# gsanya/orbslam2_NMI

Measured on AMD Instinct MI355X. Metric: pose-candidate NMI evals/sec (640x480, 256 bins), one blocking nmi_search_grid call per step incl. its 8-byte read-back (SURVEY.md 8d's definition); beside the W warm-up steps an untimed clock warm-up of clock_warmup_ms = 200 ms precedes the timed region, higher is better.
Workload: dtype u8

## Files before the change

### include/nmi_hip.h

```cpp
#ifndef NMI_HIP_H
#define NMI_HIP_H

#include <stddef.h>
#include <stdint.h>

#ifdef __cplusplus
extern "C" {
#endif

#define NMI_HIP_ABI_VERSION 2

#define NMI_OK 0
#define NMI_ERR_INVALID_ARGUMENT (-1)
#define NMI_ERR_UNSUPPORTED (-2)
#define NMI_ERR_NO_DEVICE (-3)
#define NMI_ERR_NOT_READY (-4)
#define NMI_ERR_HIP (-1000)
#define NMI_ERR_RCCL (-2000)

#define NMI_MODE_ENMI 0
#define NMI_MODE_SUC 1

typedef struct nmi_ctx nmi_ctx;

// ... 118 lines not shown
int nmi_level_create_mesh_block(nmi_ctx *ctx, const float *d_xyz, const float *d_uv, int64_t n_triangles, const nmi_texture *tex,
                                const uint8_t *d_frame, int32_t S_local, int32_t s_offset, int32_t S_total, int32_t Wn_local,
                                int32_t w_offset, int32_t Wn_total, nmi_level **out);
int nmi_level_create_mesh_colored_block(nmi_ctx *ctx, const float *d_xyz, const float *d_red, int64_t n_triangles, const uint8_t *d_frame,
                                        int32_t S_local, int32_t s_offset, int32_t S_total, int32_t Wn_local, int32_t w_offset,
                                        int32_t Wn_total, nmi_level **out);
int nmi_level_run_rccl(nmi_level *lv, const float *h_mvps, const double *h_forward, void *nccl_comm, int64_t *h_best_index,
                       float *h_best_score);
int nmi_level_copy_outputs(nmi_level *lv, uint8_t *h_renders, uint8_t *h_warps, float *h_ratings);
int nmi_level_set_masks(nmi_level *lv, int32_t enabled, const uint8_t *d_frame_mask);
int nmi_level_copy_masks(nmi_level *lv, uint8_t *h_warp_masks, int32_t *h_counts);
int nmi_level_set_coverage(nmi_level *lv, int32_t enabled, const uint8_t *d_frame_mask);
int nmi_level_copy_coverage(nmi_level *lv, uint8_t *h_render_masks, uint8_t *h_warp_masks, int32_t *h_counts);
int nmi_level_set_distortion(nmi_level *lv, const double K[9], const float dist[5] );
int nmi_level_set_distortion_fisheye(nmi_level *lv, const double K[9], const double K_raw[9] ,
                                     const float dist[4] );
int nmi_level_set_frame_format(nmi_level *lv, int32_t format, int64_t pitch );
int nmi_level_set_frame_reduction(nmi_level *lv, int32_t factor , int32_t format, int64_t pitch );
int nmi_level_destroy(nmi_level *lv);

typedef struct nmi_stream nmi_stream;
int nmi_stream_create(nmi_ctx *ctx, int32_t max_S, int32_t max_Wn, int32_t depth, nmi_stream **out);
int nmi_stream_destroy(nmi_stream *st);
int nmi_stream_submit(nmi_stream *st, const uint8_t *h_render_stack, int32_t S, const uint8_t *h_frame,
                      const double *h_forward, int32_t Wn, int64_t *ticket);
int nmi_stream_submit_block(nmi_stream *st, const uint8_t *h_render_stack, int32_t S_local, int32_t s_offset, int32_t S_total,
                            const uint8_t *h_frame, const double *h_forward, int32_t Wn_local, int32_t w_offset, int32_t Wn_total,
                            void *nccl_comm, int64_t *ticket);
int nmi_stream_wait(nmi_stream *st, int64_t ticket, int64_t *h_best_index, float *h_best_score);
int nmi_stream_keep_ratings(nmi_stream *st, int32_t enabled);
int nmi_stream_copy_ratings(nmi_stream *st, int64_t ticket, float *h_ratings, int64_t n);
int nmi_stream_submit_masked(nmi_stream *st, const uint8_t *h_render_stack, int32_t S, const uint8_t *h_frame,
                             const uint8_t *h_frame_mask , const double *h_forward, int32_t Wn, int64_t *ticket);
int nmi_stream_submit_masked_block(nmi_stream *st, const uint8_t *h_render_stack, int32_t S_local, int32_t s_offset, int32_t S_total,
                                   const uint8_t *h_frame, const uint8_t *h_frame_mask , const double *h_forward,
                                   int32_t Wn_local, int32_t w_offset, int32_t Wn_total, void *nccl_comm, int64_t *ticket);
int nmi_stream_submit_covered(nmi_stream *st, const uint8_t *h_render_stack, const uint8_t *h_render_mask_bits, int32_t S,
                              const uint8_t *h_frame, const uint8_t *h_frame_mask , const double *h_forward,
                              int32_t Wn, int64_t *ticket);
int nmi_stream_submit_covered_block(nmi_stream *st, const uint8_t *h_render_stack, const uint8_t *h_render_mask_bits, int32_t S_local,
                                    int32_t s_offset, int32_t S_total, const uint8_t *h_frame, const uint8_t *h_frame_mask ,
                                    const double *h_forward, int32_t Wn_local, int32_t w_offset, int32_t Wn_total, void *nccl_comm,
                                    int64_t *ticket);
int nmi_stream_copy_counts(nmi_stream *st, int64_t ticket, int32_t *h_counts, int64_t n);
int nmi_stream_set_distortion(nmi_stream *st, const double K[9], const float dist[5] );
int nmi_stream_set_distortion_fisheye(nmi_stream *st, const double K[9], const double K_raw[9] ,
                                      const float dist[4] );
int nmi_stream_set_frame_format(nmi_stream *st, int32_t format, int64_t pitch );
int nmi_stream_set_frame_reduction(nmi_stream *st, int32_t factor , int32_t format, int64_t pitch );

uint64_t nmi_key_pack(float score, int64_t global_linear_index);
int nmi_key_unpack(uint64_t key, int64_t *global_linear_index, float *score);

int nmi_search_grid_rccl(nmi_ctx *ctx, const uint8_t *render_stack, int32_t S_local, int32_t s_offset,
                         int32_t S_total, const uint8_t *warp_stack, int32_t Wn, float *d_ratings,
                         void *nccl_comm, int64_t *h_best_index, float *h_best_score);
int nmi_search_grid_block_rccl(nmi_ctx *ctx, const uint8_t *render_stack, int32_t S_local, int32_t s_offset, int32_t S_total,
                               const uint8_t *warp_stack, int32_t Wn_local, int32_t w_offset, int32_t Wn_total, float *d_ratings,
                               void *nccl_comm, int64_t *h_best_index, float *h_best_score);

int nmi_rccl_unique_id(uint8_t out_id[128]);
int nmi_rccl_comm_init(nmi_ctx *ctx, const uint8_t id[128], int32_t rank, int32_t nranks, void **out_comm);
int nmi_rccl_comm_destroy(void *nccl_comm);

int nmi_set_profiling(nmi_ctx *ctx, int32_t enabled);
int nmi_last_kernel_ms(nmi_ctx *ctx, float *h_ms);

#define NMI_OPT_HIST_VARIANT 1
#define NMI_OPT_PHASE_MASK 2
#define NMI_OPT_WORKGROUPS 3
#define NMI_OPT_RESULT_PATH 4
#define NMI_OPT_XCD_TILING 5
#define NMI_OPT_TILE_QUEUE 6
#define NMI_OPT_CLIP_QUEUE 11
#define NMI_OPT_SPLIT 7
#define NMI_OPT_WAIT_MODE 8
#define NMI_OPT_SPLIT_PIXELS 10
#define NMI_OPT_CONTENT_PATH 12
#define NMI_OPT_FEWLEVELS_BINS 13
#define NMI_OPT_PIX_OWNER_BIAS 14
#define NMI_OPT_STAMPS 9
#define NMI_OPT_STAMP_CANDIDATE 15
#define NMI_OPT_WAVE_SHARES 16
int nmi_set_option(nmi_ctx *ctx, int32_t option, int64_t value);

int nmi_split_status(nmi_ctx *ctx, int32_t *timeouts, int32_t *cooldown_calls_left, int32_t *next_cooldown, int32_t *last_launch_parts);
int nmi_pix_status(nmi_ctx *ctx, int32_t *last_launch_ranges, int32_t *healed);

int nmi_copy_term_table(nmi_ctx *ctx, float *h_out, int64_t n);
int nmi_abi_version(void);
const char *nmi_error_string(int code);
const char *nmi_last_error_detail(nmi_ctx *ctx);
int nmi_get_info(nmi_ctx *ctx, int32_t *compute_units, int32_t *workgroups_per_launch, int32_t *lds_bytes);
int nmi_last_content(nmi_ctx *ctx, int32_t *few_levels, int32_t *nr, int32_t *nw);

#ifdef __cplusplus
}
#endif
#endif
```

### orbslam2_nmi_amd/capi.py

```python
import ctypes as C
import os

import numpy as np

from . import build as _build

MODE_ENMI = 0
MODE_SUC = 1

NMI_OK = 0
ERR_INVALID_ARGUMENT = -1
ERR_UNSUPPORTED = -2
ERR_NO_DEVICE = -3
ERR_NOT_READY = -4

FRAME_GRAY = 0
FRAME_BGR = 1
FRAME_RGB = 2
FRAME_BGRA = 3
FRAME_RGBA = 4
FRAME_BYTES_PER_PIXEL = {FRAME_GRAY: 1, FRAME_BGR: 3, FRAME_RGB: 3, FRAME_BGRA: 4, FRAME_RGBA: 4}

EXPORTED_SYMBOLS = (
    "nmi_params_default", "nmi_create", "nmi_destroy", "nmi_set_stream", "nmi_synchronize", "nmi_eval_pair", "nmi_eval_pairs", "nmi_eval_pair_debug",
    "nmi_search_grid", "nmi_search_grid_shard", "nmi_search_grid_block", "nmi_warp_homographies", "nmi_warp_stack", "nmi_render_mvp", "nmi_render_points", "nmi_level_create", "nmi_level_create_mesh", "nmi_level_run", "nmi_level_copy_outputs", "nmi_level_destroy", "nmi_texture_create",
    "nmi_texture_destroy", "nmi_render_mesh", "nmi_stream_create", "nmi_stream_destroy",
    "nmi_stream_submit", "nmi_stream_wait", "nmi_stream_keep_ratings", "nmi_stream_copy_ratings", "nmi_key_pack", "nmi_key_unpack", "nmi_search_grid_rccl", "nmi_search_grid_block_rccl",
    "nmi_rccl_unique_id", "nmi_rccl_comm_init", "nmi_rccl_comm_destroy", "nmi_set_profiling", "nmi_last_kernel_ms",
    "nmi_set_option", "nmi_copy_term_table", "nmi_abi_version", "nmi_error_string", "nmi_last_error_detail", "nmi_get_info", "nmi_last_content", "nmi_sort_points", "nmi_sort_triangles",
    "nmi_split_status", "nmi_pix_status", "nmi_level_create_block", "nmi_level_create_mesh_block", "nmi_level_run_rccl", "nmi_stream_submit_block",
    "nmi_warp_stack_masked", "nmi_search_grid_masked", "nmi_last_mask_counts", "nmi_level_set_masks", "nmi_level_copy_masks",
    "nmi_render_points_masked", "nmi_render_mesh_masked", "nmi_search_grid_covered", "nmi_last_cover_counts",
    "nmi_level_set_coverage", "nmi_level_copy_coverage",
    "nmi_pack_mask_bits", "nmi_stream_submit_masked", "nmi_stream_submit_masked_block", "nmi_stream_submit_covered",
    "nmi_stream_submit_covered_block", "nmi_stream_copy_counts",
    "nmi_undistort_frame", "nmi_level_set_distortion", "nmi_stream_set_distortion",
    "nmi_gray_frame", "nmi_level_set_frame_format", "nmi_stream_set_frame_format",
    "nmi_reduce_frame", "nmi_level_set_frame_reduction", "nmi_stream_set_frame_reduction",
    "nmi_render_mesh_colored", "nmi_render_mesh_colored_masked", "nmi_sort_triangles_colored", "nmi_level_create_mesh_colored",
    "nmi_level_create_mesh_colored_block",
    "nmi_undistort_frame_fisheye", "nmi_level_set_distortion_fisheye", "nmi_stream_set_distortion_fisheye",
)


class NmiParams(C.Structure):
    _fields_ = [
        ("width", C.c_int32), ("height", C.c_int32), ("bins", C.c_int32), ("mode", C.c_int32),
        ("use_bg", C.c_int32), ("render_bottom_up", C.c_int32), ("device", C.c_int32),
        ("max_candidates", C.c_int32), ("stream", C.c_void_p), ("reserved", C.c_int32 * 8),
    ]


class RenderParams(C.Structure):
    _fields_ = [("fx", C.c_double), ("fy", C.c_double), ("cx", C.c_double), ("cy", C.c_double), ("near_plane", C.c_float),
                ("far_plane", C.c_float), ("point_size", C.c_float)]


class NmiError(RuntimeError):
    def __init__(self, code, what, detail=""):
        self.code = code
        super().__init__(f"{what} failed: {code} ({error_string(code)}) {detail}".strip())


_lib = None


def library_path():
    return _build.LIB


def load_library(build_if_missing=False):
    global _lib
    if _lib is not None:
        return _lib
    path = _build.LIB
    if build_if_missing:
        _build.build()
    if not os.path.exists(path):
        raise RuntimeError(f"{path} is missing: run `python -m orbslam2_nmi_amd.build` (hipcc, gfx950). "
                           "There is no CPU fallback for the NMI path.")
    lib = C.CDLL(path, mode=C.RTLD_GLOBAL)
    vp, i32, i64p, f32p, u64p = C.c_void_p, C.c_int32, C.POINTER(C.c_int64), C.POINTER(C.c_float), C.POINTER(C.c_uint64)
    lib.nmi_params_default.argtypes = [C.POINTER(NmiParams), i32, i32]
    lib.nmi_create.argtypes = [C.POINTER(NmiParams), C.POINTER(vp)]
    lib.nmi_destroy.argtypes = [vp]
    lib.nmi_set_stream.argtypes = [vp, vp]
    lib.nmi_synchronize.argtypes = [vp]
    lib.nmi_eval_pair.argtypes = [vp, vp, vp, f32p]
    lib.nmi_eval_pairs.argtypes = [vp, C.POINTER(vp), C.POINTER(vp), i32, f32p]
    lib.nmi_eval_pair_debug.argtypes = [vp, vp, vp, f32p, vp, vp, vp, vp]
    lib.nmi_search_grid.argtypes = [vp, vp, i32, vp, i32, vp, i64p, f32p]
    lib.nmi_search_grid_shard.argtypes = [vp, vp, i32, i32, i32, vp, i32, vp, vp, u64p]
    lib.nmi_search_grid_block.argtypes = [vp, vp, i32, i32, i32, vp, i32, i32, i32, vp, vp, u64p]
    lib.nmi_warp_homographies.argtypes = [C.POINTER(C.c_double), C.POINTER(i32), f32p, C.POINTER(C.c_double)]
    lib.nmi_warp_stack.argtypes = [vp, vp, C.POINTER(C.c_double), i32, vp]
    lib.nmi_warp_stack_masked.argtypes = [vp, vp, vp, C.POINTER(C.c_double), i32, vp, vp]
    lib.nmi_search_grid_masked.argtypes = [vp, vp, i32, vp, vp, i32, vp, i64p, f32p]
    lib.nmi_last_mask_counts.argtypes = [vp, C.POINTER(i32), i32]
    lib.nmi_render_points_masked.argtypes = [vp, vp, vp, C.c_int64, C.POINTER(C.c_float), i32, C.c_float, vp, vp]
    lib.nmi_render_mesh_masked.argtypes = [vp, vp, vp, C.c_int64, vp, C.POINTER(C.c_float), i32, vp, vp]
    lib.nmi_search_grid_covered.argtypes = [vp, vp, vp, i32, vp, vp, i32, vp, i64p, f32p]
    lib.nmi_last_cover_counts.argtypes = [vp, C.POINTER(i32), i32]
    lib.nmi_render_mvp.argtypes = [C.POINTER(RenderParams), f32p, f32p, f32p, f32p, f32p]
    lib.nmi_render_points.argtypes = [vp, vp, vp, C.c_int64, f32p, i32, C.c_float, vp]
    lib.nmi_texture_create.argtypes = [vp, vp, i32, i32, C.POINTER(vp)]
    lib.nmi_texture_destroy.argtypes = [vp]
    lib.nmi_render_mesh.argtypes = [vp, vp, vp, C.c_int64, vp, f32p, i32, vp]
    lib.nmi_level_create.argtypes = [vp, vp, vp, C.c_int64, vp, i32, i32, C.c_float, C.POINTER(vp)]
    lib.nmi_level_create_mesh.argtypes = [vp, vp, vp, C.c_int64, vp, vp, i32, i32, C.POINTER(vp)]
    lib.nmi_level_run.argtypes = [vp, f32p, C.POINTER(C.c_double), i64p, f32p]
    lib.nmi_level_create_block.argtypes = [vp, vp, vp, C.c_int64, vp, i32, i32, i32, i32, i32, i32, C.c_float, C.POINTER(vp)]
    lib.nmi_level_create_mesh_block.argtypes = [vp, vp, vp, C.c_int64, vp, vp, i32, i32, i32, i32, i32, i32, C.POINTER(vp)]
    lib.nmi_render_mesh_colored.argtypes = [vp, vp, vp, C.c_int64, f32p, i32, vp]
    lib.nmi_render_mesh_colored_masked.argtypes = [vp, vp, vp, C.c_int64, f32p, i32, vp, vp]
    lib.nmi_sort_triangles_colored.argtypes = [vp, vp, vp, C.c_int64, vp, vp]
    lib.nmi_level_create_mesh_colored.argtypes = [vp, vp, vp, C.c_int64, vp, i32, i32, C.POINTER(vp)]
    lib.nmi_level_create_mesh_colored_block.argtypes = [vp, vp, vp, C.c_int64, vp, i32, i32, i32, i32, i32, i32, C.POINTER(vp)]
    lib.nmi_level_run_rccl.argtypes = [vp, f32p, C.POINTER(C.c_double), vp, i64p, f32p]
    lib.nmi_stream_submit_block.argtypes = [vp, vp, i32, i32, i32, vp, C.POINTER(C.c_double), i32, i32, i32, vp, i64p]
    lib.nmi_level_copy_outputs.argtypes = [vp, vp, vp, vp]
    lib.nmi_level_set_masks.argtypes = [vp, i32, vp]
    lib.nmi_level_copy_masks.argtypes = [vp, vp, C.POINTER(i32)]
    lib.nmi_level_set_coverage.argtypes = [vp, i32, vp]
    lib.nmi_level_copy_coverage.argtypes = [vp, vp, vp, C.POINTER(i32)]
    lib.nmi_level_destroy.argtypes = [vp]
    lib.nmi_stream_create.argtypes = [vp, i32, i32, i32, C.POINTER(vp)]
    lib.nmi_stream_destroy.argtypes = [vp]
    lib.nmi_stream_submit.argtypes = [vp, vp, i32, vp, C.POINTER(C.c_double), i32, i64p]
    lib.nmi_stream_wait.argtypes = [vp, C.c_int64, i64p, f32p]
    lib.nmi_stream_keep_ratings.argtypes = [vp, i32]
    lib.nmi_stream_copy_ratings.argtypes = [vp, C.c_int64, f32p, C.c_int64]
    lib.nmi_pack_mask_bits.argtypes = [vp, vp, i32, vp]
    lib.nmi_stream_submit_masked.argtypes = [vp, vp, i32, vp, vp, C.POINTER(C.c_double), i32, i64p]
    lib.nmi_stream_submit_masked_block.argtypes = [vp, vp, i32, i32, i32, vp, vp, C.POINTER(C.c_double), i32, i32, i32, vp, i64p]
    lib.nmi_stream_submit_covered.argtypes = [vp, vp, vp, i32, vp, vp, C.POINTER(C.c_double), i32, i64p]
    lib.nmi_stream_submit_covered_block.argtypes = [vp, vp, vp, i32, i32, i32, vp, vp, C.POINTER(C.c_double), i32, i32, i32, vp, i64p]
    lib.nmi_stream_copy_counts.argtypes = [vp, C.c_int64, C.POINTER(i32), C.c_int64]
    lib.nmi_undistort_frame.argtypes = [vp, C.POINTER(C.c_double), f32p, vp, vp, vp, vp]
    lib.nmi_level_set_distortion.argtypes = [vp, C.POINTER(C.c_double), f32p]
    lib.nmi_stream_set_distortion.argtypes = [vp, C.POINTER(C.c_double), f32p]
    lib.nmi_undistort_frame_fisheye.argtypes = [vp, C.POINTER(C.c_double), C.POINTER(C.c_double), f32p, vp, vp, vp, vp]
    lib.nmi_level_set_distortion_fisheye.argtypes = [vp, C.POINTER(C.c_double), C.POINTER(C.c_double), f32p]
    lib.nmi_stream_set_distortion_fisheye.argtypes = [vp, C.POINTER(C.c_double), C.POINTER(C.c_double), f32p]
    lib.nmi_gray_frame.argtypes = [vp, vp, i32, C.c_int64, vp]
    lib.nmi_level_set_frame_format.argtypes = [vp, i32, C.c_int64]
    lib.nmi_stream_set_frame_format.argtypes = [vp, i32, C.c_int64]
    lib.nmi_reduce_frame.argtypes = [vp, vp, i32, C.c_int64, i32, vp, vp, vp]
    lib.nmi_level_set_frame_reduction.argtypes = [vp, i32, i32, C.c_int64]
    lib.nmi_stream_set_frame_reduction.argtypes = [vp, i32, i32, C.c_int64]
    lib.nmi_key_pack.argtypes = [C.c_float, C.c_int64]
    lib.nmi_key_pack.restype = C.c_uint64
    lib.nmi_key_unpack.argtypes = [C.c_uint64, i64p, f32p]
    lib.nmi_search_grid_rccl.argtypes = [vp, vp, i32, i32, i32, vp, i32, vp, vp, i64p, f32p]
    lib.nmi_search_grid_block_rccl.argtypes = [vp, vp, i32, i32, i32, vp, i32, i32, i32, vp, vp, i64p, f32p]
    lib.nmi_rccl_unique_id.argtypes = [C.POINTER(C.c_uint8)]
    lib.nmi_rccl_comm_init.argtypes = [vp, C.POINTER(C.c_uint8), i32, i32, C.POINTER(vp)]
    lib.nmi_rccl_comm_destroy.argtypes = [vp]
    lib.nmi_set_option.argtypes = [vp, i32, C.c_int64]
    lib.nmi_set_profiling.argtypes = [vp, i32]
    lib.nmi_last_kernel_ms.argtypes = [vp, f32p]
    lib.nmi_copy_term_table.argtypes = [vp, f32p, C.c_int64]
    lib.nmi_error_string.argtypes = [C.c_int]
    lib.nmi_error_string.restype = C.c_char_p
    lib.nmi_last_error_detail.argtypes = [vp]
    lib.nmi_last_error_detail.restype = C.c_char_p
    lib.nmi_get_info.argtypes = [vp, C.POINTER(i32), C.POINTER(i32), C.POINTER(i32)]
    lib.nmi_last_content.argtypes = [vp, C.POINTER(i32), C.POINTER(i32), C.POINTER(i32)]
    lib.nmi_split_status.argtypes = [vp, C.POINTER(i32), C.POINTER(i32), C.POINTER(i32), C.POINTER(i32)]
    lib.nmi_pix_status.argtypes = [vp, C.POINTER(i32), C.POINTER(i32)]
    lib.nmi_sort_points.argtypes = [vp, vp, vp, C.c_int64, vp, vp]
    lib.nmi_sort_triangles.argtypes = [vp, vp, vp, C.c_int64, vp, vp]
    _lib = lib
    return lib


def error_string(code):
    return load_library().nmi_error_string(int(code)).decode()


def key_pack(score, index):
    return int(load_library().nmi_key_pack(float(score), int(index)))


def key_unpack(key):
    idx, sc = C.c_int64(0), C.c_float(0)
    load_library().nmi_key_unpack(C.c_uint64(int(key) & 0xFFFFFFFFFFFFFFFF), C.byref(idx), C.byref(sc))
    return int(idx.value), np.float32(sc.value)


def warp_homographies(K, num_warp_xyz, step_rad_xyz):
    K = np.ascontiguousarray(K, np.float64).reshape(9)
    num = (C.c_int32 * 3)(*[int(n) for n in num_warp_xyz])
    step = (C.c_float * 3)(*[float(s) for s in step_rad_xyz])
    wn = int(np.prod([int(n) for n in num_warp_xyz]))
    out = np.zeros((wn, 3, 3), np.float64)
    rc = load_library().nmi_warp_homographies(K.ctypes.data_as(C.POINTER(C.c_double)), num, step,
                                              out.ctypes.data_as(C.POINTER(C.c_double)))
    if rc != NMI_OK:
        raise NmiError(rc, "nmi_warp_homographies")
    return out


def render_mvp(rp, cam_pos, cam_look_at, cam_up, translation):
    f3 = lambda v: (C.c_float * 3)(*[float(x) for x in v])
    out = (C.c_float * 16)()
    rc = load_library().nmi_render_mvp(C.byref(rp), f3(cam_pos), f3(cam_look_at), f3(cam_up), f3(translation), out)
    if rc != NMI_OK:
        raise NmiError(rc, "nmi_render_mvp")
    return np.array(out, np.float32)


def _lens(K, dist):
    if K is None and dist is None:
        return None, None, None, None
    k = np.ascontiguousarray(K, np.float64).reshape(-1)
    if k.size != 9:
        raise ValueError("K must have 9 entries")
    if dist is None:
        return k, None, k.ctypes.data_as(C.POINTER(C.c_double)), None
    d = np.ascontiguousarray(dist, np.float32).reshape(-1)
    if d.size != 5:
        raise ValueError("dist must be k1 k2 p1 p2 k3 (5 entries; pad k3 = 0)")
    return k, d, k.ctypes.data_as(C.POINTER(C.c_double)), d.ctypes.data_as(C.POINTER(C.c_float))


def _fisheye(K, K_raw, dist):
    if K is None and dist is None:
        return (None, None, None), (None, None, None)
    k = np.ascontiguousarray(K, np.float64).reshape(-1)
    kr = None if K_raw is None else np.ascontiguousarray(K_raw, np.float64).reshape(-1)
    if k.size != 9 or (kr is not None and kr.size != 9):
        raise ValueError("K and K_raw must have 9 entries")
    d = None if dist is None else np.ascontiguousarray(dist, np.float32).reshape(-1)
    if d is not None and d.size != 4:
        raise ValueError("dist must be k1 k2 k3 k4 (4 entries)")
    dp = C.POINTER(C.c_double)
    return (k, kr, d), (k.ctypes.data_as(dp), None if kr is None else kr.ctypes.data_as(dp),
                        None if d is None else d.ctypes.data_as(C.POINTER(C.c_float)))


def _dev_mask(t, ndim, what):
    import torch
    if not isinstance(t, torch.Tensor) or not t.is_cuda:
        raise TypeError(f"{what} must be a device (HIP) torch tensor; the NMI path has no CPU implementation")
    if t.dtype not in (torch.uint8, torch.bool) or t.dim() != ndim or not t.is_contiguous():
        raise TypeError(f"{what} must be a contiguous uint8 or bool tensor with {ndim} dims, got {t.dtype} {tuple(t.shape)}")
    return t


def _dev_u8(t, ndim, what):
    import torch
    if not isinstance(t, torch.Tensor) or not t.is_cuda:
        raise TypeError(f"{what} must be a device (HIP) torch tensor; the NMI path has no CPU implementation")
    if t.dtype != torch.uint8 or t.dim() != ndim or not t.is_contiguous():
        raise TypeError(f"{what} must be a contiguous uint8 tensor with {ndim} dims, got {t.dtype} {tuple(t.shape)}")
    return t


class NmiContext:

    default_options = {}

    def __init__(self, width, height, bins=256, mode=MODE_SUC, use_bg=True, render_bottom_up=True, device=None,
                 stream=None, max_candidates=0):
        import torch
        if not torch.cuda.is_available():
            raise RuntimeError("no HIP device visible: orbslam2_nmi_amd needs an AMD GPU (gfx950)")
        self._lib = load_library()
        self.width, self.height = int(width), int(height)
        self.bins, self.mode, self.use_bg, self.render_bottom_up = bins, mode, bool(use_bg), bool(render_bottom_up)
        if device is None:
            device = torch.cuda.current_device()
        self.device = torch.device("cuda", int(device) if not isinstance(device, torch.device) else device.index or 0)
        p = NmiParams()
        self._check(self._lib.nmi_params_default(C.byref(p), self.width, self.height), "nmi_params_default")
        p.bins, p.mode, p.use_bg, p.render_bottom_up = int(bins), int(mode), int(bool(use_bg)), int(bool(render_bottom_up))
        p.device = self.device.index
        p.max_candidates = int(max_candidates)
        p.stream = stream
        self._h = C.c_void_p()
        rc = self._lib.nmi_create(C.byref(p), C.byref(self._h))
        if rc != NMI_OK:
            self._h = C.c_void_p()
            raise NmiError(rc, "nmi_create")
        for opt, val in type(self).default_options.items():
            self.set_option(opt, val)

    def _check(self, rc, what):
        if rc != NMI_OK:
            detail = self._lib.nmi_last_error_detail(self._h).decode() if getattr(self, "_h", None) else ""
            raise NmiError(rc, what, detail)

    def close(self):
        if getattr(self, "_h", None) and self._h.value:
            self._lib.nmi_destroy(self._h)
            self._h = C.c_void_p()

    def __del__(self):
        try:
            self.close()
        except Exception:
            pass

    def __enter__(self):
        return self

    def __exit__(self, *exc):
        self.close()

    def set_stream(self, stream_handle):
        if stream_handle == 0:
            raise ValueError("handle 0 is the legacy default stream; use a torch.cuda.Stream() (non-default) instead")
        self._check(self._lib.nmi_set_stream(self._h, C.c_void_p(stream_handle)), "nmi_set_stream")
        self._bound_stream = stream_handle

    def _order_after_torch(self):
        import torch
        cur = torch.cuda.current_stream(self.device)
        if getattr(self, "_bound_stream", None) != cur.cuda_stream:
            cur.synchronize()

    OPT_HIST_VARIANT, OPT_PHASE_MASK, OPT_WORKGROUPS, OPT_RESULT_PATH, OPT_XCD_TILING, OPT_TILE_QUEUE = 1, 2, 3, 4, 5, 6
    OPT_SPLIT, OPT_WAIT_MODE, OPT_STAMPS, OPT_SPLIT_PIXELS, OPT_CLIP_QUEUE = 7, 8, 9, 10, 11
    OPT_PIX_OWNER_BIAS = 14
    OPT_STAMP_CANDIDATE, OPT_WAVE_SHARES = 15, 16
    OPT_CONTENT_PATH, OPT_FEWLEVELS_BINS = 12, 13

    def set_option(self, option, value):
        self._check(self._lib.nmi_set_option(self._h, int(option), int(value)), "nmi_set_option")

    def synchronize(self):
        self._check(self._lib.nmi_synchronize(self._h), "nmi_synchronize")

    def set_profiling(self, on):
        self._check(self._lib.nmi_set_profiling(self._h, int(bool(on))), "nmi_set_profiling")

    def last_kernel_ms(self):
        ms = C.c_float(0)
        self._check(self._lib.nmi_last_kernel_ms(self._h, C.byref(ms)), "nmi_last_kernel_ms")
        return float(ms.value)

    def info(self):
        cu, wg, lds = C.c_int32(0), C.c_int32(0), C.c_int32(0)
        self._check(self._lib.nmi_get_info(self._h, C.byref(cu), C.byref(wg), C.byref(lds)), "nmi_get_info")
        return {"compute_units": cu.value, "workgroups_per_launch": wg.value, "lds_bytes": lds.value}

    def last_content(self):
        f, r, w = C.c_int32(0), C.c_int32(0), C.c_int32(0)
        self._check(self._lib.nmi_last_content(self._h, C.byref(f), C.byref(r), C.byref(w)), "nmi_last_content")
        return {"few_levels": bool(f.value), "nr": r.value, "nw": w.value}

    def split_status(self):
        v = [C.c_int32(0) for _ in range(4)]
        self._check(self._lib.nmi_split_status(self._h, *[C.byref(x) for x in v]), "nmi_split_status")
        return dict(zip(("timeouts", "cooldown_calls_left", "next_cooldown", "last_launch_parts"), (x.value for x in v)))

    def pix_status(self):
        v = [C.c_int32(0) for _ in range(2)]
        self._check(self._lib.nmi_pix_status(self._h, *[C.byref(x) for x in v]), "nmi_pix_status")
        return dict(zip(("last_launch_ranges", "healed"), (x.value for x in v)))

    def term_table(self):
        out = np.zeros(self.width * self.height + 1, np.float32)
        self._check(self._lib.nmi_copy_term_table(self._h, out.ctypes.data_as(C.POINTER(C.c_float)), out.size),
                    "nmi_copy_term_table")
        return out

    def _img(self, t, what):
        t = _dev_u8(t, 2, what)
        if tuple(t.shape) != (self.height, self.width):
            raise ValueError(f"{what} is {tuple(t.shape)}, context is {(self.height, self.width)}")
        return t

    def _stack(self, t, what):
        t = _dev_u8(t, 3, what)
        if tuple(t.shape[1:]) != (self.height, self.width):
            raise ValueError(f"{what} is {tuple(t.shape)}, context images are {(self.height, self.width)}")
        return t

    def eval_pair(self, render, warped):
        r, w = self._img(render, "render"), self._img(warped, "warped")
        out = C.c_float(0)
        self._order_after_torch()
        self._check(self._lib.nmi_eval_pair(self._h, r.data_ptr(), w.data_ptr(), C.byref(out)), "nmi_eval_pair")
        return np.float32(out.value)

    def eval_pairs(self, renders, warps):
        assert len(renders) == len(warps)
        n = len(renders)
        rp = (C.c_void_p * max(n, 1))(*[self._img(r, "render").data_ptr() for r in renders])
        wp = (C.c_void_p * max(n, 1))(*[self._img(w, "warped").data_ptr() for w in warps])
        out = np.zeros(n, np.float32)
        self._order_after_torch()
        self._check(self._lib.nmi_eval_pairs(self._h, rp, wp, n, out.ctypes.data_as(C.POINTER(C.c_float))), "nmi_eval_pairs")
        return out

    def eval_pair_debug(self, render, warped):
        import torch
        r, w = self._img(render, "render"), self._img(warped, "warped")
        joint = torch.zeros(65536, dtype=torch.int32, device=self.device)
        h1 = torch.zeros(256, dtype=torch.int32, device=self.device)
        h2 = torch.zeros(256, dtype=torch.int32, device=self.device)
        sums = torch.zeros(3, dtype=torch.float32, device=self.device)
        torch.cuda.synchronize(self.device)
        out = C.c_float(0)
        self._check(self._lib.nmi_eval_pair_debug(self._h, r.data_ptr(), w.data_ptr(), C.byref(out), joint.data_ptr(),
                                                  h1.data_ptr(), h2.data_ptr(), sums.data_ptr()), "nmi_eval_pair_debug")
        u32 = lambda t: t.cpu().numpy().view(np.uint32)
        return np.float32(out.value), u32(joint).reshape(256, 256), u32(h1), u32(h2), sums.cpu().numpy()

    def sort_points(self, xyz, red):
        import torch
        assert xyz.is_cuda and red.is_cuda and xyz.dtype == torch.float32 and red.dtype == torch.float32
        xyz, red = xyz.contiguous(), red.contiguous()
        n = xyz.shape[0]
        assert tuple(xyz.shape) == (n, 3) and red.numel() == n
        xo, ro = torch.empty_like(xyz), torch.empty_like(red)
        self._order_after_torch()
        self._check(self._lib.nmi_sort_points(self._h, xyz.data_ptr(), red.data_ptr(), n, xo.data_ptr(), ro.data_ptr()), "nmi_sort_points")
        return xo, ro

    def sort_triangles(self, xyz, uv):
        import torch
        assert xyz.is_cuda and uv.is_cuda and xyz.dtype == torch.float32 and uv.dtype == torch.float32
        xyz, uv = xyz.contiguous(), uv.contiguous()
        t = xyz.shape[0] // 3
        assert tuple(xyz.shape) == (3 * t, 3) and tuple(uv.shape) == (3 * t, 2)
        xo, uo = torch.empty_like(xyz), torch.empty_like(uv)
        self._order_after_torch()
        self._check(self._lib.nmi_sort_triangles(self._h, xyz.data_ptr(), uv.data_ptr(), t, xo.data_ptr(), uo.data_ptr()), "nmi_sort_triangles")
        return xo, uo

    def sort_triangles_colored(self, xyz, red):
# ... 707 lines not shown
```

### orbslam2_nmi_amd/csrc/nmi_capi.cpp

```cpp
#include <sched.h>

#include "nmi_ctx.h"

namespace nmi_internal {

int hip_fail(nmi_ctx *ctx, hipError_t e, const char *what)
{
    if (ctx) {
        char buf[256];
        snprintf(buf, sizeof buf, "%s: %s (%d)", what, hipGetErrorString(e), (int)e);
        ctx->detail = buf;
    }
    return NMI_ERR_HIP - (int)e;
}



void build_order(int S, int Wn, int *order)
{
    const int tile_s = S >= 8 ? 8 : (S >= 4 ? 4 : (S >= 2 ? 2 : 1)), tile_w = 32 / tile_s;
    int64_t o = 0;
    for (int w0 = 0; w0 < Wn; w0 += tile_w)
        for (int s0 = 0; s0 < S; s0 += tile_s)
            for (int w = w0; w < w0 + tile_w && w < Wn; ++w)
                for (int s = s0; s < s0 + tile_s && s < S; ++s) order[o++] = w * S + s;
}

int ensure_order(nmi_ctx *ctx, int S, int Wn, const int **d_order)
{
    *d_order = nullptr;
    if (!ctx->xcd_tiling) return NMI_OK;
    const int64_t total = (int64_t)S * Wn;
    nmi_ctx::OrderEntry *victim = nullptr;
    for (auto &e : ctx->orders) {
        if (e.S == S && e.Wn == Wn) {
            e.last_use = ++ctx->order_clock;
            *d_order = e.d;
            return NMI_OK;
        }
        if (!victim || (e.d == nullptr && victim->d != nullptr) || ((e.d == nullptr) == (victim->d == nullptr) && e.last_use < victim->last_use))
            victim = &e;
    }
    nmi_ctx::OrderEntry &e = *victim;
    if (e.d) NMI_HIP_TRY(ctx, hipStreamSynchronize(ctx->stream));
    if (total > e.cap) {
        if (e.d) NMI_HIP_TRY(ctx, hipFree(e.d));
        if (e.h) NMI_HIP_TRY(ctx, hipHostFree(e.h));
        e.d = e.h = nullptr;
        e.cap = 0;
        e.S = e.Wn = -1;
        NMI_HIP_TRY(ctx, hipMalloc((void **)&e.d, (size_t)total * sizeof(int)));
        NMI_HIP_TRY(ctx, hipHostMalloc((void **)&e.h, (size_t)total * sizeof(int), hipHostMallocDefault));
        e.cap = total;
    }
    build_order(S, Wn, e.h);
    NMI_HIP_TRY(ctx, hipMemcpyAsync(e.d, e.h, (size_t)total * sizeof(int), hipMemcpyHostToDevice, ctx->stream));
    e.S = S;
    e.Wn = Wn;
    e.last_use = ++ctx->order_clock;
    *d_order = e.d;
    return NMI_OK;
}

static void choose_split(const nmi_ctx *ctx, int64_t total, int cap, int *parts, int *pix_parts)
{
    *parts = 0;
    *pix_parts = 1;
    if (cap > ctx->compute_units) cap = ctx->compute_units;
    if (ctx->hist_variant != 3 || ctx->split_mode == 0 || ctx->split_mode == 1 || total <= 0 || total > cap) return;
    auto fits = [&](int k, int p) { return nmi::split_workgroups((int)total, k, p) <= cap; };
    auto exists = [](int k, int p) { return p == 1 || (k == 8 && (p == 2 || p == 4)) || (k == 4 && p == 2); };
    const int want_p = ctx->split_pixels;
    if (ctx->split_mode > 0) {
        const int k = ctx->split_mode;
        if (!fits(k, 1)) return;
        *parts = k;
        if (want_p == 1) return;
        for (int p = 4; p >= 2; p >>= 1)
            if ((want_p == -1 || want_p == p) && exists(k, p) && fits(k, p)) {
                *pix_parts = p;
                return;
            }
        return;
    }
    static const int order[][2] = {{8, 4}, {8, 2}, {4, 2}, {8, 1}, {4, 1}};
    for (const auto &kp : order) {
        if (kp[1] > 1 && want_p != -1 && want_p != kp[1]) continue;
        if (fits(kp[0], kp[1])) {
            *parts = kp[0];
            *pix_parts = kp[1];
            return;
        }
    }
}

int choose_pix(const nmi_ctx *ctx, const nmi::GridArgs &a, int64_t total, int cap)
{
    if (cap > ctx->compute_units) cap = ctx->compute_units;
    if (ctx->hist_variant != 3 || a.width < 32 || (ctx->shift != 0 && !ctx->params.use_bg) || ctx->pair_renders || total <= 0) return 0;
    if ((ctx->phase_mask & ~512) != 3 || (a.dbg_stamps != nullptr && ctx->split_mode != 1)) return 0;
    if (ctx->split_mode == 1) {
        const int p = ctx->split_pixels;
        return (p >= 2 && p <= nmi::pix_max_ranges() && total * p <= cap) ? p : 0;
    }
    if (ctx->split_mode != -1 || ctx->split_pixels != -1 || total * 2 > cap) return 0;
    const int p = (int)(cap / total);
    if (!a.vec_ok) return p > nmi::pix_max_ranges() ? nmi::pix_max_ranges() : p;
    if (total <= 32) return 0;
    return p > 3 ? 3 : p;
}

double pix_owner_share(const nmi_ctx *ctx, int pix)
{
    const double owner_px = ((double)ctx->npix + (double)(pix - 1) * ctx->pix_owner_bias) / pix;
    return owner_px < ctx->npix ? owner_px / ctx->npix : 1.0;
}

int ensure_pix_timeouts(nmi_ctx *ctx)
{
    if (ctx->d_pix_timeouts) return NMI_OK;
    NMI_HIP_TRY(ctx, hipMalloc((void **)&ctx->d_pix_timeouts, sizeof(uint32_t)));
    NMI_HIP_TRY(ctx, hipMemsetAsync(ctx->d_pix_timeouts, 0, sizeof(uint32_t), ctx->stream));
    return NMI_OK;
}

int next_split_epoch(nmi_ctx *ctx, uint32_t *epoch)
{
    uint32_t e = ctx->split_epoch + 1;
    if ((e & 0xFFFFu) == 0) {
        if (ctx->d_blocks) NMI_HIP_TRY(ctx, hipMemsetAsync(ctx->d_blocks, 0, ctx->blocks_bytes, ctx->stream));
        if (ctx->d_pix_blocks) NMI_HIP_TRY(ctx, hipMemsetAsync(ctx->d_pix_blocks, 0, ctx->pix_blocks_bytes, ctx->stream));
        if (e == 0 && ctx->d_slabs) NMI_HIP_TRY(ctx, hipMemsetAsync(ctx->d_slabs, 0, (size_t)ctx->slab_cap * sizeof(nmi::SplitSlab), ctx->stream));
        ++e;
    }
    ctx->split_epoch = *epoch = e;
    return NMI_OK;
}

static int ensure_slabs(nmi_ctx *ctx, int n)
{
    if (n <= ctx->slab_cap) return NMI_OK;
    if (ctx->d_slabs) {
        NMI_HIP_TRY(ctx, hipStreamSynchronize(ctx->stream));
        NMI_HIP_TRY(ctx, hipFree(ctx->d_slabs));
// ... 16 lines not shown
        ctx->d_pix_blocks = nullptr;
        ctx->pix_blocks_bytes = 0;
    }
    NMI_HIP_TRY(ctx, hipMalloc((void **)&ctx->d_pix_blocks, bytes));
    NMI_HIP_TRY(ctx, hipMemsetAsync(ctx->d_pix_blocks, 0, bytes, ctx->stream));
    ctx->pix_blocks_bytes = bytes;
    return NMI_OK;
}

static int ensure_blocks(nmi_ctx *ctx, size_t bytes)
{
    if (bytes <= ctx->blocks_bytes) return NMI_OK;
    if (ctx->d_blocks) {
        NMI_HIP_TRY(ctx, hipStreamSynchronize(ctx->stream));
        NMI_HIP_TRY(ctx, hipFree(ctx->d_blocks));
        ctx->d_blocks = nullptr;
        ctx->blocks_bytes = 0;
    }
    NMI_HIP_TRY(ctx, hipMalloc((void **)&ctx->d_blocks, bytes));
    NMI_HIP_TRY(ctx, hipMemsetAsync(ctx->d_blocks, 0, bytes, ctx->stream));
    ctx->blocks_bytes = bytes;
    return NMI_OK;
}

int enqueue_grid(nmi_ctx *ctx, const uint8_t *render_stack, int S_local, int s_offset, int S_total,
                 const uint8_t *warp_stack, int Wn, float *d_ratings, unsigned long long *out_key, bool post,
                 uint32_t *dbg_joint, uint32_t *dbg_h1, uint32_t *dbg_h2, float *dbg_sums, int w_offset, bool post_score)
{
    const nmi_params &p = ctx->params;
    nmi::GridArgs a{};
    a.render_stack = render_stack;
    a.warp_stack = warp_stack;
    a.S_local = S_local;
    a.Wn = Wn;
    a.s_offset = s_offset;
    a.S_total = S_total;
    a.w_offset = w_offset;
    nmi::set_geometry(a, p.width, p.height, render_stack, warp_stack, p.render_bottom_up != 0);
    if (ctx->pair_renders) {
        a.pair_renders = ctx->pair_renders;
        a.pair_warps = ctx->pair_warps;
        uintptr_t bits = 0;
        for (int i = 0; i < S_local; ++i) bits |= (uintptr_t)ctx->pair_renders_host[i] | (uintptr_t)ctx->pair_warps_host[i];
        if (bits % 16) nmi::set_geometry(a, p.width, p.height, (const void *)1, (const void *)1, p.render_bottom_up != 0);
    }
    a.shift = ctx->shift;
    a.mode = p.mode;
    a.table = ctx->table;
    a.scratch = ctx->d_scratch;
    a.order = nullptr;
    a.ratings = d_ratings;
    a.key = ctx->d_keys + ctx->slot;
    a.reset_key = ctx->d_keys + (ctx->slot ^ 1);
    a.out_key = out_key;
    a.done = ctx->d_done;
    const bool split_checked = post || post_score || ctx->allow_unchecked_split || ctx->pair_renders != nullptr;
    post = post && ctx->result_path == 1;
    post_score = post_score && ctx->result_path == 1;
    a.mailbox = post ? ctx->mailbox : nullptr;
    a.score_post = post_score ? ctx->score_mailbox : nullptr;
    a.seq = post ? ctx->seq + 1 : (post_score ? ctx->pair_seq + 1 : 0);
    a.dbg_joint = dbg_joint;
    a.dbg_h1 = dbg_h1;
    a.dbg_h2 = dbg_h2;
    a.dbg_sums = dbg_sums;
    a.hist_variant = ctx->hist_variant;
    a.phase_mask = ctx->phase_mask;
    a.dbg_stamps = ctx->dbg_stamps;

    const int64_t total = (int64_t)S_local * Wn;
    if (total == 0) {
        if (out_key) NMI_HIP_TRY(ctx, hipMemsetAsync(out_key, 0, sizeof(unsigned long long), ctx->stream));
        NMI_HIP_TRY(ctx, hipMemsetAsync(ctx->d_keys + ctx->slot, 0, sizeof(unsigned long long), ctx->stream));
        NMI_HIP_TRY(ctx, hipStreamSynchronize(ctx->stream));
        if (post) {
            ++ctx->seq;
            ctx->mailbox->word = (unsigned long long)(ctx->seq & 1u) << 63;
        }
        ctx->posted = post;
        ctx->last_slot = ctx->slot;
        ctx->last_parts = 0;
        ctx->last_pix = 0;
        ctx->last_epoch = 0;
        return NMI_OK;
    }
    const int cap = ctx->workgroups > 0 ? ctx->workgroups : ctx->compute_units;
    int parts = 0, pix_parts = 1;
    choose_split(ctx, total, cap, &parts, &pix_parts);
    if (pix_parts > 1 && ctx->npix >= (1 << 24)) pix_parts = 1;
    int pix = choose_pix(ctx, a, total, cap);
    if (pix) parts = 0;
    if (parts && !split_checked) parts = 0;
    if (parts && ctx->split_cooldown > 0) {
        --ctx->split_cooldown;
        parts = 0;
    }
    if (!parts) pix_parts = 1;
    bool few = false;
    const bool few_eligible = !parts && !(pix && ctx->split_mode == 1) && a.vec_ok && (ctx->shift == 0 || p.use_bg) && ctx->hist_variant == 3 && ctx->phase_mask == 3 && !dbg_joint &&
                              !dbg_h1 && !dbg_h2 && !dbg_sums && !ctx->pair_renders && !ctx->dbg_stamps && ctx->content_path != 0;
    if (few_eligible) {
        const unsigned long long posted = __atomic_load_n(ctx->level_post, __ATOMIC_ACQUIRE);
        if ((uint32_t)(posted >> 32) != ctx->level_seen) {
            ctx->level_seen = (uint32_t)(posted >> 32);
            const uint32_t joint = (uint32_t)((posted >> 16) & 0xFFFFu) * (uint32_t)(posted & 0xFFFFu);
            ctx->few_hint = joint > 0 && joint <= (uint32_t)ctx->fewlevels_bins;
        }
        few = ctx->content_path == 1 || ctx->few_hint;
    }
    if (few) pix = 0;
    if (ctx->pair_renders && !parts) return NMI_ERR_UNSUPPORTED;
    int workgroups = (int)(total < cap ? total : cap);
    if (parts) {
        int rs = ensure_slabs(ctx, (int)total);
        if (rs == NMI_OK && pix_parts > 1) rs = ensure_blocks(ctx, (size_t)total * nmi::split_block_bytes_per_candidate(pix_parts));
        if (rs != NMI_OK) return rs;
        if (rs == NMI_OK) rs = next_split_epoch(ctx, &a.epoch);
        if (rs != NMI_OK) return rs;
        a.slabs = ctx->d_slabs;
        a.blocks = ctx->d_blocks;
        a.split_error = ctx->d_split_error;
        workgroups = nmi::split_workgroups((int)total, parts, pix_parts);
    } else if (pix) {
        int rs = ensure_pix_blocks(ctx, nmi::pix_block_bytes((int)total, pix));
        if (rs == NMI_OK) rs = next_split_epoch(ctx, &a.epoch);
        if (rs == NMI_OK) rs = ensure_pix_timeouts(ctx);
        if (rs != NMI_OK) return rs;
        a.blocks = ctx->d_pix_blocks;
        workgroups = (int)total * pix;
    } else if (ctx->xcd_tiling && total <= (1ll << 24)) {
        const int orc = ensure_order(ctx, S_local, Wn, &a.order);
        if (orc != NMI_OK) return orc;
    }
#ifdef NMI_BUILD_ABLATIONS
    if (ctx->hist_variant == 4 && workgroups > ctx->scratch_workgroups) {
        NMI_HIP_TRY(ctx, hipStreamSynchronize(ctx->stream));
        if (ctx->d_scratch) NMI_HIP_TRY(ctx, hipFree(ctx->d_scratch));
        ctx->d_scratch = nullptr;
        ctx->scratch_workgroups = 0;
        const int alloc = workgroups > ctx->compute_units ? workgroups : ctx->compute_units;
        NMI_HIP_TRY(ctx, hipMalloc((void **)&ctx->d_scratch, nmi::grid_kernel_scratch_bytes(alloc)));
        ctx->scratch_workgroups = alloc;
        a.scratch = ctx->d_scratch;
    }
#endif
    if (!parts && !few && ctx->hist_variant == 3 && ctx->content_path != 0) a.plan = ctx->d_plan;
    if (few) {
        const size_t need = (size_t)(S_local + Wn) * (size_t)ctx->npix;
        if (need > ctx->rank_bytes) {
            NMI_HIP_TRY(ctx, hipStreamSynchronize(ctx->stream));
            if (ctx->d_rank_stacks) NMI_HIP_TRY(ctx, hipFree(ctx->d_rank_stacks));
            ctx->d_rank_stacks = nullptr;
            ctx->rank_bytes = 0;
            const size_t want = need + need / 2;
            NMI_HIP_TRY(ctx, hipMalloc((void **)&ctx->d_rank_stacks, want));
            ctx->rank_bytes = want;
        }
        a.plan = ctx->d_plan;
    }
    if (ctx->profiling) NMI_HIP_TRY(ctx, hipEventRecord(ctx->ev_start, ctx->stream));
    if (few)
        NMI_HIP_TRY(ctx, nmi::launch_levels(render_stack, S_local, warp_stack, Wn, ctx->npix, ctx->shift, ctx->d_plan, ctx->level_post, ++ctx->level_seq,
                                            (uint32_t)ctx->fewlevels_bins, few, ctx->stream));
    if (parts) {
        NMI_HIP_TRY(ctx, nmi::launch_split(a, parts, pix_parts, workgroups, p.use_bg != 0, ctx->stream));
    } else if (pix) {
        NMI_HIP_TRY(ctx, nmi::launch_pix(a, pix, pix_owner_share(ctx, pix), p.use_bg != 0, nullptr, ctx->d_pix_timeouts, ctx->stream));
    } else if (few) {
        NMI_HIP_TRY(ctx, nmi::launch_fewlevels(a, ctx->d_rank_stacks, ctx->d_rank_stacks + (size_t)S_local * ctx->npix, workgroups,
                                               p.use_bg != 0, ctx->stream));
        NMI_HIP_TRY(ctx, nmi::launch_grid_gated(a, workgroups, p.use_bg != 0, ctx->stream));
    } else {
        NMI_HIP_TRY(ctx, nmi::launch_grid(a, workgroups, p.use_bg != 0, ctx->stream));
    }
    ctx->last_few = few ? 1 : 0;
    if (post) ++ctx->seq;
    if (post_score) ++ctx->pair_seq;
    ctx->posted = post;
    ctx->last_slot = ctx->slot;
    ctx->slot ^= 1;
    ctx->last_parts = parts;
    ctx->last_pix = pix;
    ctx->last_epoch = parts ? a.epoch : 0;
    if (ctx->profiling) {
        NMI_HIP_TRY(ctx, hipEventRecord(ctx->ev_stop, ctx->stream));
        ctx->have_timing = true;
    }
    return NMI_OK;
}

bool split_launch_failed(nmi_ctx *ctx, int parts, uint32_t epoch)
{
    if (!parts) return false;
    uint32_t *word = ctx->h_split_error + (epoch % nmi::kSplitRing);
    if (__atomic_load_n(word, __ATOMIC_ACQUIRE) != epoch) {
        if ((int32_t)(epoch - ctx->split_cooldown_epoch) > 0) ctx->split_backoff = nmi_ctx::kSplitBackoffMin;
        return false;
    }
    (void)hipStreamSynchronize(ctx->stream);
    __atomic_store_n(word, 0u, __ATOMIC_RELEASE);
    ++ctx->split_timeouts;
    ctx->split_cooldown = ctx->split_backoff;
    ctx->split_cooldown_epoch = ctx->split_epoch;
    if (ctx->split_backoff < nmi_ctx::kSplitBackoffMax) ctx->split_backoff *= 2;
    return true;
}

bool split_timed_out(nmi_ctx *ctx) { return split_launch_failed(ctx, ctx->last_parts, ctx->last_epoch); }

static const char *const kSplitTimeoutNote = "split kernel hand-off timed out; call redone by the one-workgroup kernel, split forms paused (nmi_split_status)";

int wait_word(nmi_ctx *ctx, const volatile unsigned long long *word, unsigned long long mask, unsigned long long want,
              unsigned long long *out)
{
    const uint64_t check_every = ctx->wait_mode == 1 ? 0x3F : 0xFFFF;
    for (uint64_t spin = 0;; ++spin) {
        const unsigned long long v = __atomic_load_n(word, __ATOMIC_ACQUIRE);
        if ((v & mask) == want) {
            *out = v;
            return NMI_OK;
        }
        if (ctx->wait_mode == 1) sched_yield();
        if ((spin & check_every) == check_every) {
            const hipError_t q = hipStreamQuery(ctx->stream);
            if (q == hipSuccess) {
                const unsigned long long v2 = __atomic_load_n(word, __ATOMIC_ACQUIRE);
                *out = v2;
                return (v2 & mask) == want ? NMI_OK : NMI_ERR_NOT_READY;
            }
            if (q != hipErrorNotReady) return hip_fail(ctx, q, "hipStreamQuery");
        }
    }
}

int fetch_key(nmi_ctx *ctx, unsigned long long *key)
{
    if (ctx->posted) {
        unsigned long long word = 0;
        const int rc = wait_word(ctx, &ctx->mailbox->word, 1ull << 63, (unsigned long long)(ctx->seq & 1u) << 63, &word);
        if (rc == NMI_OK) {
            *key = word & 0x7FFFFFFFFFFFFFFFull;
            return NMI_OK;
        }
        if (rc != NMI_ERR_NOT_READY) return rc;
    }
    NMI_HIP_TRY(ctx, hipMemcpyAsync(ctx->h_key, ctx->d_keys + ctx->last_slot, sizeof(unsigned long long),
                                    hipMemcpyDeviceToHost, ctx->stream));
    NMI_HIP_TRY(ctx, hipStreamSynchronize(ctx->stream));
    *key = *ctx->h_key;
    return NMI_OK;
}

int stage_floats(nmi_ctx *ctx, StagingRing &ring, const float *h_src, size_t n, float **d_out)
{
    if (n > ring.cap) {
        NMI_HIP_TRY(ctx, hipStreamSynchronize(ctx->stream));
        for (int i = 0; i < StagingRing::kSlots; ++i) {
            if (ring.d[i]) NMI_HIP_TRY(ctx, hipFree(ring.d[i]));
// ... 96 lines not shown
    ctx->shift = shift;
    DeviceGuard guard(dev);

    int rc = NMI_OK;
    auto fail = [&](hipError_t e, const char *what) {
        rc = hip_fail(ctx, e, what);
        fprintf(stderr, "nmi_create: %s\n", ctx->detail.c_str());
        nmi_destroy(ctx);
        return rc;
    };
    hipDeviceProp_t prop;
    hipError_t e = hipGetDeviceProperties(&prop, dev);
    if (e != hipSuccess) return fail(e, "hipGetDeviceProperties");
    ctx->compute_units = prop.multiProcessorCount;
    if ((size_t)nmi::grid_kernel_lds_bytes() > prop.sharedMemPerBlock) {
        nmi_destroy(ctx);
        return NMI_ERR_UNSUPPORTED;
    }
    if ((e = hipStreamCreateWithFlags(&ctx->own_stream, hipStreamNonBlocking)) != hipSuccess)
        return fail(e, "hipStreamCreateWithFlags");
    ctx->stream = p.stream ? (hipStream_t)p.stream : ctx->own_stream;
    if ((e = hipMalloc((void **)&ctx->table, ((size_t)ctx->npix + 1) * sizeof(float))) != hipSuccess)
        return fail(e, "hipMalloc(table)");
    if ((e = hipMalloc((void **)&ctx->d_keys, 2 * sizeof(unsigned long long))) != hipSuccess) return fail(e, "hipMalloc(key)");
    if ((e = hipMalloc((void **)&ctx->d_done, sizeof(unsigned int))) != hipSuccess) return fail(e, "hipMalloc(done)");
    if ((e = hipMemsetAsync(ctx->d_keys, 0, 2 * sizeof(unsigned long long), ctx->stream)) != hipSuccess)
        return fail(e, "hipMemsetAsync(key)");
    if ((e = hipMemsetAsync(ctx->d_done, 0, sizeof(unsigned int), ctx->stream)) != hipSuccess)
        return fail(e, "hipMemsetAsync(done)");
    if ((e = hipHostMalloc((void **)&ctx->mailbox, sizeof(nmi::Mailbox), hipHostMallocCoherent | hipHostMallocMapped)) !=
        hipSuccess)
        return fail(e, "hipHostMalloc(mailbox)");
    memset(ctx->mailbox, 0, sizeof(nmi::Mailbox));
    if ((e = hipMalloc((void **)&ctx->d_pair_rating, sizeof(float))) != hipSuccess) return fail(e, "hipMalloc(rating)");
    if ((e = hipMalloc((void **)&ctx->d_reduced_key, sizeof(unsigned long long))) != hipSuccess) return fail(e, "hipMalloc(reduced key)");
    if ((e = hipHostMalloc((void **)&ctx->score_mailbox, 2 * sizeof(unsigned long long), hipHostMallocCoherent | hipHostMallocMapped)) !=
        hipSuccess)
        return fail(e, "hipHostMalloc(score mailbox)");
    memset(ctx->score_mailbox, 0, 2 * sizeof(unsigned long long));
    if ((e = hipHostMalloc((void **)&ctx->h_split_error, nmi::kSplitRing * sizeof(uint32_t), hipHostMallocCoherent | hipHostMallocMapped)) != hipSuccess)
        return fail(e, "hipHostMalloc(split error)");
    memset(ctx->h_split_error, 0, nmi::kSplitRing * sizeof(uint32_t));
    if ((e = hipHostGetDevicePointer((void **)&ctx->d_split_error, ctx->h_split_error, 0)) != hipSuccess)
        return fail(e, "hipHostGetDevicePointer(split error)");
    if ((e = hipHostMalloc((void **)&ctx->h_key, sizeof(unsigned long long), hipHostMallocDefault)) != hipSuccess)
        return fail(e, "hipHostMalloc(key)");
    if ((e = hipHostMalloc((void **)&ctx->level_post, 64, hipHostMallocCoherent | hipHostMallocMapped)) != hipSuccess)
        return fail(e, "hipHostMalloc(level post)");
    *ctx->level_post = 0;
    if ((e = hipMalloc((void **)&ctx->d_plan, sizeof(nmi::LevelPlan))) != hipSuccess) return fail(e, "hipMalloc(level plan)");
    if ((e = hipMemsetAsync(ctx->d_plan, 0, sizeof(nmi::LevelPlan), ctx->stream)) != hipSuccess) return fail(e, "hipMemsetAsync(level plan)");
    {
        unsigned long long *d_post = nullptr;
        if ((e = hipHostGetDevicePointer((void **)&d_post, ctx->level_post, 0)) != hipSuccess) return fail(e, "hipHostGetDevicePointer(level post)");
        if ((e = hipMemcpyAsync(&ctx->d_plan->seen_post, &d_post, sizeof d_post, hipMemcpyHostToDevice, ctx->stream)) != hipSuccess)
            return fail(e, "hipMemcpyAsync(level post)");
        const uint32_t max_joint = (uint32_t)ctx->fewlevels_bins;
        if ((e = hipMemcpyAsync(&ctx->d_plan->seen_max_joint, &max_joint, sizeof max_joint, hipMemcpyHostToDevice, ctx->stream)) != hipSuccess)
            return fail(e, "hipMemcpyAsync(level plan)");
        if ((e = hipStreamSynchronize(ctx->stream)) != hipSuccess) return fail(e, "hipStreamSynchronize");
    }
    if ((e = hipEventCreate(&ctx->ev_start)) != hipSuccess) return fail(e, "hipEventCreate");
    if ((e = hipEventCreate(&ctx->ev_stop)) != hipSuccess) return fail(e, "hipEventCreate");
    if ((e = nmi::launch_table(ctx->table, ctx->npix, ctx->stream)) != hipSuccess) return fail(e, "launch_table");
    if ((e = hipStreamSynchronize(ctx->stream)) != hipSuccess) return fail(e, "hipStreamSynchronize");
    *out_ctx = ctx;
    return NMI_OK;
}

int nmi_destroy(nmi_ctx *ctx)
{
    if (!ctx) return NMI_OK;
    DeviceGuard guard(ctx->device);
    if (ctx->own_stream) (void)hipStreamSynchronize(ctx->own_stream);
    if (ctx->table) (void)hipFree(ctx->table);
    if (ctx->d_reduced_key) (void)hipFree(ctx->d_reduced_key);
    if (ctx->score_mailbox) (void)hipHostFree(ctx->score_mailbox);
    if (ctx->d_slabs) (void)hipFree(ctx->d_slabs);
    if (ctx->h_pair_table) (void)hipHostFree(ctx->h_pair_table);
    if (ctx->d_pair_scores) (void)hipFree(ctx->d_pair_scores);
    if (ctx->d_blocks) (void)hipFree(ctx->d_blocks);
    if (ctx->d_pix_timeouts) (void)hipFree(ctx->d_pix_timeouts);
    if (ctx->d_pix_blocks) (void)hipFree(ctx->d_pix_blocks);
    if (ctx->h_split_error) (void)hipHostFree(ctx->h_split_error);
    if (ctx->level_post) (void)hipHostFree(ctx->level_post);
    if (ctx->d_plan) (void)hipFree(ctx->d_plan);
    if (ctx->d_rank_stacks) (void)hipFree(ctx->d_rank_stacks);
    if (ctx->d_keys) (void)hipFree(ctx->d_keys);
    if (ctx->d_done) (void)hipFree(ctx->d_done);
    if (ctx->mailbox) (void)hipHostFree(ctx->mailbox);
    if (ctx->d_pair_rating) (void)hipFree(ctx->d_pair_rating);
    if (ctx->d_scratch) (void)hipFree(ctx->d_scratch);
    if (ctx->d_mask_counts) (void)hipFree(ctx->d_mask_counts);
    if (ctx->d_mask_tables) (void)hipFree(ctx->d_mask_tables);
    if (ctx->d_mask_redo) (void)hipFree(ctx->d_mask_redo);
    if (ctx->d_mask_redo_state) (void)hipFree(ctx->d_mask_redo_state);
    if (ctx->d_cover_counts) (void)hipFree(ctx->d_cover_counts);
    if (ctx->d_zbuf) (void)hipFree(ctx->d_zbuf);
    mesh_work_free(&ctx->mesh);
    for (int i = 0; i < StagingRing::kSlots; ++i) {
        if (ctx->mvp_ring.d[i]) (void)hipFree(ctx->mvp_ring.d[i]);
        if (ctx->mvp_ring.h[i]) (void)hipHostFree(ctx->mvp_ring.h[i]);
        if (ctx->mvp_ring.ev[i]) (void)hipEventDestroy(ctx->mvp_ring.ev[i]);
    }
    for (auto &oe : ctx->orders) {
        if (oe.d) (void)hipFree(oe.d);
        if (oe.h) (void)hipHostFree(oe.h);
    }
    for (int i = 0; i < nmi_ctx::kWarpRing; ++i) {
        if (ctx->d_warp_coeffs[i]) (void)hipFree(ctx->d_warp_coeffs[i]);
        if (ctx->h_warp_coeffs[i]) (void)hipHostFree(ctx->h_warp_coeffs[i]);
        if (ctx->warp_ev[i]) (void)hipEventDestroy(ctx->warp_ev[i]);
    }
    if (ctx->h_key) (void)hipHostFree(ctx->h_key);
    if (ctx->ev_start) (void)hipEventDestroy(ctx->ev_start);
    if (ctx->ev_stop) (void)hipEventDestroy(ctx->ev_stop);
    if (ctx->own_stream) (void)hipStreamDestroy(ctx->own_stream);
    delete ctx;
    return NMI_OK;
}

int nmi_set_stream(nmi_ctx *ctx, void *stream)
{
    if (!ctx) return NMI_ERR_INVALID_ARGUMENT;
    ctx->stream = stream ? (hipStream_t)stream : ctx->own_stream;
    return NMI_OK;
}

int nmi_synchronize(nmi_ctx *ctx)
{
    if (!ctx) return NMI_ERR_INVALID_ARGUMENT;
    DeviceGuard guard(ctx->device);
    NMI_HIP_TRY(ctx, hipStreamSynchronize(ctx->stream));
    return NMI_OK;
}

int nmi_set_option(nmi_ctx *ctx, int32_t option, int64_t value)
{
    if (!ctx) return NMI_ERR_INVALID_ARGUMENT;
    switch (option) {
    case NMI_OPT_HIST_VARIANT:
        if (value < 0 || value > 4) return NMI_ERR_INVALID_ARGUMENT;
        if (value != 1 && value != 3 && !nmi::ablation_variants_built()) return NMI_ERR_UNSUPPORTED;
        ctx->hist_variant = (int)value;
        return NMI_OK;
    case NMI_OPT_SPLIT:
        if (value != -1 && value != 0 && value != 1 && value != 2 && value != 4 && value != 8) return NMI_ERR_INVALID_ARGUMENT;
        ctx->split_mode = (int)value;
        return NMI_OK;
    case NMI_OPT_SPLIT_PIXELS:
        if (value != -1 && (value < 1 || value > 8)) return NMI_ERR_INVALID_ARGUMENT;
        ctx->split_pixels = (int)value;
        return NMI_OK;
    case NMI_OPT_PIX_OWNER_BIAS:
        if (value < 0 || value > (1 << 24)) return NMI_ERR_INVALID_ARGUMENT;
        ctx->pix_owner_bias = (int)value;
        return NMI_OK;
    case NMI_OPT_STAMPS:
        ctx->dbg_stamps = (unsigned long long *)(uintptr_t)value;
        return NMI_OK;
    case NMI_OPT_STAMP_CANDIDATE:
    case NMI_OPT_WAVE_SHARES:
        if (option == NMI_OPT_STAMP_CANDIDATE ? (value < 0 || value > 65535) : value == 0) return NMI_ERR_INVALID_ARGUMENT;
        {
            DeviceGuard guard(ctx->device);
            NMI_HIP_TRY(ctx, hipStreamSynchronize(ctx->stream));
            if (option == NMI_OPT_STAMP_CANDIDATE) ctx->stamp_candidate = (int)value;
            NMI_HIP_TRY(ctx, nmi::set_stamped_experiment(ctx->stamp_candidate, option == NMI_OPT_WAVE_SHARES ? (const uint32_t *)(uintptr_t)value : nullptr));
        }
        return NMI_OK;
    case NMI_OPT_WAIT_MODE:
        if (value < 0 || value > 1) return NMI_ERR_INVALID_ARGUMENT;
        ctx->wait_mode = (int)value;
        return NMI_OK;
    case NMI_OPT_PHASE_MASK:
        if (value < 0 || value > 1023) return NMI_ERR_INVALID_ARGUMENT;
        ctx->phase_mask = (int)value;
        return NMI_OK;
    case NMI_OPT_XCD_TILING:
        if (value < 0 || value > 1) return NMI_ERR_INVALID_ARGUMENT;
        ctx->xcd_tiling = (int)value;
        return NMI_OK;
    case NMI_OPT_RESULT_PATH:
        if (value < 0 || value > 1) return NMI_ERR_INVALID_ARGUMENT;
        ctx->result_path = (int)value;
        return NMI_OK;
    case NMI_OPT_TILE_QUEUE:
        if (value < 0 || value > (4ll << 20)) return NMI_ERR_INVALID_ARGUMENT;
        ctx->tile_queue_limit = (unsigned long long)value;
        return NMI_OK;
    case NMI_OPT_CLIP_QUEUE:
        if (value < 0) return NMI_ERR_INVALID_ARGUMENT;
        ctx->clip_queue_limit = (unsigned long long)value;
        return NMI_OK;
    case NMI_OPT_CONTENT_PATH:
        if (value < -1 || value > 1) return NMI_ERR_INVALID_ARGUMENT;
        ctx->content_path = (int)value;
        ctx->few_hint = false;
        {
            DeviceGuard guard(ctx->device);
            const uint32_t zero = 0;
            NMI_HIP_TRY(ctx, hipMemcpyAsync(&ctx->d_plan->seen_state, &zero, sizeof zero, hipMemcpyHostToDevice, ctx->stream));
            NMI_HIP_TRY(ctx, hipStreamSynchronize(ctx->stream));
        }
        return NMI_OK;
    case NMI_OPT_FEWLEVELS_BINS:
        if (value < 1 || value > nmi::fewlevels_max_joint()) return NMI_ERR_INVALID_ARGUMENT;
        ctx->fewlevels_bins = (int)value;
        {
            DeviceGuard guard(ctx->device);
            const uint32_t max_joint = (uint32_t)value, zero = 0;
            NMI_HIP_TRY(ctx, hipMemcpyAsync(&ctx->d_plan->seen_max_joint, &max_joint, sizeof max_joint, hipMemcpyHostToDevice, ctx->stream));
            NMI_HIP_TRY(ctx, hipMemcpyAsync(&ctx->d_plan->seen_state, &zero, sizeof zero, hipMemcpyHostToDevice, ctx->stream));
            NMI_HIP_TRY(ctx, hipStreamSynchronize(ctx->stream));
            ctx->few_hint = false;
        }
        return NMI_OK;
    case NMI_OPT_WORKGROUPS:
        if (value < 0 || value > (1 << 20)) return NMI_ERR_INVALID_ARGUMENT;
        ctx->workgroups = (int)value;
        return NMI_OK;
    default:
        return NMI_ERR_INVALID_ARGUMENT;
    }
}

int nmi_set_profiling(nmi_ctx *ctx, int32_t enabled)
{
    if (!ctx) return NMI_ERR_INVALID_ARGUMENT;
    ctx->profiling = enabled != 0;
    ctx->have_timing = false;
    return NMI_OK;
}

int nmi_last_kernel_ms(nmi_ctx *ctx, float *h_ms)
{
    if (!ctx || !h_ms) return NMI_ERR_INVALID_ARGUMENT;
    if (!ctx->have_timing) return NMI_ERR_NOT_READY;
    DeviceGuard guard(ctx->device);
    NMI_HIP_TRY(ctx, hipEventSynchronize(ctx->ev_stop));
    NMI_HIP_TRY(ctx, hipEventElapsedTime(h_ms, ctx->ev_start, ctx->ev_stop));
    return NMI_OK;
}

int nmi_get_info(nmi_ctx *ctx, int32_t *compute_units, int32_t *workgroups_per_launch, int32_t *lds_bytes)
{
    if (!ctx) return NMI_ERR_INVALID_ARGUMENT;
    if (compute_units) *compute_units = ctx->compute_units;
    if (workgroups_per_launch) *workgroups_per_launch = ctx->workgroups > 0 ? ctx->workgroups : ctx->compute_units;
    if (lds_bytes) *lds_bytes = nmi::grid_kernel_lds_bytes();
    return NMI_OK;
}

int nmi_last_content(nmi_ctx *ctx, int32_t *few_levels, int32_t *nr, int32_t *nw)
{
    if (!ctx) return NMI_ERR_INVALID_ARGUMENT;
    DeviceGuard guard(ctx->device);
    NMI_HIP_TRY(ctx, hipStreamSynchronize(ctx->stream));
    const unsigned long long posted = __atomic_load_n(ctx->level_post, __ATOMIC_ACQUIRE);
    const int32_t r = (int32_t)((posted >> 16) & 0xFFFFu), w = (int32_t)(posted & 0xFFFFu);
    if (nr) *nr = r;
    if (nw) *nw = w;
    uint32_t use = 0;
    if (few_levels && ctx->last_few) {
        NMI_HIP_TRY(ctx, hipMemcpyAsync(&use, &ctx->d_plan->use, sizeof use, hipMemcpyDeviceToHost, ctx->stream));
        NMI_HIP_TRY(ctx, hipStreamSynchronize(ctx->stream));
    }
    if (few_levels) *few_levels = use ? 1 : 0;
    return NMI_OK;
}

int nmi_copy_term_table(nmi_ctx *ctx, float *h_out, int64_t n)
{
    if (!ctx || !h_out || n != (int64_t)ctx->npix + 1) return NMI_ERR_INVALID_ARGUMENT;
    DeviceGuard guard(ctx->device);
    NMI_HIP_TRY(ctx, hipMemcpyAsync(h_out, ctx->table, (size_t)n * sizeof(float), hipMemcpyDeviceToHost, ctx->stream));
    NMI_HIP_TRY(ctx, hipStreamSynchronize(ctx->stream));
    return NMI_OK;
}

uint64_t nmi_key_pack(float score, int64_t global_linear_index)
{
    if (!(score >= 0.0f) || global_linear_index < 0 || global_linear_index >= 0xFFFFFFFFll) return 0;
    uint32_t bits = 0;
    if (score != 0.0f) memcpy(&bits, &score, sizeof bits);
    return ((uint64_t)bits << 32) | (uint64_t)(0xFFFFFFFFu - (uint32_t)global_linear_index);
}

int nmi_key_unpack(uint64_t key, int64_t *global_linear_index, float *score)
{
    if (key == 0) {
        if (global_linear_index) *global_linear_index = -1;
        if (score) *score = 0.0f;
        return NMI_OK;
    }
    const uint32_t bits = (uint32_t)(key >> 32);
    if (global_linear_index) *global_linear_index = (int64_t)(0xFFFFFFFFu - (uint32_t)(key & 0xFFFFFFFFu));
    if (score) memcpy(score, &bits, sizeof bits);
    return NMI_OK;
}

int nmi_search_grid_shard(nmi_ctx *ctx, const uint8_t *render_stack, int32_t S_local, int32_t s_offset, int32_t S_total,
                          const uint8_t *warp_stack, int32_t Wn, float *d_ratings, uint64_t *d_key, uint64_t *h_key)
{
    return nmi_search_grid_block(ctx, render_stack, S_local, s_offset, S_total, warp_stack, Wn, 0, Wn, d_ratings, d_key, h_key);
}

int nmi_search_grid_block(nmi_ctx *ctx, const uint8_t *render_stack, int32_t S_local, int32_t s_offset, int32_t S_total,
                          const uint8_t *warp_stack, int32_t Wn_local, int32_t w_offset, int32_t Wn_total, float *d_ratings,
                          uint64_t *d_key, uint64_t *h_key)
{
    return search_block(ctx, render_stack, S_local, s_offset, S_total, warp_stack, Wn_local, w_offset, Wn_total, d_ratings, d_key, h_key,
                        false);
}

}

int nmi_internal::search_block(nmi_ctx *ctx, const uint8_t *render_stack, int32_t S_local, int32_t s_offset, int32_t S_total,
                               const uint8_t *warp_stack, int32_t Wn_local, int32_t w_offset, int32_t Wn_total, float *d_ratings,
                               uint64_t *d_key, uint64_t *h_key, bool caller_checks)
{
    int rc = check_grid_args(ctx, render_stack, S_local, s_offset, S_total, warp_stack, Wn_local);
    if (rc != NMI_OK) return rc;
    if (w_offset < 0 || Wn_total < Wn_local || w_offset + Wn_local > Wn_total) return NMI_ERR_INVALID_ARGUMENT;
    if ((int64_t)S_total * Wn_total >= 0x7FFFFFFFll) return NMI_ERR_UNSUPPORTED;
    const int32_t Wn = Wn_local;
    DeviceGuard guard(ctx->device);
    ctx->allow_unchecked_split = caller_checks;
    rc = enqueue_grid(ctx, render_stack, S_local, s_offset, S_total, warp_stack, Wn, d_ratings, (unsigned long long *)d_key,
                      h_key != nullptr, nullptr, nullptr, nullptr, nullptr, w_offset);
    ctx->allow_unchecked_split = false;
    if (rc != NMI_OK) return rc;
    if (h_key) {
        unsigned long long k = 0;
        rc = fetch_key(ctx, &k);
// ... 171 lines not shown
```

### orbslam2_nmi_amd/csrc/nmi_capi_masked.cpp

```cpp
#include "nmi_ctx.h"

using namespace nmi_internal;

namespace {

int ensure_mask_work(nmi_ctx *ctx, int Wn)
{
    if (Wn > ctx->mask_warps_cap) {
        NMI_HIP_TRY(ctx, hipStreamSynchronize(ctx->stream));
        if (ctx->d_mask_counts) NMI_HIP_TRY(ctx, hipFree(ctx->d_mask_counts));
        if (ctx->d_mask_tables) NMI_HIP_TRY(ctx, hipFree(ctx->d_mask_tables));
        ctx->d_mask_counts = nullptr;
        ctx->d_mask_tables = nullptr;
        ctx->mask_warps_cap = 0;
        ctx->mask_count_n = 0;
        NMI_HIP_TRY(ctx, hipMalloc((void **)&ctx->d_mask_counts, (size_t)Wn * sizeof(int32_t)));
        NMI_HIP_TRY(ctx, hipMalloc((void **)&ctx->d_mask_tables, (size_t)Wn * ((size_t)ctx->npix + 1) * sizeof(float)));
        ctx->mask_warps_cap = Wn;
    }
    return NMI_OK;
}

}

// ... 30 lines not shown
        m.redo_n = redo_state;
        m.redo_done = redo_state + 1;
    } else {
        nmi::MaskedGridArgs &m = ms.masked;
        m.g = a;
        m.warp_masks = warp_masks;
        m.tables = tables;
        m.counts = counts;
        m.vec_ok = a.vec_ok && ((uintptr_t)warp_masks % 16) == 0;
        m.redo = redo;
        m.redo_n = redo_state;
        m.redo_done = redo_state + 1;
    }
    return ms;
}

hipError_t nmi_internal::launch_mask_search(const MaskSearch &ms, int pix, double owner_share, int workgroups, bool use_bg, bool exact,
                                            const uint32_t *replay, uint32_t *healed, hipStream_t stream)
{
    if (ms.covered)
        return pix ? nmi::launch_pix_covered(ms.cover, pix, owner_share, use_bg, replay, healed, stream)
                   : nmi::launch_grid_covered(ms.cover, workgroups, use_bg, exact, stream);
    return pix ? nmi::launch_pix_masked(ms.masked, pix, owner_share, use_bg, replay, healed, stream)
               : nmi::launch_grid_masked(ms.masked, workgroups, use_bg, exact, stream);
}

int nmi_internal::enqueue_grid_mask(nmi_ctx *ctx, const uint8_t *render_stack, const uint8_t *render_masks, int S_local, int s_offset,
                                    int S_total, const uint8_t *warp_stack, const uint8_t *warp_masks, int Wn, int w_offset, int32_t *counts,
                                    const float *tables, int32_t *redo, uint32_t *redo_state, float *d_ratings, unsigned long long *out_key,
                                    bool post)
{
    const nmi_params &p = ctx->params;
    const int64_t total = (int64_t)S_local * Wn;
    int rc = NMI_OK;
    nmi::GridArgs a{};
    a.render_stack = render_stack;
    a.warp_stack = warp_stack;
    a.S_local = S_local;
    a.Wn = Wn;
    a.s_offset = s_offset;
    a.S_total = S_total;
    a.w_offset = w_offset;
    nmi::set_geometry(a, p.width, p.height, render_stack, warp_stack, p.render_bottom_up != 0);
    a.shift = ctx->shift;
    a.mode = p.mode;
    a.table = nullptr;
    a.plan = nullptr;
    a.ratings = d_ratings;
    a.key = ctx->d_keys + ctx->slot;
    a.reset_key = ctx->d_keys + (ctx->slot ^ 1);
    a.out_key = out_key;
    a.done = ctx->d_done;
    post = post && ctx->result_path == 1;
    a.mailbox = post ? ctx->mailbox : nullptr;
    a.seq = post ? ctx->seq + 1 : 0;
    a.hist_variant = ctx->hist_variant;
    a.phase_mask = 3;
    const int cap = ctx->workgroups > 0 ? ctx->workgroups : ctx->compute_units;
    const int workgroups = (int)(total < cap ? total : cap);
    const int pix = choose_pix(ctx, a, total, cap);
    if (pix) {
        rc = ensure_pix_blocks(ctx, nmi::pix_block_bytes((int)total, pix));
        if (rc == NMI_OK) rc = next_split_epoch(ctx, &a.epoch);
        if (rc == NMI_OK) rc = ensure_pix_timeouts(ctx);
        if (rc != NMI_OK) return rc;
        a.blocks = ctx->d_pix_blocks;
        a.phase_mask = 3 | (ctx->phase_mask & 512);
    } else if (ctx->xcd_tiling && total <= (1ll << 24)) {
        rc = ensure_order(ctx, S_local, Wn, &a.order);
        if (rc != NMI_OK) return rc;
    }
    const MaskSearch ms = mask_search_args(a, warp_masks, render_masks, counts, tables, redo, redo_state);
    if (ctx->profiling) NMI_HIP_TRY(ctx, hipEventRecord(ctx->ev_start, ctx->stream));
    NMI_HIP_TRY(ctx, launch_mask_search(ms, pix, pix ? pix_owner_share(ctx, pix) : 0.0, workgroups, p.use_bg != 0, ctx->hist_variant == 1, nullptr,
                                        ctx->d_pix_timeouts, ctx->stream));
    if (post) ++ctx->seq;
    ctx->posted = post;
    ctx->last_slot = ctx->slot;
    ctx->slot ^= 1;
    ctx->last_parts = 0;
    ctx->last_pix = pix;
    ctx->last_epoch = 0;
    ctx->last_few = 0;
    if (ctx->profiling) {
        NMI_HIP_TRY(ctx, hipEventRecord(ctx->ev_stop, ctx->stream));
        ctx->have_timing = true;
    }
    return NMI_OK;
}

extern "C" {

int nmi_warp_stack_masked(nmi_ctx *ctx, const uint8_t *d_frame, const uint8_t *d_frame_mask, const double *h_forward, int32_t Wn,
                          uint8_t *d_warp_stack, uint8_t *d_warp_masks)
{
    if (!ctx || !d_frame || !h_forward || !d_warp_stack || !d_warp_masks || Wn <= 0) return NMI_ERR_INVALID_ARGUMENT;
    int rc = nmi_warp_stack(ctx, d_frame, h_forward, Wn, d_warp_stack);
    if (rc != NMI_OK) return rc;
    DeviceGuard guard(ctx->device);
    const int ring = (int)((ctx->warp_uses - 1) % nmi_ctx::kWarpRing);
    NMI_HIP_TRY(ctx, nmi::launch_warp_masks(d_frame_mask, ctx->d_warp_coeffs[ring], d_warp_masks, ctx->params.width, ctx->params.height,
                                            Wn, ctx->stream));
    NMI_HIP_TRY(ctx, hipEventRecord(ctx->warp_ev[ring], ctx->stream));
    return NMI_OK;
}

int nmi_search_grid_masked(nmi_ctx *ctx, const uint8_t *render_stack, int32_t S, const uint8_t *warp_stack, const uint8_t *warp_masks,
                           int32_t Wn, float *d_ratings, int64_t *h_best_index, float *h_best_score)
{
    int rc = check_grid_args(ctx, render_stack, S, 0, S, warp_stack, Wn);
    if (rc != NMI_OK) return rc;
    if (!warp_masks) return NMI_ERR_INVALID_ARGUMENT;
    DeviceGuard guard(ctx->device);
    const int64_t total = (int64_t)S * Wn;
    if (Wn > 0) {
        rc = ensure_mask_work(ctx, Wn);
        if (rc == NMI_OK) rc = ensure_mask_redo(ctx, total);
        if (rc != NMI_OK) return rc;
        NMI_HIP_TRY(ctx, nmi::launch_mask_counts(warp_masks, Wn, ctx->npix, ctx->d_mask_counts, ctx->stream));
        NMI_HIP_TRY(ctx, nmi::launch_mask_tables(ctx->d_mask_counts, Wn, ctx->npix, ctx->d_mask_tables, ctx->stream));
        ctx->mask_count_n = Wn;
    }
    if (total == 0) {
        NMI_HIP_TRY(ctx, hipStreamSynchronize(ctx->stream));
        ctx->have_timing = false;
        return nmi_key_unpack(0, h_best_index, h_best_score);
    }

    rc = enqueue_grid_mask(ctx, render_stack, nullptr, S, 0, S, warp_stack, warp_masks, Wn, 0, ctx->d_mask_counts, ctx->d_mask_tables,
                           ctx->d_mask_redo, ctx->d_mask_redo_state, d_ratings, nullptr, true);
    if (rc != NMI_OK) return rc;
    unsigned long long key = 0;
    rc = fetch_key(ctx, &key);
    if (rc != NMI_OK) return rc;
    if (d_ratings) NMI_HIP_TRY(ctx, hipStreamSynchronize(ctx->stream));
    return nmi_key_unpack(key, h_best_index, h_best_score);
}

int nmi_last_mask_counts(nmi_ctx *ctx, int32_t *h_counts, int32_t n)
{
    if (!ctx || !h_counts || n < 0 || n > ctx->mask_count_n) return NMI_ERR_INVALID_ARGUMENT;
    if (n == 0) return NMI_OK;
    DeviceGuard guard(ctx->device);
    NMI_HIP_TRY(ctx, hipMemcpyAsync(h_counts, ctx->d_mask_counts, (size_t)n * sizeof(int32_t), hipMemcpyDeviceToHost, ctx->stream));
    NMI_HIP_TRY(ctx, hipStreamSynchronize(ctx->stream));
    return NMI_OK;
}

}
```

### orbslam2_nmi_amd/csrc/nmi_capi_pipeline.cpp

```cpp
#include "nmi_covered.h"
#include "nmi_color.h"
#include "nmi_ctx.h"
#include "nmi_intake.h"
#include "nmi_mask_bits.h"
#include "nmi_masked.h"
#include "nmi_reduce.h"
#include "nmi_undistort.h"

using namespace nmi_internal;

extern "C" {

}

struct LevelSettings {
    bool masked = false, covered = false;
    const uint8_t *d_frame_mask = nullptr;
    FrameIntake intake;
};

struct nmi_level {
    nmi_ctx *ctx = nullptr;
    int S = 0, Wn = 0, size = 1;
    int s_offset = 0, S_total = 0, w_offset = 0, Wn_total = 0;
    uint8_t *d_renders = nullptr, *d_warps = nullptr;
    uint32_t *d_zbuf = nullptr;
    void *d_packed = nullptr;
    nmi::MeshWork mesh;
    MapKind kind = MapKind::points;
    bool fused_points = false;
    uint32_t *d_kept = nullptr, *d_kept_count = nullptr;
    uint32_t replay = 0;
    float *d_mvps = nullptr, *h_mvps = nullptr, *d_coeffs = nullptr, *h_coeffs = nullptr;
    int *d_order = nullptr;
    float *d_ratings = nullptr;
    unsigned long long *d_key = nullptr, *h_key = nullptr;
    unsigned int *d_done = nullptr;
    uint32_t *d_epoch = nullptr;
    unsigned long long *d_pix_blocks = nullptr;
    int pix = 0;
    hipStream_t side = nullptr;
    hipEvent_t ev_fork = nullptr, ev_join = nullptr;
    hipGraph_t graph = nullptr;
    hipGraphExec_t exec = nullptr;
    const float *d_xyz = nullptr, *d_attr = nullptr;
    int64_t n_points = 0;
    const nmi_texture *tex = nullptr;
    const uint8_t *d_frame = nullptr;
    nmi::GridArgs args{};
    float *hd_mvps = nullptr, *hd_coeffs = nullptr;
    int workgroups = 0;
    size_t pix_blocks_bytes = 0;
    LevelSettings set;
    uint8_t *d_masks = nullptr;
    int32_t *d_counts = nullptr;
    float *d_tables = nullptr;
    int32_t *d_redo = nullptr;
    uint32_t *d_redo_state = nullptr;
    uint8_t *d_rmasks = nullptr;
    int32_t *d_cover_counts = nullptr;
    uint8_t *d_ud = nullptr, *d_ud_mask = nullptr, *d_small = nullptr;
};

extern "C" {

int nmi_level_destroy(nmi_level *lv)
{
    if (!lv) return NMI_OK;
    DeviceGuard guard(lv->ctx->device);
    (void)hipStreamSynchronize(lv->ctx->stream);
    if (lv->exec) (void)hipGraphExecDestroy(lv->exec);
    if (lv->graph) (void)hipGraphDestroy(lv->graph);
    void *dev[] = {lv->d_kept, lv->d_kept_count, lv->d_packed, lv->d_renders, lv->d_warps, lv->d_zbuf, lv->d_mvps, lv->d_coeffs, lv->d_order, lv->d_key, lv->d_done, lv->d_ratings, lv->d_epoch, lv->d_pix_blocks,
                   lv->d_masks, lv->d_counts, lv->d_tables, lv->d_redo, lv->d_redo_state, lv->d_rmasks, lv->d_cover_counts, lv->d_ud, lv->d_ud_mask, lv->d_small};
    for (void *q : dev)
        if (q) (void)hipFree(q);
    void *host[] = {lv->h_mvps, lv->h_coeffs, lv->h_key};
    for (void *q : host)
        if (q) (void)hipHostFree(q);
    if (lv->ev_fork) (void)hipEventDestroy(lv->ev_fork);
    if (lv->ev_join) (void)hipEventDestroy(lv->ev_join);
    if (lv->side) (void)hipStreamDestroy(lv->side);
    mesh_work_free(&lv->mesh);
    delete lv;
    return NMI_OK;
}

}

struct LevelNeeds {
    bool mode;
    bool masks;
    bool cover;
    bool ud;
    bool ud_mask;
    bool small;
};

static LevelNeeds level_needs(const LevelSettings &s)
{
    const bool mode = s.masked || s.covered;
    return {mode, s.masked, s.covered, s.intake.own_frame(), s.intake.distorted && mode, s.intake.reduced() && s.intake.distorted};
}

struct LevelBuffer {
    void **slot;
    size_t bytes, zeroed;
    bool needed;
};

static std::vector<LevelBuffer> level_buffers(nmi_level *lv, const LevelSettings &s)
{
    const LevelNeeds n = level_needs(s);
    const size_t npix = (size_t)lv->ctx->npix, S = (size_t)lv->S, Wn = (size_t)lv->Wn, cells = S * Wn * sizeof(int32_t);
    return {{(void **)&lv->d_masks, npix * Wn, npix * Wn, n.mode},
            {(void **)&lv->d_redo, cells, 0, n.mode},
            {(void **)&lv->d_redo_state, 2 * sizeof(uint32_t), 2 * sizeof(uint32_t), n.mode},
            {(void **)&lv->d_counts, 3 * Wn * sizeof(int32_t), Wn * sizeof(int32_t), n.masks},
            {(void **)&lv->d_tables, Wn * (npix + 1) * sizeof(float), 0, n.masks},
            {(void **)&lv->d_rmasks, npix * S, npix * S, n.cover},
            {(void **)&lv->d_cover_counts, cells, cells, n.cover},
            {(void **)&lv->d_ud, npix, 0, n.ud},
            {(void **)&lv->d_ud_mask, npix, 0, n.ud_mask},
            {(void **)&lv->d_small, npix, 0, n.small}};
}

static int level_capture(nmi_level *lv)
{
    nmi_ctx *ctx = lv->ctx;
    const nmi_params &p = ctx->params;
    const int S = lv->S, Wn = lv->Wn;
    const int64_t total = (int64_t)S * Wn;
    const nmi_texture *tex = lv->tex;
    const bool mesh = lv->kind != MapKind::points;
    const float *d_xyz = lv->d_xyz, *d_attr = lv->d_attr, *d_red = lv->d_attr;
    const int64_t n_points = lv->n_points;
    float *hd_mvps = lv->hd_mvps, *hd_coeffs = lv->hd_coeffs;
    FirstError ok;
    const LevelSettings &set = lv->set;
    const FrameIntake &in = set.intake;
    const bool masked = set.masked, covered = set.covered;
    uint8_t *ud_mask = level_needs(set).ud_mask ? lv->d_ud_mask : nullptr;
    const uint8_t *d_frame = in.own_frame() ? lv->d_ud : lv->d_frame;
    const uint8_t *d_frame_mask = in.distorted ? ud_mask : set.d_frame_mask;
    nmi::GridArgs a = lv->args;
    const int cap = ctx->workgroups > 0 ? ctx->workgroups : ctx->compute_units;
    lv->pix = choose_pix(ctx, a, total, cap);
    if (lv->pix) {
        const size_t bytes = nmi::pix_block_bytes((int)total, lv->pix);
        if (bytes > lv->pix_blocks_bytes) {
            if (lv->d_pix_blocks) ok(hipFree(lv->d_pix_blocks));
            lv->d_pix_blocks = nullptr;
            lv->pix_blocks_bytes = 0;
            ok(hipMalloc((void **)&lv->d_pix_blocks, bytes));
            if (ok.e == hipSuccess) ok(hipMemset(lv->d_pix_blocks, 0, bytes));
            if (ok.e == hipSuccess) lv->pix_blocks_bytes = bytes;
        }
        if (ok.e == hipSuccess && lv->args.epoch == 0 && next_split_epoch(ctx, &lv->args.epoch) != NMI_OK) ok.e = hipErrorOutOfMemory;
        if (ok.e == hipSuccess && ensure_pix_timeouts(ctx) != NMI_OK) ok.e = hipErrorOutOfMemory;
        if (ok.e == hipSuccess) ok(hipStreamSynchronize(ctx->stream));
        a.epoch = lv->args.epoch;
        a.blocks = lv->d_pix_blocks;
        a.order = nullptr;
    }
    const int workgroups = lv->workgroups;
    nmi::GridArgs ma = a;
    ma.phase_mask = lv->pix ? 3 | (ctx->phase_mask & 512) : 3;
    const MaskSearch ms = mask_search_args(ma, lv->d_masks, covered ? lv->d_rmasks : nullptr, covered ? lv->d_cover_counts : lv->d_counts,
                                           lv->d_tables, lv->d_redo, lv->d_redo_state);
    uint8_t *cover = covered ? lv->d_rmasks : nullptr;
    int32_t *d_prev = lv->d_counts + Wn, *d_changed = lv->d_counts + 2 * Wn;
    hipGraph_t graph = nullptr;
    hipGraphExec_t exec = nullptr;
    hipStream_t st = ctx->stream;
    if (ok.e == hipSuccess && ok(hipStreamBeginCapture(st, hipStreamCaptureModeThreadLocal))) {
        ok(nmi::launch_level_prep(hd_mvps, lv->d_mvps, S * 16 + nmi::kLevelMvpExtra, hd_coeffs, lv->d_coeffs, Wn * 9, lv->d_key, lv->d_zbuf,
                                  (mesh || lv->fused_points) ? 0 : nmi::render_zbuf_words(S, p.width, p.height, lv->size), st,
                                  lv->d_epoch, lv->fused_points ? lv->d_packed : nullptr, n_points,
                                  lv->fused_points ? hd_mvps + (size_t)S * 16 : nullptr, lv->d_kept, lv->d_kept_count));
        ok(launch_intake(in, lv->d_frame, in.frame_pitch, set.d_frame_mask, lv->d_small, lv->d_ud, ud_mask, p.width, p.height, st));
        const bool fused = mesh ? (nmi::level_front_eligible(d_frame, lv->d_warps, p.width, S) && n_points > 0) : lv->fused_points;
        if (!fused || masked || covered) {
            ok(hipEventRecord(lv->ev_fork, st));
            ok(hipStreamWaitEvent(lv->side, lv->ev_fork, 0));
            if (!fused) ok(nmi::launch_warp(d_frame, lv->d_coeffs, lv->d_warps, p.width, p.height, Wn, lv->side));
            if (masked) {
                ok(nmi::launch_warp_masks(d_frame_mask, lv->d_coeffs, lv->d_masks, p.width, p.height, Wn, lv->side));
                ok(nmi::launch_level_mask_counts(lv->d_masks, Wn, ctx->npix, lv->d_counts, d_prev, d_changed, lv->side));
                ok(nmi::launch_level_mask_tables(lv->d_counts, d_changed, Wn, ctx->npix, lv->d_tables, lv->side));
            }
            if (covered) ok(nmi::launch_warp_masks(d_frame_mask, lv->d_coeffs, lv->d_masks, p.width, p.height, Wn, lv->side));
            ok(hipEventRecord(lv->ev_join, lv->side));
        }
        if (mesh)
            ok(nmi::launch_render_mesh(d_xyz, mesh_shading(lv->kind, d_attr, tex), n_points, lv->d_mvps, S, lv->mesh, S,
                                       (int)(ctx->tile_queue_limit < 511 ? ctx->tile_queue_limit : 511), ctx->clip_queue_limit, lv->d_renders,
                                       p.width, p.height, st, fused ? d_frame : nullptr, lv->d_coeffs, lv->d_warps, Wn, cover));
        else if (fused)
            ok(nmi::launch_level_front_points(lv->d_packed, n_points, lv->d_mvps, S, lv->d_zbuf, lv->d_epoch, lv->d_renders, p.width, p.height,
                                              lv->size, d_frame, lv->d_coeffs, lv->d_warps, Wn, st, lv->d_kept, lv->d_kept_count, ctx->compute_units,
                                              cover));
        else
            ok(nmi::launch_render_points(d_xyz, d_red, n_points, lv->d_mvps, S, lv->d_zbuf, lv->d_renders, p.width, p.height, lv->size, st,
                                         false, cover));
        if (!fused || masked || covered) ok(hipStreamWaitEvent(st, lv->ev_join, 0));
        if (masked || covered)
            ok(launch_mask_search(ms, lv->pix, lv->pix ? pix_owner_share(ctx, lv->pix) : 0.0, workgroups, true, false, lv->d_epoch,
                                  ctx->d_pix_timeouts, st));
        else if (lv->pix)
            ok(nmi::launch_pix(a, lv->pix, pix_owner_share(ctx, lv->pix), true, lv->d_epoch, ctx->d_pix_timeouts, st));
        else
            ok(nmi::launch_grid(a, workgroups, true, st));
        hipError_t ec = hipStreamEndCapture(st, &graph);
        ok(ec);
    }
    if (ok.e == hipSuccess) ok(hipGraphInstantiate(&exec, graph, nullptr, nullptr, 0));
    if (ok.e != hipSuccess) {
        if (exec) (void)hipGraphExecDestroy(exec);
        if (graph) (void)hipGraphDestroy(graph);
        return hip_fail(ctx, ok.e, "nmi_level (graph capture)");
    }
    if (lv->exec) (void)hipGraphExecDestroy(lv->exec);
    if (lv->graph) (void)hipGraphDestroy(lv->graph);
    lv->graph = graph;
    lv->exec = exec;
    return NMI_OK;
}

static int level_apply(nmi_level *lv, const LevelSettings &next, const char *what, bool all_tables = false)
{
    nmi_ctx *ctx = lv->ctx;
    ctx->detail.clear();
    if (lv->S == 0 || lv->Wn == 0) {
        lv->set = next;
        return NMI_OK;
    }
    DeviceGuard guard(ctx->device);
    NMI_HIP_TRY(ctx, hipStreamSynchronize(ctx->stream));
    FirstError ok;
    std::vector<void **> fresh;
    for (const LevelBuffer &b : level_buffers(lv, next)) {
        if (!b.needed || *b.slot || ok.e != hipSuccess) continue;
        if (ok(hipMalloc(b.slot, b.bytes))) fresh.push_back(b.slot);
        if (ok.e == hipSuccess && b.zeroed) ok(hipMemset(*b.slot, 0, b.zeroed));
    }
    if (ok.e == hipSuccess && all_tables) ok(hipMemset(lv->d_counts + lv->Wn, 0xFF, (size_t)lv->Wn * sizeof(int32_t)));
    int rc = ok.e == hipSuccess ? NMI_OK : hip_fail(ctx, ok.e, what);
    const LevelSettings was = lv->set;
    if (rc == NMI_OK) {
        lv->set = next;
        rc = level_capture(lv);
    }
    if (rc != NMI_OK) {
        lv->set = was;
        for (void **slot : fresh) {
            (void)hipFree(*slot);
            *slot = nullptr;
        }
        return rc;
    }
    for (const LevelBuffer &b : level_buffers(lv, lv->set))
        if (!b.needed && *b.slot) {
            (void)hipFree(*b.slot);
            *b.slot = nullptr;
        }
    return NMI_OK;
}

struct LevelBlock {
    int32_t S, s_offset, S_total, Wn, w_offset, Wn_total;
};

static int level_create(nmi_ctx *ctx, MapKind kind, const float *d_xyz, const float *d_attr, int64_t n_points, const nmi_texture *tex,
                        const uint8_t *d_frame, const LevelBlock &blk, float point_size, nmi_level **out)
{
    const bool mesh = kind != MapKind::points;
    const float *d_red = d_attr;
    const int32_t S = blk.S, Wn = blk.Wn;
    if (!ctx || !out || !d_frame || S < 0 || Wn < 0 || n_points < 0 || (n_points > 0 && (!d_xyz || !d_attr)))
        return NMI_ERR_INVALID_ARGUMENT;
    if (blk.S_total <= 0 || blk.Wn_total <= 0 || blk.s_offset < 0 || blk.w_offset < 0 || blk.s_offset + S > blk.S_total ||
        blk.w_offset + Wn > blk.Wn_total)
        return NMI_ERR_INVALID_ARGUMENT;
    if ((int64_t)blk.S_total * blk.Wn_total >= 0x7FFFFFFFll) return NMI_ERR_UNSUPPORTED;
    if (kind == MapKind::textured_mesh ? (!tex || tex->ctx != ctx) : tex != nullptr) return NMI_ERR_INVALID_ARGUMENT;
    int size = 1;
    if (!mesh && point_sprite_size(point_size, &size) != NMI_OK) return NMI_ERR_INVALID_ARGUMENT;
    if (!ctx->params.use_bg) return NMI_ERR_UNSUPPORTED;
    *out = nullptr;
    ctx->detail.clear();
    DeviceGuard guard(ctx->device);
    nmi_level *lv = new (std::nothrow) nmi_level;
    if (!lv) return NMI_ERR_INVALID_ARGUMENT;
    lv->ctx = ctx;
    lv->kind = kind;
    lv->S = S;
    lv->Wn = Wn;
    lv->s_offset = blk.s_offset;
    lv->S_total = blk.S_total;
    lv->w_offset = blk.w_offset;
    lv->Wn_total = blk.Wn_total;
    if (S == 0 || Wn == 0) {
        hipError_t e0 = hipMalloc((void **)&lv->d_key, sizeof(unsigned long long));
        if (e0 == hipSuccess) e0 = hipMemset(lv->d_key, 0, sizeof(unsigned long long));
        if (e0 != hipSuccess) {
            const int rc = hip_fail(ctx, e0, "nmi_level_create (empty block)");
            nmi_level_destroy(lv);
            return rc;
        }
        *out = lv;
        return NMI_OK;
    }
    lv->size = size;
    const nmi_params &p = ctx->params;
    const size_t npix = (size_t)ctx->npix;
    const int64_t total = (int64_t)S * Wn;
    FirstError ok;
    ok(hipMalloc((void **)&lv->d_renders, npix * S));
    ok(hipMalloc((void **)&lv->d_warps, npix * Wn));
    if (mesh) {
        if (mesh_work_alloc(ctx, S, &lv->mesh) != NMI_OK) ok.e = hipErrorOutOfMemory;
        if (ok.e == hipSuccess && ensure_mesh_pairs(ctx, &lv->mesh, n_points) != NMI_OK) ok.e = hipErrorOutOfMemory;
        ok(hipMalloc((void **)&lv->d_epoch, sizeof(uint32_t)));
        if (ok.e == hipSuccess) ok(hipMemsetAsync(lv->d_epoch, 0, sizeof(uint32_t), ctx->stream));
    } else {
        lv->fused_points = nmi::level_front_eligible(d_frame, nullptr, p.width, S) && n_points > 0 && nmi::level_points_double_buffered(p.width, lv->size);
        const size_t words = lv->fused_points ? 2 * nmi::level_zbuf_pair_words(S, p.width, p.height, lv->size)
                                              : nmi::render_zbuf_words(S, p.width, p.height, lv->size);
        ok(hipMalloc((void **)&lv->d_zbuf, words * sizeof(uint32_t)));
        ok(hipMalloc((void **)&lv->d_epoch, sizeof(uint32_t)));
        ok(hipMalloc(&lv->d_packed, nmi::cloud_pack_bytes(n_points, nullptr) + 16));
        if (ok.e == hipSuccess) ok(hipMemsetAsync(lv->d_zbuf, 0xFF, words * sizeof(uint32_t), ctx->stream));
        if (ok.e == hipSuccess) ok(hipMemsetAsync(lv->d_epoch, 0, sizeof(uint32_t), ctx->stream));
        if (ok.e == hipSuccess) ok(nmi::launch_cloud_pack(d_xyz, d_red, n_points, lv->d_packed, ctx->stream));
        if (lv->fused_points) {
            ok(hipMalloc((void **)&lv->d_kept, (size_t)(2 * ((n_points + 63) / 64) + 1) * sizeof(uint32_t)));
            ok(hipMalloc((void **)&lv->d_kept_count, 2 * sizeof(uint32_t)));
            if (ok.e == hipSuccess) ok(hipMemsetAsync(lv->d_kept_count, 0, 2 * sizeof(uint32_t), ctx->stream));
        }
    }
    ok(hipMalloc((void **)&lv->d_mvps, ((size_t)S * 16 + nmi::kLevelMvpExtra) * sizeof(float)));
    ok(hipMalloc((void **)&lv->d_coeffs, (size_t)Wn * 9 * sizeof(float)));
    ok(hipMalloc((void **)&lv->d_order, (size_t)total * sizeof(int)));
    ok(hipMalloc((void **)&lv->d_ratings, (size_t)total * sizeof(float)));
    ok(hipMalloc((void **)&lv->d_key, sizeof(unsigned long long)));
    ok(hipMalloc((void **)&lv->d_done, sizeof(unsigned int)));
    ok(hipHostMalloc((void **)&lv->h_mvps, ((size_t)S * 16 + nmi::kLevelMvpExtra) * sizeof(float), hipHostMallocMapped | hipHostMallocCoherent));
    ok(hipHostMalloc((void **)&lv->h_coeffs, (size_t)Wn * 9 * sizeof(float), hipHostMallocMapped | hipHostMallocCoherent));
    ok(hipHostMalloc((void **)&lv->h_key, sizeof(unsigned long long), hipHostMallocMapped | hipHostMallocCoherent));
    ok(hipStreamCreateWithFlags(&lv->side, hipStreamNonBlocking));
    ok(hipEventCreateWithFlags(&lv->ev_fork, hipEventDisableTiming));
    ok(hipEventCreateWithFlags(&lv->ev_join, hipEventDisableTiming));
    int *order = ok.e == hipSuccess ? new (std::nothrow) int[(size_t)total] : nullptr;
    if (ok.e != hipSuccess || !order) {
        const int rc = ok.e != hipSuccess ? hip_fail(ctx, ok.e, "nmi_level_create") : NMI_ERR_INVALID_ARGUMENT;
        nmi_level_destroy(lv);
        return rc;
    }
    build_order(S, Wn, order);
    ok(hipMemcpy(lv->d_order, order, (size_t)total * sizeof(int), hipMemcpyHostToDevice));
    delete[] order;
    ok(hipMemset(lv->d_done, 0, sizeof(unsigned int)));
    memset(lv->h_mvps, 0, ((size_t)S * 16 + nmi::kLevelMvpExtra) * sizeof(float));
    memset(lv->h_coeffs, 0, (size_t)Wn * 9 * sizeof(float));
    ok(hipDeviceSynchronize());

    nmi::GridArgs a{};
    a.render_stack = lv->d_renders;
    a.warp_stack = lv->d_warps;
    a.S_local = S;
    a.Wn = Wn;
    a.s_offset = blk.s_offset;
    a.S_total = blk.S_total;
    a.w_offset = blk.w_offset;
    nmi::set_geometry(a, p.width, p.height, lv->d_renders, lv->d_warps, p.render_bottom_up != 0);
    a.shift = ctx->shift;
    a.mode = p.mode;
    a.table = ctx->table;
    a.order = lv->d_order;
    a.ratings = lv->d_ratings;
    a.key = lv->d_key;
    a.reset_key = nullptr;
    a.done = lv->d_done;
    float *hd_mvps = nullptr, *hd_coeffs = nullptr;
    unsigned long long *hd_key = nullptr;
    if (ok.e == hipSuccess) {
        ok(hipHostGetDevicePointer((void **)&hd_mvps, lv->h_mvps, 0));
        ok(hipHostGetDevicePointer((void **)&hd_coeffs, lv->h_coeffs, 0));
        ok(hipHostGetDevicePointer((void **)&hd_key, lv->h_key, 0));
    }
    a.out_key = hd_key;
    a.hist_variant = 3;
    a.phase_mask = 3;
    const int cap = ctx->workgroups > 0 ? ctx->workgroups : ctx->compute_units;
    const int workgroups = (int)(total < cap ? total : cap);
    lv->d_xyz = d_xyz;
    lv->d_attr = d_attr;
    lv->n_points = n_points;
    lv->tex = tex;
    lv->d_frame = d_frame;
    lv->args = a;
    lv->hd_mvps = hd_mvps;
    lv->hd_coeffs = hd_coeffs;
    lv->workgroups = workgroups;
    if (ok.e == hipSuccess) {
        const int rc = level_capture(lv);
        if (rc != NMI_OK) {
            nmi_level_destroy(lv);
            return rc;
        }
    }
    if (ok.e != hipSuccess) {
        const int rc = hip_fail(ctx, ok.e, "nmi_level_create");
        nmi_level_destroy(lv);
        return rc;
    }
    *out = lv;
    return NMI_OK;
}

extern "C" {

int nmi_level_create(nmi_ctx *ctx, const float *d_xyz, const float *d_red, int64_t n_points, const uint8_t *d_frame, int32_t S,
                     int32_t Wn, float point_size, nmi_level **out)
{
    if (S <= 0 || Wn <= 0) return NMI_ERR_INVALID_ARGUMENT;
    return level_create(ctx, MapKind::points, d_xyz, d_red, n_points, nullptr, d_frame, LevelBlock{S, 0, S, Wn, 0, Wn}, point_size, out);
}

int nmi_level_create_mesh(nmi_ctx *ctx, const float *d_xyz, const float *d_uv, int64_t n_triangles, const nmi_texture *tex,
                          const uint8_t *d_frame, int32_t S, int32_t Wn, nmi_level **out)
{
    if (!tex || S <= 0 || Wn <= 0) return NMI_ERR_INVALID_ARGUMENT;
    return level_create(ctx, MapKind::textured_mesh, d_xyz, d_uv, n_triangles, tex, d_frame, LevelBlock{S, 0, S, Wn, 0, Wn}, 1.0f, out);
}

int nmi_level_create_mesh_colored(nmi_ctx *ctx, const float *d_xyz, const float *d_red, int64_t n_triangles, const uint8_t *d_frame, int32_t S,
                                  int32_t Wn, nmi_level **out)
{
    if (S <= 0 || Wn <= 0) return NMI_ERR_INVALID_ARGUMENT;
    return level_create(ctx, MapKind::colored_mesh, d_xyz, d_red, n_triangles, nullptr, d_frame, LevelBlock{S, 0, S, Wn, 0, Wn}, 1.0f, out);
}

int nmi_level_create_block(nmi_ctx *ctx, const float *d_xyz, const float *d_red, int64_t n_points, const uint8_t *d_frame, int32_t S_local,
                           int32_t s_offset, int32_t S_total, int32_t Wn_local, int32_t w_offset, int32_t Wn_total, float point_size,
                           nmi_level **out)
{
    return level_create(ctx, MapKind::points, d_xyz, d_red, n_points, nullptr, d_frame,
                        LevelBlock{S_local, s_offset, S_total, Wn_local, w_offset, Wn_total}, point_size, out);
}

int nmi_level_create_mesh_block(nmi_ctx *ctx, const float *d_xyz, const float *d_uv, int64_t n_triangles, const nmi_texture *tex,
                                const uint8_t *d_frame, int32_t S_local, int32_t s_offset, int32_t S_total, int32_t Wn_local,
                                int32_t w_offset, int32_t Wn_total, nmi_level **out)
{
    if (!tex) return NMI_ERR_INVALID_ARGUMENT;
    return level_create(ctx, MapKind::textured_mesh, d_xyz, d_uv, n_triangles, tex, d_frame,
                        LevelBlock{S_local, s_offset, S_total, Wn_local, w_offset, Wn_total}, 1.0f, out);
}

int nmi_level_create_mesh_colored_block(nmi_ctx *ctx, const float *d_xyz, const float *d_red, int64_t n_triangles, const uint8_t *d_frame,
                                        int32_t S_local, int32_t s_offset, int32_t S_total, int32_t Wn_local, int32_t w_offset,
                                        int32_t Wn_total, nmi_level **out)
{
    return level_create(ctx, MapKind::colored_mesh, d_xyz, d_red, n_triangles, nullptr, d_frame,
                        LevelBlock{S_local, s_offset, S_total, Wn_local, w_offset, Wn_total}, 1.0f, out);
}

}

static int level_launch(nmi_level *lv, const float *h_mvps, const double *h_forward)
{
    nmi_ctx *ctx = lv->ctx;
    std::vector<float> coeffs((size_t)lv->Wn * 9);
    for (int w = 0; w < lv->Wn; ++w)
        if (warp_inverse_coeffs(h_forward + (size_t)w * 9, coeffs.data() + (size_t)w * 9) != NMI_OK) return NMI_ERR_INVALID_ARGUMENT;
    memcpy(lv->h_mvps, h_mvps, (size_t)lv->S * 16 * sizeof(float));
    nmi::level_views_bound(h_mvps, lv->S, lv->h_mvps + (size_t)lv->S * 16);
    static const bool no_bound = getenv("NMI_LEVEL_NO_BOUND") != nullptr;
    if (no_bound) memset(lv->h_mvps + (size_t)lv->S * 16, 0, 24 * sizeof(float));
    const uint32_t parity = ++lv->replay & 1u;
    memcpy(lv->h_mvps + (size_t)lv->S * 16 + 24, &parity, sizeof parity);
    memcpy(lv->h_coeffs, coeffs.data(), coeffs.size() * sizeof(float));
    constexpr unsigned long long kPending = ~0ull;
    __atomic_store_n(lv->h_key, kPending, __ATOMIC_RELEASE);
    const hipError_t le = hipGraphLaunch(lv->exec, ctx->stream);
    if (le != hipSuccess) {
        --lv->replay;
        return hip_fail(ctx, le, "hipGraphLaunch");
    }
    return NMI_OK;
}

int nmi_internal::level_enqueue(nmi_level *lv, const float *h_mvps, const double *h_forward, const unsigned long long **d_key)
{
    if (!lv || !d_key) return NMI_ERR_INVALID_ARGUMENT;
    *d_key = lv->d_key;
    if (lv->S == 0 || lv->Wn == 0) return NMI_OK;
    if (!h_mvps || !h_forward) return NMI_ERR_INVALID_ARGUMENT;
    lv->ctx->detail.clear();
    return level_launch(lv, h_mvps, h_forward);
}

nmi_ctx *nmi_internal::level_ctx(nmi_level *lv) { return lv ? lv->ctx : nullptr; }

extern "C" {

int nmi_level_run(nmi_level *lv, const float *h_mvps, const double *h_forward, int64_t *h_best_index, float *h_best_score)
{
    if (!lv) return NMI_ERR_INVALID_ARGUMENT;
    if (lv->S == 0 || lv->Wn == 0) return nmi_key_unpack(0, h_best_index, h_best_score);
    if (!h_mvps || !h_forward) return NMI_ERR_INVALID_ARGUMENT;
    nmi_ctx *ctx = lv->ctx;
    ctx->detail.clear();
    DeviceGuard guard(ctx->device);
    constexpr unsigned long long kPending = ~0ull;
    const int lrc = level_launch(lv, h_mvps, h_forward);
    if (lrc != NMI_OK) return lrc;
    unsigned long long key = kPending;
    for (uint64_t spin = 0; key == kPending; ++spin) {
        key = __atomic_load_n(lv->h_key, __ATOMIC_ACQUIRE);
        if (key == kPending && (spin & 0xFFFF) == 0xFFFF) {
            const hipError_t q = hipStreamQuery(ctx->stream);
            if (q == hipSuccess) {
                key = __atomic_load_n(lv->h_key, __ATOMIC_ACQUIRE);
                break;
            }
            if (q != hipErrorNotReady) return hip_fail(ctx, q, "hipStreamQuery");
        }
    }
    if (key == kPending) return NMI_ERR_HIP;
    return nmi_key_unpack(key, h_best_index, h_best_score);
}

int nmi_level_copy_outputs(nmi_level *lv, uint8_t *h_renders, uint8_t *h_warps, float *h_ratings)
{
    if (!lv) return NMI_ERR_INVALID_ARGUMENT;
    nmi_ctx *ctx = lv->ctx;
    if (lv->S == 0 || lv->Wn == 0) return NMI_OK;
    DeviceGuard guard(ctx->device);
    NMI_HIP_TRY(ctx, hipStreamSynchronize(ctx->stream));
    const size_t npix = (size_t)ctx->npix;
    if (h_renders) NMI_HIP_TRY(ctx, hipMemcpy(h_renders, lv->d_renders, npix * lv->S, hipMemcpyDeviceToHost));
    if (h_warps) NMI_HIP_TRY(ctx, hipMemcpy(h_warps, lv->d_warps, npix * lv->Wn, hipMemcpyDeviceToHost));
    if (h_ratings) NMI_HIP_TRY(ctx, hipMemcpy(h_ratings, lv->d_ratings, (size_t)lv->S * lv->Wn * sizeof(float), hipMemcpyDeviceToHost));
    return NMI_OK;
}

int nmi_level_set_masks(nmi_level *lv, int32_t enabled, const uint8_t *d_frame_mask)
{
    if (!lv || (enabled != 0 && enabled != 1) || (!enabled && d_frame_mask)) return NMI_ERR_INVALID_ARGUMENT;
    if (lv->set.covered) return NMI_ERR_INVALID_ARGUMENT;
    LevelSettings next = lv->set;
    next.masked = enabled != 0;
    next.d_frame_mask = d_frame_mask;
    return level_apply(lv, next, "nmi_level_set_masks", next.masked);
}

int nmi_level_copy_masks(nmi_level *lv, uint8_t *h_warp_masks, int32_t *h_counts)
{
    if (!lv || !lv->set.masked) return NMI_ERR_INVALID_ARGUMENT;
    if (lv->S == 0 || lv->Wn == 0) return NMI_OK;
    nmi_ctx *ctx = lv->ctx;
    DeviceGuard guard(ctx->device);
    NMI_HIP_TRY(ctx, hipStreamSynchronize(ctx->stream));
    if (h_warp_masks) NMI_HIP_TRY(ctx, hipMemcpy(h_warp_masks, lv->d_masks, (size_t)ctx->npix * lv->Wn, hipMemcpyDeviceToHost));
    if (h_counts) NMI_HIP_TRY(ctx, hipMemcpy(h_counts, lv->d_counts, (size_t)lv->Wn * sizeof(int32_t), hipMemcpyDeviceToHost));
    return NMI_OK;
}

int nmi_level_set_coverage(nmi_level *lv, int32_t enabled, const uint8_t *d_frame_mask)
{
    if (!lv || (enabled != 0 && enabled != 1) || (!enabled && d_frame_mask)) return NMI_ERR_INVALID_ARGUMENT;
// ... 107 lines not shown
    nmi_ctx *ctx = st->ctx;
    const size_t npix = (size_t)ctx->npix, cells = (size_t)st->max_S * st->max_Wn;
    auto alloc = [](void *p, size_t bytes) {
        void **pp = (void **)p;
        return *pp ? hipSuccess : hipMalloc(pp, bytes);
    };
    for (int b = 0; b < 2; ++b) {
        NMI_HIP_TRY(ctx, alloc(&st->d_fmask[b], npix));
        NMI_HIP_TRY(ctx, alloc(&st->d_wmasks[b], npix * st->max_Wn));
    }
    for (int i = 0; i < st->depth; ++i) NMI_HIP_TRY(ctx, alloc(&st->slots[i].d_counts, cells * sizeof(int32_t)));
    NMI_HIP_TRY(ctx, alloc(&st->d_redo, cells * sizeof(int32_t)));
    if (!st->d_redo_state) {
        NMI_HIP_TRY(ctx, alloc(&st->d_redo_state, 2 * sizeof(uint32_t)));
        NMI_HIP_TRY(ctx, hipMemsetAsync(st->d_redo_state, 0, 2 * sizeof(uint32_t), ctx->stream));
    }
    if (kind == kMasked) {
        for (int b = 0; b < 2; ++b) {
            NMI_HIP_TRY(ctx, alloc(&st->d_wcounts[b], (size_t)st->max_Wn * sizeof(int32_t)));
            NMI_HIP_TRY(ctx, alloc(&st->d_wtables[b], (size_t)st->max_Wn * (npix + 1) * sizeof(float)));
        }
    }
    if (kind == kCovered) {
        for (int i = 0; i < st->depth; ++i) NMI_HIP_TRY(ctx, alloc(&st->slots[i].d_bits, nmi::mask_bit_bytes(ctx->npix) * st->max_S));
        NMI_HIP_TRY(ctx, alloc(&st->d_rmasks, npix * st->max_S));
    }
    return NMI_OK;
}

}

extern "C" {

int nmi_stream_destroy(nmi_stream *st)
{
    if (!st) return NMI_OK;
    DeviceGuard guard(st->ctx->device);
    (void)hipStreamSynchronize(st->ctx->stream);
    if (st->copy) (void)hipStreamSynchronize(st->copy);
    for (int i = 0; st->slots && i < st->depth; ++i) {
        nmi_stream::Slot &s = st->slots[i];
        if (s.d_renders) (void)hipFree(s.d_renders);
        if (s.d_ratings) (void)hipFree(s.d_ratings);
        if (s.d_key) (void)hipFree(s.d_key);
        if (s.h_key) (void)hipHostFree(s.h_key);
        if (s.copied) (void)hipEventDestroy(s.copied);
        if (s.done) (void)hipEventDestroy(s.done);
        if (s.d_counts) (void)hipFree(s.d_counts);
        if (s.d_bits) (void)hipFree(s.d_bits);
    }
    delete[] st->slots;
    for (int b = 0; b < 2; ++b) {
        if (st->d_frame[b]) (void)hipFree(st->d_frame[b]);
        if (st->d_warps[b]) (void)hipFree(st->d_warps[b]);
        if (st->warps_free[b]) (void)hipEventDestroy(st->warps_free[b]);
        if (st->d_fmask[b]) (void)hipFree(st->d_fmask[b]);
        if (st->d_wmasks[b]) (void)hipFree(st->d_wmasks[b]);
        if (st->d_wcounts[b]) (void)hipFree(st->d_wcounts[b]);
        if (st->d_wtables[b]) (void)hipFree(st->d_wtables[b]);
        if (st->d_ud[b]) (void)hipFree(st->d_ud[b]);
        if (st->d_ud_mask[b]) (void)hipFree(st->d_ud_mask[b]);
        if (st->d_color[b]) (void)hipFree(st->d_color[b]);
    }
    if (st->d_rmasks) (void)hipFree(st->d_rmasks);
    if (st->d_redo) (void)hipFree(st->d_redo);
    if (st->d_redo_state) (void)hipFree(st->d_redo_state);
    if (st->frame_copied) (void)hipEventDestroy(st->frame_copied);
    if (st->copy) (void)hipStreamDestroy(st->copy);
    delete st;
    return NMI_OK;
}

int nmi_stream_create(nmi_ctx *ctx, int32_t max_S, int32_t max_Wn, int32_t depth, nmi_stream **out)
{
    if (!ctx || !out || max_S <= 0 || max_Wn <= 0 || depth < 2 || depth > 64) return NMI_ERR_INVALID_ARGUMENT;
    *out = nullptr;
    DeviceGuard guard(ctx->device);
    nmi_stream *st = new (std::nothrow) nmi_stream;
    if (!st) return NMI_ERR_INVALID_ARGUMENT;
    st->ctx = ctx;
    st->depth = depth;
    st->max_S = max_S;
    st->max_Wn = max_Wn;
    st->slots = new (std::nothrow) nmi_stream::Slot[depth];
    const size_t npix = (size_t)ctx->npix;
    FirstError ok;
    ok(hipStreamCreateWithFlags(&st->copy, hipStreamNonBlocking));
    for (int i = 0; st->slots && i < depth && ok.e == hipSuccess; ++i) {
        nmi_stream::Slot &s = st->slots[i];
        ok(hipMalloc((void **)&s.d_renders, npix * max_S));
        ok(hipMalloc((void **)&s.d_key, 2 * sizeof(unsigned long long)));
        ok(hipHostMalloc((void **)&s.h_key, sizeof(unsigned long long), hipHostMallocDefault));
        ok(hipEventCreateWithFlags(&s.copied, hipEventDisableTiming));
        ok(hipEventCreateWithFlags(&s.done, hipEventDisableTiming));
    }
    for (int b = 0; b < 2 && ok.e == hipSuccess; ++b) {
        ok(hipMalloc((void **)&st->d_frame[b], npix));
        ok(hipMalloc((void **)&st->d_warps[b], npix * max_Wn));
        ok(hipEventCreateWithFlags(&st->warps_free[b], hipEventDisableTiming));
    }
    ok(hipEventCreateWithFlags(&st->frame_copied, hipEventDisableTiming));
    if (!st->slots || ok.e != hipSuccess) {
        const int rc = st->slots ? hip_fail(ctx, ok.e, "nmi_stream_create") : NMI_ERR_INVALID_ARGUMENT;
        nmi_stream_destroy(st);
        return rc;
    }
    *out = st;
    return NMI_OK;
}

int nmi_stream_submit(nmi_stream *st, const uint8_t *h_render_stack, int32_t S, const uint8_t *h_frame,
                      const double *h_forward, int32_t Wn, int64_t *ticket)
{
    if (S <= 0) return NMI_ERR_INVALID_ARGUMENT;
    return nmi_stream_submit_block(st, h_render_stack, S, 0, S, h_frame, h_forward, Wn, 0, h_frame ? Wn : (st ? st->cur_Wn : 0), nullptr, ticket);
}

}

static int stream_submit(nmi_stream *st, int kind, const uint8_t *h_render_stack, const uint8_t *h_bits, int32_t S, int32_t s_offset,
                         int32_t S_total, const uint8_t *h_frame, const uint8_t *h_frame_mask, const double *h_forward, int32_t Wn,
                         int32_t w_offset, int32_t Wn_total, void *nccl_comm, int64_t *ticket)
{
    if (!st || !ticket || S < 0 || S > st->max_S || (S > 0 && !h_render_stack)) return NMI_ERR_INVALID_ARGUMENT;
    if (h_frame && (!h_forward || Wn <= 0 || Wn > st->max_Wn)) return NMI_ERR_INVALID_ARGUMENT;
    if (!h_frame && !st->have_warps && !(S == 0 && nccl_comm)) return NMI_ERR_INVALID_ARGUMENT;
    if (h_frame_mask && !h_frame) return NMI_ERR_INVALID_ARGUMENT;
    if (kind == kCovered && S > 0 && !h_bits) return NMI_ERR_INVALID_ARGUMENT;
    if (kind != kPlain && !h_frame && st->have_warps && !st->masks_ok[st->warp_buf]) return NMI_ERR_INVALID_ARGUMENT;
    const int32_t Wn_block = h_frame ? Wn : st->cur_Wn;
    if (s_offset < 0 || w_offset < 0 || s_offset + S > S_total || w_offset + Wn_block > Wn_total) return NMI_ERR_INVALID_ARGUMENT;
    if ((int64_t)S_total * Wn_total >= 0x7FFFFFFFll) return NMI_ERR_UNSUPPORTED;
    nmi_ctx *ctx = st->ctx;
    ctx->detail.clear();
    DeviceGuard guard(ctx->device);
    const int64_t t = st->next_ticket;
    nmi_stream::Slot &s = st->slots[t % st->depth];
    if (!s.waited) return NMI_ERR_NOT_READY;
    const size_t npix = (size_t)ctx->npix;
    if (kind != kPlain) {
        const int rc = stream_alloc_masks(st, kind);
        if (rc != NMI_OK) return rc;
    }
    const FrameIntake in = st->intake;
    const bool undistort = h_frame && in.distorted, colored = h_frame && in.colored;
    const int32_t factor = in.frame_factor;
    const int64_t dense_row = (int64_t)factor * ctx->params.width * frame_bytes_per_pixel(in.frame_format);
    const size_t color_rows = (size_t)factor * ctx->params.height, color_need = (size_t)dense_row * color_rows;
    for (int b = 0; (undistort || colored) && b < 2; ++b) {
        if (!st->d_ud[b]) NMI_HIP_TRY(ctx, hipMalloc((void **)&st->d_ud[b], npix));
        if (undistort && kind != kPlain && !st->d_ud_mask[b]) NMI_HIP_TRY(ctx, hipMalloc((void **)&st->d_ud_mask[b], npix));
    }
    if (colored && st->color_bytes < color_need) {
        NMI_HIP_TRY(ctx, hipStreamSynchronize(st->copy));
        NMI_HIP_TRY(ctx, hipStreamSynchronize(ctx->stream));
        st->color_bytes = 0;
        for (int b = 0; b < 2; ++b) {
            if (st->d_color[b]) (void)hipFree(st->d_color[b]);
            st->d_color[b] = nullptr;
        }
        for (int b = 0; b < 2; ++b) NMI_HIP_TRY(ctx, hipMalloc((void **)&st->d_color[b], color_need));
        st->color_bytes = color_need;
    }

    if (S > 0) NMI_HIP_TRY(ctx, hipMemcpyAsync(s.d_renders, h_render_stack, npix * S, hipMemcpyHostToDevice, st->copy));
    if (kind == kCovered && S > 0)
// ... 207 lines not shown
```

### orbslam2_nmi_amd/csrc/nmi_ctx.h

```cpp
#pragma once
#include <hip/hip_runtime.h>
#include <math.h>
#include <stdio.h>
#include <string.h>

#include <new>
#include <string>
#include <vector>

#include "nmi_hip.h"
#include "nmi_covered.h"
#include "nmi_kernels.h"
#include "nmi_masked.h"

struct StagingRing {
    static constexpr int kSlots = 4;
    float *h[kSlots] = {};
    float *d[kSlots] = {};
    hipEvent_t ev[kSlots] = {};
    size_t cap = 0;
    unsigned uses = 0;
};

struct nmi_ctx {
    nmi_params params{};
    int device = 0;
    int compute_units = 0;
    int npix = 0;
    int shift = 0;
    hipStream_t own_stream = nullptr;
    hipStream_t stream = nullptr;
    float *table = nullptr;
    unsigned long long *d_keys = nullptr;
    unsigned long long *h_key = nullptr;
    unsigned int *d_done = nullptr;
    nmi::Mailbox *mailbox = nullptr;
    unsigned int seq = 0;
    int slot = 0;
    int last_slot = 0;
    int last_parts = 0;
    int pix_owner_bias = 49152;
    int last_pix = 0;
    uint32_t *d_pix_timeouts = nullptr;
    uint32_t last_epoch = 0;
    bool allow_unchecked_split = false;
    uint32_t split_timeouts = 0;
    uint32_t split_cooldown = 0;
    uint32_t split_backoff = kSplitBackoffMin;
    uint32_t split_cooldown_epoch = 0;
    static constexpr uint32_t kSplitBackoffMin = 16, kSplitBackoffMax = 4096;
    int result_path = 1;
    bool posted = false;
    float *d_pair_rating = nullptr;
    unsigned long long *d_reduced_key = nullptr;
    unsigned long long *score_mailbox = nullptr;
    unsigned int pair_seq = 0;
    int wait_mode = 0;
    struct OrderEntry {
        int S = -1, Wn = -1;
        int *d = nullptr, *h = nullptr;
        int64_t cap = 0;
        uint64_t last_use = 0;
    };
    static constexpr int kOrderCache = 16;
    OrderEntry orders[kOrderCache];
    uint64_t order_clock = 0;
    int xcd_tiling = 1;
    nmi::SplitSlab *d_slabs = nullptr;
    int slab_cap = 0;
    unsigned long long *d_blocks = nullptr;
    uint32_t split_epoch = 0;
    uint32_t *h_split_error = nullptr, *d_split_error = nullptr;
    size_t blocks_bytes = 0;
    unsigned long long *d_pix_blocks = nullptr;
    size_t pix_blocks_bytes = 0;
    const uint8_t **h_pair_table = nullptr, **d_pair_table = nullptr;
    float *d_pair_scores = nullptr;
    int pairs_cap = 0;
    const uint8_t *const *pair_renders = nullptr, *const *pair_warps = nullptr;
    const uint8_t *const *pair_renders_host = nullptr, *const *pair_warps_host = nullptr;
    int split_pixels = -1;
    nmi::LevelPlan *d_plan = nullptr;
    unsigned long long *level_post = nullptr;
    uint32_t level_seq = 0;
    uint32_t level_seen = 0;
    bool few_hint = false;
    int content_path = -1;
    int fewlevels_bins = 4096;
    uint8_t *d_rank_stacks = nullptr;
    size_t rank_bytes = 0;
    int last_few = 0;
    unsigned long long *dbg_stamps = nullptr;
    int stamp_candidate = 0;
    int split_mode = -1;
    uint32_t *d_zbuf = nullptr;
    int64_t zbuf_cap = 0;
    nmi::MeshWork mesh;
    int mesh_views = 0;
    unsigned long long tile_queue_limit = 4ull << 20;
    unsigned long long clip_queue_limit = ~0ull;
    StagingRing mvp_ring;
    uint32_t *d_scratch = nullptr;
    int scratch_workgroups = 0;
    static constexpr int kWarpRing = 4;
    float *d_warp_coeffs[kWarpRing] = {};
    float *h_warp_coeffs[kWarpRing] = {};
    hipEvent_t warp_ev[kWarpRing] = {};
    int warp_coeffs_cap = 0;
    unsigned warp_uses = 0;
    int32_t *d_mask_counts = nullptr;
    float *d_mask_tables = nullptr;
    int mask_warps_cap = 0;
    int mask_count_n = 0;
    int32_t *d_mask_redo = nullptr;
    uint32_t *d_mask_redo_state = nullptr;
    int64_t mask_redo_cap = 0;
    int32_t *d_cover_counts = nullptr;
    int64_t cover_cap = 0;
    int64_t cover_count_n = 0;
    hipEvent_t ev_start = nullptr, ev_stop = nullptr;
    int hist_variant = 3;
    int phase_mask = 3;
    int workgroups = 0;
    bool profiling = false;
    bool have_timing = false;
    std::string detail;
};

struct nmi_texture {
    nmi_ctx *ctx = nullptr;
    float *d_luma = nullptr;
    int levels = 0;
    int w[16] = {}, h[16] = {};
    long long off[16] = {};
};

namespace nmi_internal {

int mesh_work_alloc(nmi_ctx *ctx, int S, nmi::MeshWork *w);
void mesh_work_free(nmi::MeshWork *w);
int ensure_mesh_work(nmi_ctx *ctx, int S);
int ensure_mesh_pairs(nmi_ctx *ctx, nmi::MeshWork *w, long long n_triangles);
int warp_inverse_coeffs(const double *forward , float *coeffs );
int point_sprite_size(float point_size, int *size);
int level_enqueue(nmi_level *lv, const float *h_mvps, const double *h_forward, const unsigned long long **d_key);
nmi_ctx *level_ctx(nmi_level *lv);
int rccl_allreduce_key(nmi_ctx *ctx, const unsigned long long *d_send, unsigned long long *d_recv, void *nccl_comm);

int hip_fail(nmi_ctx *ctx, hipError_t e, const char *what);
void build_order(int S, int Wn, int *order);
int ensure_order(nmi_ctx *ctx, int S, int Wn, const int **d_order);
int choose_pix(const nmi_ctx *ctx, const nmi::GridArgs &a, int64_t total, int cap);
double pix_owner_share(const nmi_ctx *ctx, int pix);
int next_split_epoch(nmi_ctx *ctx, uint32_t *epoch);
int ensure_pix_timeouts(nmi_ctx *ctx);
int ensure_pix_blocks(nmi_ctx *ctx, size_t bytes);
int enqueue_grid(nmi_ctx *ctx, const uint8_t *render_stack, int S_local, int s_offset, int S_total, const uint8_t *warp_stack, int Wn,
                 float *d_ratings, unsigned long long *out_key, bool post, uint32_t *dbg_joint, uint32_t *dbg_h1, uint32_t *dbg_h2,
                 float *dbg_sums, int w_offset = 0, bool post_score = false);
struct MaskSearch {
    bool covered;
    nmi::MaskedGridArgs masked;
    nmi::CoveredGridArgs cover;
};
MaskSearch mask_search_args(const nmi::GridArgs &a, const uint8_t *warp_masks, const uint8_t *render_masks, int32_t *counts,
                            const float *tables, int32_t *redo, uint32_t *redo_state);
hipError_t launch_mask_search(const MaskSearch &ms, int pix, double owner_share, int workgroups, bool use_bg, bool exact,
                              const uint32_t *replay, uint32_t *healed, hipStream_t stream);
int ensure_mask_redo(nmi_ctx *ctx, int64_t total);
int enqueue_grid_mask(nmi_ctx *ctx, const uint8_t *render_stack, const uint8_t *render_masks, int S_local, int s_offset, int S_total,
                      const uint8_t *warp_stack, const uint8_t *warp_masks, int Wn, int w_offset, int32_t *counts, const float *tables,
                      int32_t *redo, uint32_t *redo_state, float *d_ratings, unsigned long long *out_key, bool post);
int wait_word(nmi_ctx *ctx, const volatile unsigned long long *word, unsigned long long mask, unsigned long long want,
              unsigned long long *out);
int stage_floats(nmi_ctx *ctx, StagingRing &ring, const float *h_src, size_t n, float **d_out);
int fetch_key(nmi_ctx *ctx, unsigned long long *key);
bool split_timed_out(nmi_ctx *ctx);
bool split_launch_failed(nmi_ctx *ctx, int parts, uint32_t epoch);
int search_block(nmi_ctx *ctx, const uint8_t *render_stack, int32_t S_local, int32_t s_offset, int32_t S_total, const uint8_t *warp_stack,
                 int32_t Wn_local, int32_t w_offset, int32_t Wn_total, float *d_ratings, uint64_t *d_key, uint64_t *h_key,
                 bool caller_checks);
enum class MapKind { points, textured_mesh, colored_mesh };
int render_points_impl(nmi_ctx *ctx, const float *d_xyz, const float *d_red, int64_t n_points, const float *h_mvps, int32_t S,
                       float point_size, uint8_t *d_render_stack, uint8_t *cover);
int render_mesh_impl(nmi_ctx *ctx, MapKind kind, const float *d_xyz, const float *d_attr, int64_t n_triangles, const nmi_texture *tex,
                     const float *h_mvps, int32_t S, uint8_t *d_render_stack, uint8_t *cover);
nmi::MeshShading mesh_shading(MapKind kind, const float *d_attr, const nmi_texture *tex);
int check_grid_args(nmi_ctx *ctx, const uint8_t *render_stack, int S_local, int s_offset, int S_total, const uint8_t *warp_stack,
                    int Wn);

#define NMI_HIP_TRY(ctx, call)                                  \
    do {                                                        \
        hipError_t e_ = (call);                                 \
        if (e_ != hipSuccess) return nmi_internal::hip_fail((ctx), e_, #call); \
    } while (0)

struct FirstError {
    hipError_t e = hipSuccess;
    bool operator()(hipError_t r)
    {
        if (e == hipSuccess) e = r;
        return r == hipSuccess;
    }
};

struct DeviceGuard {
    int prev = -1;
    bool active = false;
    explicit DeviceGuard(int dev)
    {
        if (hipGetDevice(&prev) == hipSuccess && prev != dev) active = hipSetDevice(dev) == hipSuccess;
    }
    ~DeviceGuard()
    {
        if (active) (void)hipSetDevice(prev);
    }
};

}
```

### orbslam2_nmi_amd/csrc/nmi_grid_device.h

```cpp
#pragma once
#include <hip/hip_runtime.h>
#include <stdint.h>

#include "nmi_kernels.h"
#include "nmi_device.h"

namespace nmi {

namespace {

constexpr int kBlock = NMI_BLOCK_THREADS;
constexpr int kWaves = kBlock / 64;
constexpr int kBins = 256;
constexpr int kWords = kBins * kBins / 2;
constexpr int kRowStride = 129;
constexpr int kJointWords = kBins * kRowStride;
constexpr int kOvfCap = 1024;
constexpr int kRowsPerWave = kBins / kWaves;
constexpr int kLdsTable = 4096;
constexpr int kSide = 8;


struct Lds {
    uint32_t joint[kJointWords];
// ... 260 lines not shown
                const int cn = min(ch + kStep, last);
                const uint4 wn = ldw(cn), rn = ldr(cn);
                add_chunk<BG, SHIFTED, HIST, true>(lds, par, rc, wc, a.shift, try_flat);
                wc = wn;
                rc = rn;
            }
        }
        if (ROWS && row_rem > 0) {
            const int x0 = a.chunks_per_row << 4, n = a.height * row_rem;
            for (int t = tid; t < n; t += NT) {
                const int y = t / row_rem, x = x0 + t - y * row_rem;
                const int ry = a.flip ? (a.height - 1 - y) : y;
                uint32_t d1 = render[ry * a.width + x], d2 = warped[y * a.width + x];
                if (HIST == 2) {
                    if (BG || (d1 != 0 && d2 != 0)) {
                        if (SHIFTED) {
                            d1 >>= a.shift;
                            d2 >>= a.shift;
                        }
                        (void)__hip_atomic_fetch_add(&lds.joint[joint_word(d1, d2)], joint_inc(d2), __ATOMIC_RELAXED, __HIP_MEMORY_SCOPE_WORKGROUP);
                    }
                } else {
                    add_pixel<BG, SHIFTED>(lds, par, d1, d2, a.shift);
                }
            }
        }
    } else {
        for (int pos = tid; pos < a.npix; pos += NT) {
            const int y = pos / a.width;
            const int x = pos - y * a.width;
            const int ry = a.flip ? (a.height - 1 - y) : y;
            if (HIST == 2) {
                uint32_t d1 = render[ry * a.width + x], d2 = warped[pos];
                if (BG || (d1 != 0 && d2 != 0)) {
                    if (SHIFTED) {
                        d1 >>= a.shift;
                        d2 >>= a.shift;
                    }
                    (void)__hip_atomic_fetch_add(&lds.joint[joint_word(d1, d2)], joint_inc(d2), __ATOMIC_RELAXED,
                                                 __HIP_MEMORY_SCOPE_WORKGROUP);
                }
            } else {
                add_pixel<BG, SHIFTED>(lds, par, render[ry * a.width + x], warped[pos], a.shift);
            }
        }
    }
}

__device__ __forceinline__ float term(const float *__restrict__ table, uint32_t c)
{
    return c ? table[c] : 0.0f;
}
__device__ __forceinline__ float term_lds(const Lds &lds, const float *__restrict__ table, uint32_t c)
{
    float t = lds.table[c < (uint32_t)kLdsTable ? c : 0u];
    if (__builtin_expect(c >= (uint32_t)kLdsTable, 0)) t = table[c];
    return t;
}

static_assert(kWaves == 16 && (kWaves * kRowStride) % 32 == 16, "rows kWaves apart must fall on opposite halves of the 32 banks");
__device__ __forceinline__ int decode_row(int wave, int pass, int r) { return wave + 4 * kWaves * pass + kWaves * r; }
__device__ __forceinline__ bool in_decode_pass(uint32_t d1, int wave, int pass)
{
    return (d1 % (uint32_t)kWaves) == (uint32_t)wave && (d1 / (uint32_t)(4 * kWaves)) == (uint32_t)pass;
}
__device__ __forceinline__ uint32_t decode_word(int d1, int i, int k) { return (uint32_t)(d1 * kRowStride + i + 16 * k); }

__device__ __forceinline__ void apply_wraps(const Lds &lds, int par, uint32_t novf, uint32_t word, uint32_t &lo,
                                            uint32_t &hi)
{
    for (uint32_t e = 0; e < novf; ++e) {
        const uint32_t ev = lds.ovf[par][e];
        if ((ev >> 1) == word) {
            if (ev & 1u) {
                hi += 65536u;
            } else {
                lo += 65536u;
                hi -= 1u;
            }
        }
    }
}

template <bool ZERO0 = false>
__device__ __forceinline__ void decode_phase(Lds &lds, int par, const GridArgs &a, int wave, int lane)
{
    const uint32_t novf = lds.ovf_n[par] < (uint32_t)kOvfCap ? lds.ovf_n[par] : (uint32_t)kOvfCap;
    const bool side_any = lds.side_key[par][0] != 0u;
    uint32_t wave_total = 0;
    const int i = lane & 15, r = lane >> 4;
    uint32_t col_lo[8], col_hi[8];
#pragma unroll
    for (int k = 0; k < 8; ++k) col_lo[k] = col_hi[k] = 0;
#pragma unroll 1
    for (int pass = 0; pass < kRowsPerWave / 4; ++pass) {
        const int d1 = decode_row(wave, pass, r);
        const uint32_t a0 = decode_word(d1, i, 0);
        uint32_t lo[8], hi[8];
#pragma unroll
        for (int k = 0; k < 8; ++k) {
            const uint32_t idx = a0 + 16 * k;
            const uint32_t wd = lds.joint[idx];
            lds.joint[idx] = 0;
            lo[k] = wd & 0xFFFFu;
            hi[k] = wd >> 16;
        }
        if (__builtin_expect(novf != 0, 0)) {
#pragma unroll
            for (int k = 0; k < 8; ++k) apply_wraps(lds, par, novf, a0 + 16 * k, lo[k], hi[k]);
        }
        if (__builtin_expect(side_any, 0)) {
            for (int e = 0; e < kSide; ++e) {
                const uint32_t key1 = __builtin_amdgcn_readfirstlane(lds.side_key[par][e]);
                if (key1 == 0u) break;
                const uint32_t sd1 = (key1 - 1u) >> 8, sd2 = (key1 - 1u) & 0xFFu;
                if (!in_decode_pass(sd1, wave, pass)) continue;
                const uint32_t sword = joint_word(sd1, sd2);
                const uint32_t cnt = lds.side_cnt[par][e];
#pragma unroll
                for (int k = 0; k < 8; ++k) {
                    if (a0 + 16 * k == sword) {
                        if (sd2 & 128u)
                            hi[k] += cnt;
                        else
                            lo[k] += cnt;
                    }
                }
            }
        }
        uint32_t rsum = 0, cmax = 0;
        if (ZERO0) {
            uint32_t raw = 0;
#pragma unroll
            for (int k = 0; k < 8; ++k) raw += lo[k] + hi[k];
            wave_total += row_sum_16(raw);
            if (i == 0) lo[0] = 0;
            if (d1 == 0) {
#pragma unroll
                for (int k = 0; k < 8; ++k) lo[k] = hi[k] = 0;
            }
        }
        float tl[8], th[8];
#pragma unroll
        for (int k = 0; k < 8; ++k) {
            col_lo[k] += lo[k];
            col_hi[k] += hi[k];
            rsum += lo[k] + hi[k];
            cmax = max(cmax, max(lo[k], hi[k]));
            tl[k] = lds.table[lo[k] & (kLdsTable - 1)];
            th[k] = lds.table[hi[k] & (kLdsTable - 1)];
        }
        if (__builtin_expect(cmax >= (uint32_t)kLdsTable, 0)) {
#pragma unroll
            for (int k = 0; k < 8; ++k) {
                if (lo[k] >= (uint32_t)kLdsTable) tl[k] = a.table[lo[k]];
                if (hi[k] >= (uint32_t)kLdsTable) th[k] = a.table[hi[k]];
            }
        }
        rsum = row_sum_16(rsum);
        if (!ZERO0) wave_total += rsum;
        const float x = row_tree_16(lane_tree_16(tl, th));
        if (i == 0) {
            lds.hist_render[d1] = rsum;
            lds.joint_row_sums[d1] = x;
        }
        if (a.dbg_joint) {
            uint32_t *row = a.dbg_joint + d1 * kBins;
#pragma unroll
            for (int k = 0; k < 8; ++k) {
                const int q = i + 16 * k;
                row[q] = lo[k];
                row[q + 128] = hi[k];
            }
        }
    }
#pragma unroll
    for (int k = 0; k < 8; ++k) {
        const int q = i + 16 * k;
        atomicAdd(&lds.hist_warped[q], col_lo[k]);
        atomicAdd(&lds.hist_warped[q + 128], col_hi[k]);
    }
    if (i == 0) atomicAdd(&lds.total[par], wave_total);
}

__device__ __forceinline__ void final_phase(Lds &lds, const GridArgs &a, int lane, int p, int w, int s,
                                            unsigned long long &prev_key)
{
    const int i = lane & 15, r = lane >> 4;
    float lo[8], hi[8];
    const uint32_t *h = r == 0 ? lds.hist_render : lds.hist_warped;
    uint32_t cl[8], ch[8];
#pragma unroll
    for (int k = 0; k < 8; ++k) {
        cl[k] = r < 2 ? h[i + 16 * k] : 0u;
        ch[k] = r < 2 ? h[i + 16 * k + 128] : 0u;
    }
#pragma unroll
    for (int k = 0; k < 8; ++k) {
        lo[k] = a.table[cl[k]];
        hi[k] = a.table[ch[k]];
    }
    if ((w == 0 || s == 0) && a.plan) {
        uint32_t m = 0;
#pragma unroll
        for (int k = 0; k < 8; ++k) m |= (cl[k] != 0u ? 1u << k : 0u) | (ch[k] != 0u ? 0x100u << k : 0u);
        if (lane < 32 && m) __hip_atomic_fetch_or(const_cast<uint32_t *>(&a.plan->seen[lane]), m, __ATOMIC_RELAXED, __HIP_MEMORY_SCOPE_AGENT);
    }
    if (r == 2) {
#pragma unroll
        for (int k = 0; k < 8; ++k) {
            lo[k] = lds.joint_row_sums[i + 16 * k];
            hi[k] = lds.joint_row_sums[i + 16 * k + 128];
        }
    }
    const float x = row_tree_16(lane_tree_16(lo, hi));
    const float a1 = __shfl(x, 0, 64), a2 = __shfl(x, 16, 64), a3 = __shfl(x, 32, 64);
    if (a.dbg_h1 && lane < 64) {
        for (int t = lane; t < kBins; t += 64) {
            a.dbg_h1[t] = lds.hist_render[t];
            if (a.dbg_h2) a.dbg_h2[t] = lds.hist_warped[t];
        }
    }
    if (lane == 0) commit_score(a, p, w, s, a1, a2, a3, prev_key);
}

__device__ __forceinline__ void finish_search(const GridArgs &a, int lane, unsigned long long prev_key, uint32_t expected)
{
    LevelPlan *plan = const_cast<LevelPlan *>(a.plan);
    uint32_t arrived = 0;
    if (lane == 0) {
        const unsigned int one = prev_key == ~0ull ? 2u : 1u;
        arrived = __hip_atomic_fetch_add(a.done, one, __ATOMIC_RELAXED, __HIP_MEMORY_SCOPE_AGENT);
    }
    if (__builtin_amdgcn_readfirstlane(arrived) != expected - 1) return;
    unsigned long long final_key = 0;
    uint32_t bits = 0;
    unsigned long long *post = nullptr;
    uint32_t state = 0, max_joint = 0;
    if (lane == 0) final_key = __hip_atomic_load(a.key, __ATOMIC_RELAXED, __HIP_MEMORY_SCOPE_AGENT);
    if (plan && lane < 32) bits = __hip_atomic_exchange(&plan->seen[lane], 0u, __ATOMIC_RELAXED, __HIP_MEMORY_SCOPE_AGENT);
    if (plan && lane == 0) post = plan->seen_post, state = plan->seen_state, max_joint = plan->seen_max_joint;
    if (lane == 0) {
        __hip_atomic_store(a.done, 0u, __ATOMIC_RELAXED, __HIP_MEMORY_SCOPE_AGENT);
        if (a.out_key) __hip_atomic_store(a.out_key, final_key, __ATOMIC_RELAXED, __HIP_MEMORY_SCOPE_SYSTEM);
        if (a.mailbox)
            __hip_atomic_store(&a.mailbox->word, final_key | ((unsigned long long)(a.seq & 1u) << 63), __ATOMIC_RELAXED, __HIP_MEMORY_SCOPE_SYSTEM);
    }
    if (plan) {
        const uint32_t n = row_sum_16((uint32_t)__popc(bits));
        const uint32_t nw = (uint32_t)__shfl((int)n, 16, 64);
        const uint32_t few = (n > 0u && nw > 0u && n * nw <= max_joint) ? 1u : 0u;
        if (lane == 0 && post && few != state) {
            plan->seen_state = few;
            const uint32_t stamp = 0x80000000u | (uint32_t)wall_clock64();
            __hip_atomic_store(post, ((unsigned long long)stamp << 32) | ((unsigned long long)n << 16) | nw, __ATOMIC_RELAXED, __HIP_MEMORY_SCOPE_SYSTEM);
        }
    }
}

template <bool SHIFTED, bool BG = true, bool ROWS = false>
__device__ __forceinline__ void exact_candidate(Lds &lds, const GridArgs &a, int tid, int p, unsigned long long &prev_key)
{
    const int lane = tid & 63, wave = tid >> 6;
    const int w = p / a.S_local, s = p - w * a.S_local;
    __syncthreads();
    histogram_phase<true, SHIFTED, 1, kBlock, true, ROWS>(lds, 0, a, a.render_stack + (size_t)s * a.npix, a.warp_stack + (size_t)w * a.npix, tid, 0,
                                                          ROWS ? a.height * a.chunks_per_row : a.npix >> 4);
    __syncthreads();
    decode_phase<!BG>(lds, 0, a, wave, lane);
    __syncthreads();
    if (wave == 0) {
        final_phase(lds, a, lane, p, w, s, prev_key);
        for (int t = lane; t < kBins; t += 64) lds.hist_warped[t] = 0;
        if (lane == 0) lds.ovf_n[0] = lds.total[0] = 0;
        if (lane < kSide) lds.side_key[0][lane] = lds.side_cnt[0][lane] = 0;
    }
    __syncthreads();
}

}

}
```

### orbslam2_nmi_amd/csrc/nmi_kernels.h

```cpp
#pragma once
#include <hip/hip_runtime.h>
#include <stdint.h>

#define NMI_BLOCK_THREADS 1024
#define NMI_MODE_ENMI_ 0
#define NMI_MODE_SUC_ 1

namespace nmi {

struct Mailbox {
    unsigned long long word;
    unsigned long long pad;
};

struct LevelPlan {
    uint32_t use;
    uint32_t nr, nw;
    uint32_t copies;
    uint32_t ticket;
    uint32_t pad[3];
    uint32_t mask[2][8];
    uint8_t rank_r[256], rank_w[256];
    uint8_t level_r[256], level_w[256];
    uint32_t seen[32];
    uint32_t seen_state;
    uint32_t seen_max_joint;
    unsigned long long *seen_post;
};

constexpr uint32_t kSplitRing = 256;

struct GridArgs {
    const uint8_t *render_stack;
    const uint8_t *warp_stack;
    const uint8_t *const *pair_renders;
    const uint8_t *const *pair_warps;
    int S_local, Wn;
    int s_offset, S_total;
    int w_offset;
    int width, height, npix;
    int chunks_per_row;
    uint32_t cpr_magic;
    int vec_ok;
    int flip_base, flip_row;
    int shift;
    int mode;
    int flip;
    const float *table;
    union {
        uint32_t *scratch;
        const LevelPlan *plan;
    };
    const int *order;
    float *ratings;
    unsigned long long *key;
    unsigned long long *reset_key;
    unsigned long long *out_key;
    unsigned int *done;
    Mailbox *mailbox;
    unsigned int seq;
    unsigned long long *score_post;
    struct SplitSlab *slabs;
    unsigned long long *blocks;
    uint32_t epoch;
    uint32_t *split_error;
    unsigned long long *dbg_stamps;
    uint32_t *dbg_joint, *dbg_h1, *dbg_h2;
    float *dbg_sums;
    int hist_variant;
    int phase_mask;
};

inline void set_geometry(GridArgs &a, int width, int height, const void *render_stack, const void *warp_stack, bool render_bottom_up)
{
    a.width = width;
    a.height = height;
    a.npix = width * height;
    a.vec_ok = (width % 16 == 0) && width >= 32 && (((uintptr_t)render_stack | (uintptr_t)warp_stack) % 16 == 0);
    a.chunks_per_row = width >= 32 ? width / 16 : 1;
    a.cpr_magic = a.chunks_per_row > 1 ? (uint32_t)((0x100000000ull + a.chunks_per_row - 1) / a.chunks_per_row) : 0u;
    a.flip = render_bottom_up ? 1 : 0;
    a.flip_base = render_bottom_up ? (height - 1) * a.chunks_per_row : 0;
    a.flip_row = render_bottom_up ? -2 * a.chunks_per_row : 0;
}

hipError_t launch_table(float *table, int npix, hipStream_t stream);
hipError_t launch_grid(const GridArgs &a, int workgroups, bool use_bg, hipStream_t stream);
hipError_t launch_grid_gated(const GridArgs &a, int workgroups, bool use_bg, hipStream_t stream);
hipError_t launch_grid_rows(const GridArgs &a, int workgroups, bool use_bg, hipStream_t stream);
hipError_t launch_grid_stamped(const GridArgs &a, int workgroups, hipStream_t stream);
hipError_t set_stamped_experiment(int k, const uint32_t *cum);

hipError_t launch_levels(const uint8_t *render_stack, int S, const uint8_t *warp_stack, int Wn, int npix, int shift, LevelPlan *plan,
                         unsigned long long *post, uint32_t seq, uint32_t max_joint, bool commit, hipStream_t stream);
hipError_t launch_fewlevels(const GridArgs &a, uint8_t *rank_renders, uint8_t *rank_warps, int workgroups, bool use_bg,
                            hipStream_t stream);
int fewlevels_max_joint();
bool ablation_variants_built();

struct SplitSlab {
    unsigned long long row_sums[256];
    unsigned long long hist_render[256];
    unsigned long long hw_part[8][256];
};
hipError_t launch_split(const GridArgs &a, int parts, int pix_parts, int workgroups, bool use_bg, hipStream_t stream);
__host__ __device__ int split_workgroups(int candidates, int parts, int pix_parts);
inline size_t split_block_bytes_per_candidate(int pix_parts) { return (size_t)pix_parts * 256 * 128 * sizeof(unsigned long long); }
hipError_t launch_pix(const GridArgs &a, int pix_parts, double owner_share, bool use_bg, const uint32_t *replay, uint32_t *timeouts, hipStream_t stream);
size_t pix_block_bytes(int candidates, int pix_parts);
int pix_max_ranges();
int grid_kernel_lds_bytes();
size_t grid_kernel_scratch_bytes(int workgroups);
hipError_t launch_warp(const uint8_t *frame, const float *coeffs , uint8_t *out, int width,
                       int height, int Wn, hipStream_t stream);

struct MeshWork {
    unsigned long long *zbuf = nullptr;
    uint32_t *bins = nullptr;
    uint32_t *state = nullptr;
    void *clip_queue = nullptr;
    unsigned long long clip_cap = 0;
    unsigned long long *clip_state = nullptr;
    uint32_t *pairs = nullptr;
    uint32_t *pair_state = nullptr;
    unsigned long long pairs_cap = 0;
    int compute_units = 0;
};
size_t mesh_pairs_entries(long long ntri);
size_t mesh_zbuf_bytes(int S, int width, int height);
size_t mesh_bins_bytes(int S, int width, int height);
size_t mesh_state_bytes(int S, int width, int height);
size_t mesh_clip_item_bytes();
hipError_t launch_mesh_clear(const MeshWork &w, int S, int width, int height, hipStream_t stream);
struct MeshShading {
    bool textured;
    const float *attr;
    const float *luma = nullptr;
    int levels = 0;
    const int *lw = nullptr, *lh = nullptr;
    const long long *loff = nullptr;
};
hipError_t launch_render_mesh(const float *xyz, const MeshShading &shading, long long ntri, const float *mvps , int S, const MeshWork &w,
                              int layout_views , int bin_cap_limit,
                              unsigned long long clip_cap_limit, uint8_t *out, int width, int height, hipStream_t stream,
                              const uint8_t *warp_frame = nullptr, const float *warp_coeffs = nullptr, uint8_t *warp_out = nullptr, int Wn = 0,
                              uint8_t *cover = nullptr);
inline int zbuf_stride(int width, int size) { return size > 1 ? ((width + size - 1 + 3) & ~3) + 4 : width; }
size_t render_zbuf_words(int S, int width, int height, int size);
hipError_t launch_render_points(const float *xyz, const float *red, long long npoints, const float *mvps ,
                                int S, uint32_t *zbuf , uint8_t *out, int width, int height, int size, hipStream_t stream,
                                bool clear_first = true, uint8_t *cover = nullptr );
hipError_t sort_records_morton(const float *a, int na, int verts, const float *b, int nb, long long n, float *a_out, float *b_out,
                               hipStream_t stream);
size_t cloud_pack_bytes(long long npoints, size_t *boxes_offset);
hipError_t launch_cloud_pack(const float *xyz, const float *red, long long npoints, void *packed, hipStream_t stream);
bool level_front_eligible(const void *frame, const void *warps, int width, int S);
void level_views_bound(const float *mvps , int S, float out[24]);
constexpr int kLevelMvpExtra = 28;
bool level_points_double_buffered(int width, int size);
size_t level_zbuf_pair_words(int S, int width, int height, int size);
hipError_t launch_level_front_points(const void *packed, long long npoints, const float *mvps, int S, uint32_t *zbuf ,
                                     const uint32_t *epoch, uint8_t *out, int width, int height, int size, const uint8_t *frame,
                                     const float *coeffs, uint8_t *warps, int Wn, hipStream_t stream,
                                     const uint32_t *kept ,
                                     const uint32_t *kept_count , int compute_units,
                                     uint8_t *cover = nullptr );
hipError_t launch_level_prep(const float *h_mvps, float *d_mvps, int n_mvps, const float *h_coeffs, float *d_coeffs, int n_coeffs,
                             unsigned long long *key, uint32_t *zbuf, size_t nz, hipStream_t stream, uint32_t *epoch = nullptr,
                             const void *packed = nullptr, long long npoints = 0, const float *h_bound  = nullptr,
                             uint32_t *kept = nullptr, uint32_t *kept_count = nullptr);

}
// ... 1 lines not shown
```

### orbslam2_nmi_amd/csrc/nmi_kernels.hip

```cpp
#include <hip/hip_runtime.h>
#include <stdint.h>

#include "nmi_grid_device.h"

namespace nmi {

#if defined(NMI_GRID_KERNEL_GATED)
#define NMI_GRID_KERNEL_NAME nmi_grid_kernel_gated
#elif defined(NMI_GRID_KERNEL_STAMPED)
#define NMI_GRID_KERNEL_NAME nmi_grid_kernel_stamped
#elif defined(NMI_GRID_KERNEL_ROWS)
#define NMI_GRID_KERNEL_NAME nmi_grid_kernel_rows
#else
#define NMI_GRID_KERNEL_NAME nmi_grid_kernel
#endif
#ifdef NMI_GRID_KERNEL_STAMPED
#define NMI_GRID_STAMP(k)                                                                                         \
    do {                                                                                                          \
        if (a.dbg_stamps && tid == ((k) == 7 ? 64 : 0) && stamp_on) a.dbg_stamps[blockIdx.x * 8 + (k)] = wall_clock64(); \
    } while (0)
#else
#define NMI_GRID_STAMP(k) \
    do {                  \
    } while (0)
#endif
#ifndef NMI_WAVE_SLABS
#define NMI_WAVE_SLABS 1
#endif
#ifdef NMI_GRID_KERNEL_STAMPED
namespace {
__device__ uint32_t stamp_candidate = 0;
}
#endif
template <bool BG, bool SHIFTED, int HIST>
__global__ __launch_bounds__(NMI_BLOCK_THREADS) void NMI_GRID_KERNEL_NAME(GridArgs a)
{
    __shared__ Lds lds;
#ifdef NMI_GRID_KERNEL_GATED
    if (a.plan->use != 0u) return;
#endif
    const int tid = threadIdx.x;
    const int lane = tid & 63;
    const int wave = tid >> 6;
#ifdef NMI_GRID_KERNEL_STAMPED
    bool stamp_on = true;
    const int stamp_ordinal = slot_in_round(blockIdx.x, gridDim.x) + (int)stamp_candidate * (int)gridDim.x;
#endif
    NMI_GRID_STAMP(0);
    constexpr bool kOptimistic = HIST == 3;
    constexpr int kFirst = kOptimistic ? 2 : HIST;
#ifdef NMI_GRID_KERNEL_ROWS
    constexpr bool kRows = true;
#define NMI_ALL_CHUNKS (a.height * a.chunks_per_row)
#else
    constexpr bool kRows = false;
#define NMI_ALL_CHUNKS (a.npix >> 4)
#endif
    constexpr bool kZero0 = !BG && kOptimistic && !SHIFTED;
    constexpr bool kCountAll = BG || kZero0;
    constexpr bool kSlabs = NMI_WAVE_SLABS != 0 && kFirst == 2;

    if (blockIdx.x == 0 && tid == 0 && a.reset_key) *a.reset_key = 0ull;
    float tab[kLdsTable / kBlock];
#pragma unroll
    for (int k = 0; k < kLdsTable / kBlock; ++k) {
        const int c = tid + k * kBlock;
        tab[k] = a.table[c <= a.npix ? c : 0];
    }
    {
        uint4 *j4 = reinterpret_cast<uint4 *>(lds.joint);
        const uint4 z = {0, 0, 0, 0};
        for (int i = tid; i < kJointWords / 4; i += kBlock) j4[i] = z;
    }
    if (tid < kBins) lds.hist_warped[tid] = 0;
    if (tid < 2) lds.ovf_n[tid] = lds.total[tid] = 0;
    if (tid < 2 * kSide) (&lds.side_key[0][0])[tid] = (&lds.side_cnt[0][0])[tid] = 0;
    bool table_pending = true;
    int exact_from = -1;
    __syncthreads();
    NMI_GRID_STAMP(1);

    const int total = a.S_local * a.Wn;
    unsigned long long prev_key = 0;
    int par = 0;
    const int slot = slot_in_round(blockIdx.x, gridDim.x);
    int ordinal = slot;
    for (; ordinal < total; ordinal += gridDim.x, par ^= 1) {
        const int p = candidate_at(a, ordinal);
        const int w = p / a.S_local;
        const int s = p - w * a.S_local;
        const uint8_t *render = a.render_stack + (size_t)s * a.npix;
        const uint8_t *warped = a.warp_stack + (size_t)w * a.npix;
#ifdef NMI_GRID_KERNEL_STAMPED
        stamp_on = ordinal == stamp_ordinal;
#endif
        NMI_GRID_STAMP(7);

        if (a.phase_mask & 1) {
            if (a.phase_mask & 8) {
                if (wave < kWaves / 2) histogram_phase<kCountAll, SHIFTED, kFirst, kBlock / 2, true, kRows>(lds, par, a, render, warped, tid, 0, NMI_ALL_CHUNKS);
            } else
                histogram_phase<kCountAll, SHIFTED, kFirst, kBlock, true, kRows, kSlabs>(lds, par, a, render, warped, tid, 0, NMI_ALL_CHUNKS, ordinal != slot);
        }
        if (table_pending) {
#pragma unroll
            for (int k = 0; k < kLdsTable / kBlock; ++k) lds.table[tid + k * kBlock] = tab[k];
            table_pending = false;
        }
        NMI_GRID_STAMP(2);
#ifdef NMI_GRID_KERNEL_STAMPED
        if (a.dbg_stamps && lane == 0 && stamp_on) a.dbg_stamps[gridDim.x * 8 + blockIdx.x * 16 + wave] = wall_clock64();
#endif
        __syncthreads();
        NMI_GRID_STAMP(3);
        if (a.phase_mask & 2) decode_phase<kZero0>(lds, par, a, wave, lane);
        __syncthreads();
        NMI_GRID_STAMP(4);
        if (kOptimistic && (a.phase_mask & 3) == 3 && lds.total[par] != (uint32_t)a.npix) {
            exact_from = ordinal;
            break;
        }
        if (wave == 0) {
            if (a.phase_mask & 2) final_phase(lds, a, lane, p, w, s, prev_key);
            for (int t = lane; t < kBins; t += 64) lds.hist_warped[t] = 0;
            if (lane == 0) {
                lds.ovf_n[par] = 0;
                lds.total[par ^ 1] = 0;
            }
            if (lane < kSide) {
                int l = lane;
                asm volatile("" : "+v"(l));
                lds.side_key[par][l] = lds.side_cnt[par][l] = 0;
            }
        }
        NMI_GRID_STAMP(5);
    }

    if (kOptimistic && exact_from >= 0) {
        __syncthreads();
        if (tid < kBins) lds.hist_warped[tid] = 0;
        if (tid < 2) lds.total[tid] = lds.ovf_n[tid] = 0;
        if (tid < 2 * kSide) (&lds.side_key[0][0])[tid] = (&lds.side_cnt[0][0])[tid] = 0;
        __syncthreads();
        for (int o = exact_from; o < total; o += gridDim.x) exact_candidate<SHIFTED, !kZero0, kRows>(lds, a, tid, candidate_at(a, o), prev_key);
    }

    if (wave == 0 && !(a.phase_mask & 16)) {
        finish_search(a, lane, prev_key, gridDim.x);
    }
#ifdef NMI_GRID_KERNEL_STAMPED
    stamp_on = true;
#endif
    NMI_GRID_STAMP(6);
}

#if defined(NMI_GRID_KERNEL_ROWS)
hipError_t launch_grid_rows(const GridArgs &a, int workgroups, bool use_bg, hipStream_t stream)
{
    if (a.width < 32 || (a.hist_variant != 1 && a.hist_variant != 3)) return hipErrorInvalidValue;
    const dim3 grid(workgroups), block(kBlock);
    const bool exact_only = a.hist_variant == 1 || (!use_bg && a.shift != 0);
    if (exact_only) {
        if (use_bg) {
            if (a.shift != 0) hipLaunchKernelGGL((nmi_grid_kernel_rows<true, true, 1>), grid, block, 0, stream, a);
            else hipLaunchKernelGGL((nmi_grid_kernel_rows<true, false, 1>), grid, block, 0, stream, a);
        } else {
            if (a.shift != 0) hipLaunchKernelGGL((nmi_grid_kernel_rows<false, true, 1>), grid, block, 0, stream, a);
            else hipLaunchKernelGGL((nmi_grid_kernel_rows<false, false, 1>), grid, block, 0, stream, a);
        }
    } else if (a.shift != 0) {
        hipLaunchKernelGGL((nmi_grid_kernel_rows<true, true, 3>), grid, block, 0, stream, a);
    } else if (use_bg) {
        hipLaunchKernelGGL((nmi_grid_kernel_rows<true, false, 3>), grid, block, 0, stream, a);
    } else {
        hipLaunchKernelGGL((nmi_grid_kernel_rows<false, false, 3>), grid, block, 0, stream, a);
    }
    return hipGetLastError();
}
#elif defined(NMI_GRID_KERNEL_STAMPED)
hipError_t set_stamped_experiment(int k, const uint32_t *cum)
{
    const uint32_t kk = (uint32_t)k;
    hipError_t e = hipMemcpyToSymbol(HIP_SYMBOL(stamp_candidate), &kk, sizeof kk);
    if (e == hipSuccess && cum) {
        for (int r = 0; r < 2; ++r)
            for (int v = 0; v <= kWaves; ++v) {
                const uint32_t c = cum[r * (kWaves + 1) + v];
                if (c > 65536u || (v == 0 && c != 0u) || (v == kWaves && c != 65536u) || (v > 0 && c < cum[r * (kWaves + 1) + v - 1])) return hipErrorInvalidValue;
            }
        e = hipMemcpyToSymbol(HIP_SYMBOL(slab_cum), cum, 2 * (kWaves + 1) * sizeof(uint32_t));
    }
    return e;
}

hipError_t launch_grid_stamped(const GridArgs &a, int workgroups, hipStream_t stream)
{
    if (a.hist_variant != 3 || a.shift != 0) return hipErrorInvalidValue;
    hipLaunchKernelGGL((nmi_grid_kernel_stamped<true, false, 3>), dim3(workgroups), dim3(kBlock), 0, stream, a);
    return hipGetLastError();
}
#elif defined(NMI_GRID_KERNEL_GATED)
hipError_t launch_grid_gated(const GridArgs &a, int workgroups, bool use_bg, hipStream_t stream)
{
    if (a.hist_variant != 3 || !a.plan || (a.shift != 0 && !use_bg)) return hipErrorInvalidValue;
    const dim3 grid(workgroups), block(kBlock);
    if (a.shift != 0)
        hipLaunchKernelGGL((nmi_grid_kernel_gated<true, true, 3>), grid, block, 0, stream, a);
    else if (use_bg)
        hipLaunchKernelGGL((nmi_grid_kernel_gated<true, false, 3>), grid, block, 0, stream, a);
    else
        hipLaunchKernelGGL((nmi_grid_kernel_gated<false, false, 3>), grid, block, 0, stream, a);
    return hipGetLastError();
}
#else

#ifdef NMI_BUILD_ABLATIONS
namespace {

constexpr int kHalf = kBlock / 2;
constexpr int kDWaves = kWaves / 2;
constexpr int kDRows = kBins / kDWaves;
constexpr int kDPasses = kDRows / 4;

__device__ __forceinline__ int ws_row(int dwave, int pass, int r) { return dwave * kDRows + (r & 1) * 16 + pass * 2 + (r >> 1); }

__device__ __forceinline__ void drain_to_scratch(Lds &lds, uint32_t *__restrict__ slab, int wave, int lane)
{
    const int i = lane & 15, r = lane >> 4;
    const int dwave = wave >> 1, pass0 = (wave & 1) * (kDPasses / 2);
#pragma unroll
    for (int pp = 0; pp < kDPasses / 2; ++pp) {
        const int pass = pass0 + pp;
        const int d1 = ws_row(dwave, pass, r);
        uint32_t wd[8];
#pragma unroll
        for (int k = 0; k < 8; ++k) {
            const uint32_t idx = decode_word(d1, i, k);
            wd[k] = lds.joint[idx];
            lds.joint[idx] = 0;
        }
        uint32_t *dst = slab + ((dwave * kDPasses + pass) * 8) * 64 + lane;
#pragma unroll
        for (int k = 0; k < 8; ++k) dst[k * 64] = wd[k];
    }
}

__device__ __forceinline__ void load_pass(const uint32_t *__restrict__ src, uint32_t (&wd)[8])
{
#pragma unroll
    for (int k = 0; k < 8; ++k) wd[k] = __hip_atomic_load(src + k * 64, __ATOMIC_RELAXED, __HIP_MEMORY_SCOPE_AGENT);
}

__device__ __forceinline__ void decode_pass(Lds &lds, const GridArgs &a, int d1, int i, const uint32_t (&wd)[8],
                                            uint32_t (&col_lo)[8], uint32_t (&col_hi)[8], uint32_t &wave_total)
{
    uint32_t lo[8], hi[8], rsum = 0, cmax = 0;
    float tl[8], th[8];
#pragma unroll
    for (int k = 0; k < 8; ++k) {
        lo[k] = wd[k] & 0xFFFFu;
        hi[k] = wd[k] >> 16;
        col_lo[k] += lo[k];
        col_hi[k] += hi[k];
        rsum += lo[k] + hi[k];
        cmax = max(cmax, max(lo[k], hi[k]));
        tl[k] = lds.table[lo[k] & (kLdsTable - 1)];
        th[k] = lds.table[hi[k] & (kLdsTable - 1)];
    }
    if (__builtin_expect(cmax >= (uint32_t)kLdsTable, 0)) {
#pragma unroll
        for (int k = 0; k < 8; ++k) {
            if (lo[k] >= (uint32_t)kLdsTable) tl[k] = a.table[lo[k]];
            if (hi[k] >= (uint32_t)kLdsTable) th[k] = a.table[hi[k]];
        }
    }
    rsum = row_sum_16(rsum);
    wave_total += rsum;
    const float x = row_tree_16(lane_tree_16(tl, th));
    if (i == 0) {
        lds.hist_render[d1] = rsum;
        lds.joint_row_sums[d1] = x;
// ... 211 lines not shown
```

Measured before the change: 9.103 million.

## Add lean grid kernel computing per-image marginal entropies once instead of per candidate

Adds a lean variant of the grid NMI kernel for the case where every pixel counts (background on). Each candidate now computes only the joint-entropy term. The render and warped marginal entropies are computed once per image as extra ride-along tasks, and a final single-wave pass combines them into scores and the best key. This removes the per-candidate warped-histogram LDS atomics and the column accumulation. In exchange it adds a global marginals buffer, a few extra tasks and a serial finish loop over all candidates. The path is on by default (mode 1) when the extra tasks fit in the existing rounds.

```diff
diff --git a/include/nmi_hip.h b/include/nmi_hip.h
--- a/include/nmi_hip.h
+++ b/include/nmi_hip.h
@@ -224,6 +224,7 @@
 #define NMI_OPT_STAMPS 9
 #define NMI_OPT_STAMP_CANDIDATE 15
 #define NMI_OPT_WAVE_SHARES 16
+#define NMI_OPT_MARGINALS 17
 int nmi_set_option(nmi_ctx *ctx, int32_t option, int64_t value);
 
 int nmi_split_status(nmi_ctx *ctx, int32_t *timeouts, int32_t *cooldown_calls_left, int32_t *next_cooldown, int32_t *last_launch_parts);
@@ -235,6 +236,7 @@
 const char *nmi_last_error_detail(nmi_ctx *ctx);
 int nmi_get_info(nmi_ctx *ctx, int32_t *compute_units, int32_t *workgroups_per_launch, int32_t *lds_bytes);
 int nmi_last_content(nmi_ctx *ctx, int32_t *few_levels, int32_t *nr, int32_t *nw);
+int nmi_last_marginals(nmi_ctx *ctx);
 
 #ifdef __cplusplus
 }
diff --git a/orbslam2_nmi_amd/capi.py b/orbslam2_nmi_amd/capi.py
--- a/orbslam2_nmi_amd/capi.py
+++ b/orbslam2_nmi_amd/capi.py
@@ -27,7 +27,7 @@
     "nmi_texture_destroy", "nmi_render_mesh", "nmi_stream_create", "nmi_stream_destroy",
     "nmi_stream_submit", "nmi_stream_wait", "nmi_stream_keep_ratings", "nmi_stream_copy_ratings", "nmi_key_pack", "nmi_key_unpack", "nmi_search_grid_rccl", "nmi_search_grid_block_rccl",
     "nmi_rccl_unique_id", "nmi_rccl_comm_init", "nmi_rccl_comm_destroy", "nmi_set_profiling", "nmi_last_kernel_ms",
-    "nmi_set_option", "nmi_copy_term_table", "nmi_abi_version", "nmi_error_string", "nmi_last_error_detail", "nmi_get_info", "nmi_last_content", "nmi_sort_points", "nmi_sort_triangles",
+    "nmi_set_option", "nmi_copy_term_table", "nmi_abi_version", "nmi_error_string", "nmi_last_error_detail", "nmi_get_info", "nmi_last_content", "nmi_last_marginals", "nmi_sort_points", "nmi_sort_triangles",
     "nmi_split_status", "nmi_pix_status", "nmi_level_create_block", "nmi_level_create_mesh_block", "nmi_level_run_rccl", "nmi_stream_submit_block",
     "nmi_warp_stack_masked", "nmi_search_grid_masked", "nmi_last_mask_counts", "nmi_level_set_masks", "nmi_level_copy_masks",
     "nmi_render_points_masked", "nmi_render_mesh_masked", "nmi_search_grid_covered", "nmi_last_cover_counts",
@@ -166,6 +166,8 @@
     lib.nmi_last_error_detail.restype = C.c_char_p
     lib.nmi_get_info.argtypes = [vp, C.POINTER(i32), C.POINTER(i32), C.POINTER(i32)]
     lib.nmi_last_content.argtypes = [vp, C.POINTER(i32), C.POINTER(i32), C.POINTER(i32)]
+    if hasattr(lib, "nmi_last_marginals"):
+        lib.nmi_last_marginals.argtypes = [vp]
     lib.nmi_split_status.argtypes = [vp, C.POINTER(i32), C.POINTER(i32), C.POINTER(i32), C.POINTER(i32)]
     lib.nmi_pix_status.argtypes = [vp, C.POINTER(i32), C.POINTER(i32)]
     lib.nmi_sort_points.argtypes = [vp, vp, vp, C.c_int64, vp, vp]
@@ -325,6 +327,7 @@
     OPT_PIX_OWNER_BIAS = 14
     OPT_STAMP_CANDIDATE, OPT_WAVE_SHARES = 15, 16
     OPT_CONTENT_PATH, OPT_FEWLEVELS_BINS = 12, 13
+    OPT_MARGINALS = 17
 
     def set_option(self, option, value):
         self._check(self._lib.nmi_set_option(self._h, int(option), int(value)), "nmi_set_option")
@@ -349,6 +352,13 @@
         f, r, w = C.c_int32(0), C.c_int32(0), C.c_int32(0)
         self._check(self._lib.nmi_last_content(self._h, C.byref(f), C.byref(r), C.byref(w)), "nmi_last_content")
         return {"few_levels": bool(f.value), "nr": r.value, "nw": w.value}
+
+    def last_marginals(self):
+        if not hasattr(self._lib, "nmi_last_marginals"):
+            return False
+        v = self._lib.nmi_last_marginals(self._h)
+        self._check(min(v, 0), "nmi_last_marginals")
+        return bool(v)
 
     def split_status(self):
         v = [C.c_int32(0) for _ in range(4)]
diff --git a/orbslam2_nmi_amd/csrc/nmi_capi.cpp b/orbslam2_nmi_amd/csrc/nmi_capi.cpp
--- a/orbslam2_nmi_amd/csrc/nmi_capi.cpp
+++ b/orbslam2_nmi_amd/csrc/nmi_capi.cpp
@@ -60,6 +60,32 @@
     e.last_use = ++ctx->order_clock;
     *d_order = e.d;
     return NMI_OK;
+}
+
+int ensure_marginals(nmi_ctx *ctx, int S, int Wn)
+{
+    const size_t words = nmi::marginal_words(S, Wn);
+    if (words <= ctx->marginals_cap) return NMI_OK;
+    if (ctx->d_marginals) {
+        NMI_HIP_TRY(ctx, hipStreamSynchronize(ctx->stream));
+        NMI_HIP_TRY(ctx, hipFree(ctx->d_marginals));
+        ctx->d_marginals = nullptr;
+        ctx->marginals_cap = 0;
+    }
+    const size_t want = words + words / 2;
+    NMI_HIP_TRY(ctx, hipMalloc((void **)&ctx->d_marginals, want * sizeof(uint32_t)));
+    ctx->marginals_cap = want;
+    return NMI_OK;
+}
+
+bool choose_marginals(const nmi_ctx *ctx, int64_t total, int S, int Wn, int cap, int *workgroups)
+{
+    if (ctx->marginals_mode == 0 || total > (1ll << 24)) return false;
+    bool ride_along = false;
+    const int g = nmi::lean_workgroups(total, S, Wn, cap, &ride_along);
+    if (ctx->marginals_mode != 2 && !ride_along) return false;
+    *workgroups = g;
+    return true;
 }
 
 static void choose_split(const nmi_ctx *ctx, int64_t total, int cap, int *parts, int *pix_parts)
@@ -242,6 +268,7 @@
         ctx->last_parts = 0;
         ctx->last_pix = 0;
         ctx->last_epoch = 0;
+        ctx->last_marginals = 0;
         return NMI_OK;
     }
     const int cap = ctx->workgroups > 0 ? ctx->workgroups : ctx->compute_units;
@@ -305,6 +332,14 @@
     }
 #endif
     if (!parts && !few && ctx->hist_variant == 3 && ctx->content_path != 0) a.plan = ctx->d_plan;
+    bool lean = !parts && !pix && !few && ctx->hist_variant == 3 && p.use_bg && a.vec_ok && ctx->phase_mask == 3 && !dbg_joint && !dbg_h1 &&
+                !dbg_h2 && !dbg_sums && !ctx->dbg_stamps && !ctx->pair_renders && !a.score_post && !post_score;
+    lean = lean && choose_marginals(ctx, total, S_local, Wn, cap, &workgroups);
+    if (lean) {
+        const int mrc = ensure_marginals(ctx, S_local, Wn);
+        if (mrc != NMI_OK) return mrc;
+        a.marginals = ctx->d_marginals;
+    }
     if (few) {
         const size_t need = (size_t)(S_local + Wn) * (size_t)ctx->npix;
         if (need > ctx->rank_bytes) {
@@ -330,10 +365,13 @@
         NMI_HIP_TRY(ctx, nmi::launch_fewlevels(a, ctx->d_rank_stacks, ctx->d_rank_stacks + (size_t)S_local * ctx->npix, workgroups,
                                                p.use_bg != 0, ctx->stream));
         NMI_HIP_TRY(ctx, nmi::launch_grid_gated(a, workgroups, p.use_bg != 0, ctx->stream));
+    } else if (lean) {
+        NMI_HIP_TRY(ctx, nmi::launch_grid_lean(a, workgroups, ctx->stream));
     } else {
         NMI_HIP_TRY(ctx, nmi::launch_grid(a, workgroups, p.use_bg != 0, ctx->stream));
     }
     ctx->last_few = few ? 1 : 0;
+    ctx->last_marginals = lean ? 1 : 0;
     if (post) ++ctx->seq;
     if (post_score) ++ctx->pair_seq;
     ctx->posted = post;
@@ -596,6 +634,7 @@
     if (ctx->d_blocks) (void)hipFree(ctx->d_blocks);
     if (ctx->d_pix_timeouts) (void)hipFree(ctx->d_pix_timeouts);
     if (ctx->d_pix_blocks) (void)hipFree(ctx->d_pix_blocks);
+    if (ctx->d_marginals) (void)hipFree(ctx->d_marginals);
     if (ctx->h_split_error) (void)hipHostFree(ctx->h_split_error);
     if (ctx->level_post) (void)hipHostFree(ctx->level_post);
     if (ctx->d_plan) (void)hipFree(ctx->d_plan);
@@ -730,6 +769,10 @@
             ctx->few_hint = false;
         }
         return NMI_OK;
+    case NMI_OPT_MARGINALS:
+        if (value < 0 || value > 2) return NMI_ERR_INVALID_ARGUMENT;
+        ctx->marginals_mode = (int)value;
+        return NMI_OK;
     case NMI_OPT_WORKGROUPS:
         if (value < 0 || value > (1 << 20)) return NMI_ERR_INVALID_ARGUMENT;
         ctx->workgroups = (int)value;
@@ -765,6 +808,8 @@
     if (lds_bytes) *lds_bytes = nmi::grid_kernel_lds_bytes();
     return NMI_OK;
 }
+
+int nmi_last_marginals(nmi_ctx *ctx) { return ctx ? ctx->last_marginals : NMI_ERR_INVALID_ARGUMENT; }
 
 int nmi_last_content(nmi_ctx *ctx, int32_t *few_levels, int32_t *nr, int32_t *nw)
 {
diff --git a/orbslam2_nmi_amd/csrc/nmi_capi_masked.cpp b/orbslam2_nmi_amd/csrc/nmi_capi_masked.cpp
--- a/orbslam2_nmi_amd/csrc/nmi_capi_masked.cpp
+++ b/orbslam2_nmi_amd/csrc/nmi_capi_masked.cpp
@@ -136,6 +136,7 @@
     ctx->last_pix = pix;
     ctx->last_epoch = 0;
     ctx->last_few = 0;
+    ctx->last_marginals = 0;
     if (ctx->profiling) {
         NMI_HIP_TRY(ctx, hipEventRecord(ctx->ev_stop, ctx->stream));
         ctx->have_timing = true;
diff --git a/orbslam2_nmi_amd/csrc/nmi_capi_pipeline.cpp b/orbslam2_nmi_amd/csrc/nmi_capi_pipeline.cpp
--- a/orbslam2_nmi_amd/csrc/nmi_capi_pipeline.cpp
+++ b/orbslam2_nmi_amd/csrc/nmi_capi_pipeline.cpp
@@ -33,6 +33,8 @@
     uint32_t replay = 0;
     float *d_mvps = nullptr, *h_mvps = nullptr, *d_coeffs = nullptr, *h_coeffs = nullptr;
     int *d_order = nullptr;
+    uint32_t *d_marginals = nullptr;
+    bool lean = false;
     float *d_ratings = nullptr;
     unsigned long long *d_key = nullptr, *h_key = nullptr;
     unsigned int *d_done = nullptr;
@@ -71,7 +73,7 @@
     (void)hipStreamSynchronize(lv->ctx->stream);
     if (lv->exec) (void)hipGraphExecDestroy(lv->exec);
     if (lv->graph) (void)hipGraphDestroy(lv->graph);
-    void *dev[] = {lv->d_kept, lv->d_kept_count, lv->d_packed, lv->d_renders, lv->d_warps, lv->d_zbuf, lv->d_mvps, lv->d_coeffs, lv->d_order, lv->d_key, lv->d_done, lv->d_ratings, lv->d_epoch, lv->d_pix_blocks,
+    void *dev[] = {lv->d_kept, lv->d_kept_count, lv->d_packed, lv->d_renders, lv->d_warps, lv->d_zbuf, lv->d_mvps, lv->d_coeffs, lv->d_order, lv->d_marginals, lv->d_key, lv->d_done, lv->d_ratings, lv->d_epoch, lv->d_pix_blocks,
                    lv->d_masks, lv->d_counts, lv->d_tables, lv->d_redo, lv->d_redo_state, lv->d_rmasks, lv->d_cover_counts, lv->d_ud, lv->d_ud_mask, lv->d_small};
     for (void *q : dev)
         if (q) (void)hipFree(q);
@@ -164,6 +166,8 @@
         a.order = nullptr;
     }
     const int workgroups = lv->workgroups;
+    int grid_workgroups = workgroups;
+    lv->lean = !masked && !covered && !lv->pix && a.vec_ok && choose_marginals(ctx, total, S, Wn, cap, &grid_workgroups);
     nmi::GridArgs ma = a;
     ma.phase_mask = lv->pix ? 3 | (ctx->phase_mask & 512) : 3;
     const MaskSearch ms = mask_search_args(ma, lv->d_masks, covered ? lv->d_rmasks : nullptr, covered ? lv->d_cover_counts : lv->d_counts,
@@ -209,7 +213,10 @@
                                   ctx->d_pix_timeouts, st));
         else if (lv->pix)
             ok(nmi::launch_pix(a, lv->pix, pix_owner_share(ctx, lv->pix), true, lv->d_epoch, ctx->d_pix_timeouts, st));
-        else
+        else if (lv->lean) {
+            a.marginals = lv->d_marginals;
+            ok(nmi::launch_grid_lean(a, grid_workgroups, st));
+        } else
             ok(nmi::launch_grid(a, workgroups, true, st));
         hipError_t ec = hipStreamEndCapture(st, &graph);
         ok(ec);
@@ -342,6 +349,7 @@
     ok(hipMalloc((void **)&lv->d_mvps, ((size_t)S * 16 + nmi::kLevelMvpExtra) * sizeof(float)));
     ok(hipMalloc((void **)&lv->d_coeffs, (size_t)Wn * 9 * sizeof(float)));
     ok(hipMalloc((void **)&lv->d_order, (size_t)total * sizeof(int)));
+    ok(hipMalloc((void **)&lv->d_marginals, nmi::marginal_words(S, Wn) * sizeof(uint32_t)));
     ok(hipMalloc((void **)&lv->d_ratings, (size_t)total * sizeof(float)));
     ok(hipMalloc((void **)&lv->d_key, sizeof(unsigned long long)));
     ok(hipMalloc((void **)&lv->d_done, sizeof(unsigned int)));
@@ -489,6 +497,7 @@
         --lv->replay;
         return hip_fail(ctx, le, "hipGraphLaunch");
     }
+    ctx->last_marginals = lv->lean ? 1 : 0;
     return NMI_OK;
 }
 
@@ -762,6 +771,13 @@
     st->depth = depth;
     st->max_S = max_S;
     st->max_Wn = max_Wn;
+    {
+        const int mrc = ensure_marginals(ctx, max_S, max_Wn);
+        if (mrc != NMI_OK) {
+            delete st;
+            return mrc;
+        }
+    }
     st->slots = new (std::nothrow) nmi_stream::Slot[depth];
     const size_t npix = (size_t)ctx->npix;
     FirstError ok;
diff --git a/orbslam2_nmi_amd/csrc/nmi_ctx.h b/orbslam2_nmi_amd/csrc/nmi_ctx.h
--- a/orbslam2_nmi_amd/csrc/nmi_ctx.h
+++ b/orbslam2_nmi_amd/csrc/nmi_ctx.h
@@ -66,6 +66,10 @@
     OrderEntry orders[kOrderCache];
     uint64_t order_clock = 0;
     int xcd_tiling = 1;
+    uint32_t *d_marginals = nullptr;
+    size_t marginals_cap = 0;
+    int marginals_mode = 1;
+    int last_marginals = 0;
     nmi::SplitSlab *d_slabs = nullptr;
     int slab_cap = 0;
     unsigned long long *d_blocks = nullptr;
@@ -150,6 +154,8 @@
 int hip_fail(nmi_ctx *ctx, hipError_t e, const char *what);
 void build_order(int S, int Wn, int *order);
 int ensure_order(nmi_ctx *ctx, int S, int Wn, const int **d_order);
+int ensure_marginals(nmi_ctx *ctx, int S, int Wn);
+bool choose_marginals(const nmi_ctx *ctx, int64_t total, int S, int Wn, int cap, int *workgroups);
 int choose_pix(const nmi_ctx *ctx, const nmi::GridArgs &a, int64_t total, int cap);
 double pix_owner_share(const nmi_ctx *ctx, int pix);
 int next_split_epoch(nmi_ctx *ctx, uint32_t *epoch);
diff --git a/orbslam2_nmi_amd/csrc/nmi_grid_device.h b/orbslam2_nmi_amd/csrc/nmi_grid_device.h
--- a/orbslam2_nmi_amd/csrc/nmi_grid_device.h
+++ b/orbslam2_nmi_amd/csrc/nmi_grid_device.h
@@ -366,7 +366,7 @@
     }
 }
 
-template <bool ZERO0 = false>
+template <bool ZERO0 = false, bool LEAN = false>
 __device__ __forceinline__ void decode_phase(Lds &lds, int par, const GridArgs &a, int wave, int lane)
 {
     const uint32_t novf = lds.ovf_n[par] < (uint32_t)kOvfCap ? lds.ovf_n[par] : (uint32_t)kOvfCap;
@@ -427,8 +427,10 @@
         float tl[8], th[8];
 #pragma unroll
         for (int k = 0; k < 8; ++k) {
-            col_lo[k] += lo[k];
-            col_hi[k] += hi[k];
+            if (!LEAN) {
+                col_lo[k] += lo[k];
+                col_hi[k] += hi[k];
+            }
             rsum += lo[k] + hi[k];
             cmax = max(cmax, max(lo[k], hi[k]));
             tl[k] = lds.table[lo[k] & (kLdsTable - 1)];
@@ -445,10 +447,10 @@
         if (!ZERO0) wave_total += rsum;
         const float x = row_tree_16(lane_tree_16(tl, th));
         if (i == 0) {
-            lds.hist_render[d1] = rsum;
+            if (!LEAN) lds.hist_render[d1] = rsum;
             lds.joint_row_sums[d1] = x;
         }
-        if (a.dbg_joint) {
+        if (!LEAN && a.dbg_joint) {
             uint32_t *row = a.dbg_joint + d1 * kBins;
 #pragma unroll
             for (int k = 0; k < 8; ++k) {
@@ -458,20 +460,43 @@
             }
         }
     }
-#pragma unroll
-    for (int k = 0; k < 8; ++k) {
-        const int q = i + 16 * k;
-        atomicAdd(&lds.hist_warped[q], col_lo[k]);
-        atomicAdd(&lds.hist_warped[q + 128], col_hi[k]);
+    if (!LEAN) {
+#pragma unroll
+        for (int k = 0; k < 8; ++k) {
+            const int q = i + 16 * k;
+            atomicAdd(&lds.hist_warped[q], col_lo[k]);
+            atomicAdd(&lds.hist_warped[q + 128], col_hi[k]);
+        }
     }
     if (i == 0) atomicAdd(&lds.total[par], wave_total);
 }
 
+__device__ __forceinline__ uint32_t *sum_a3(const GridArgs &a, int p) { return a.marginals + p; }
+__device__ __forceinline__ uint32_t *sum_a1(const GridArgs &a, int s) { return a.marginals + a.S_local * a.Wn + s; }
+__device__ __forceinline__ uint32_t *sum_a2(const GridArgs &a, int w) { return a.marginals + a.S_local * a.Wn + a.S_local + w; }
+__device__ __forceinline__ void post_sum(uint32_t *slot, float x, unsigned long long &prev_key)
+{
+    prev_key |= (unsigned long long)__hip_atomic_exchange(slot, __float_as_uint(x), __ATOMIC_RELAXED, __HIP_MEMORY_SCOPE_AGENT);
+}
+
+enum { kFinalScore = 0, kFinalJoint = 1, kFinalMarginals = 2 };
+template <int FORM = kFinalScore>
 __device__ __forceinline__ void final_phase(Lds &lds, const GridArgs &a, int lane, int p, int w, int s,
                                             unsigned long long &prev_key)
 {
     const int i = lane & 15, r = lane >> 4;
     float lo[8], hi[8];
+    if (FORM == kFinalJoint) {
+#pragma unroll
+        for (int k = 0; k < 8; ++k) {
+            lo[k] = r == 2 ? lds.joint_row_sums[i + 16 * k] : 0.0f;
+            hi[k] = r == 2 ? lds.joint_row_sums[i + 16 * k + 128] : 0.0f;
+        }
+        const float xj = row_tree_16(lane_tree_16(lo, hi));
+        const float a3j = __shfl(xj, 32, 64);
+        if (lane == 0) post_sum(sum_a3(a, p), a3j, prev_key);
+        return;
+    }
     const uint32_t *h = r == 0 ? lds.hist_render : lds.hist_warped;
     uint32_t cl[8], ch[8];
 #pragma unroll
@@ -484,13 +509,18 @@
         lo[k] = a.table[cl[k]];
         hi[k] = a.table[ch[k]];
     }
-    if ((w == 0 || s == 0) && a.plan) {
+    if ((FORM == kFinalMarginals || w == 0 || s == 0) && a.plan) {
         uint32_t m = 0;
 #pragma unroll
         for (int k = 0; k < 8; ++k) m |= (cl[k] != 0u ? 1u << k : 0u) | (ch[k] != 0u ? 0x100u << k : 0u);
-        if (lane < 32 && m) __hip_atomic_fetch_or(const_cast<uint32_t *>(&a.plan->seen[lane]), m, __ATOMIC_RELAXED, __HIP_MEMORY_SCOPE_AGENT);
-    }
-    if (r == 2) {
+        if (FORM == kFinalMarginals) {
+            uint32_t got = 0;
+            if (lane < 32 && m) got = __hip_atomic_fetch_or(const_cast<uint32_t *>(&a.plan->seen[lane]), m, __ATOMIC_RELAXED, __HIP_MEMORY_SCOPE_AGENT);
+            prev_key |= (unsigned long long)(__ballot(got > 0xFFFFu) != 0ull);
+        } else if (lane < 32 && m)
+            __hip_atomic_fetch_or(const_cast<uint32_t *>(&a.plan->seen[lane]), m, __ATOMIC_RELAXED, __HIP_MEMORY_SCOPE_AGENT);
+    }
+    if (FORM == kFinalScore && r == 2) {
 #pragma unroll
         for (int k = 0; k < 8; ++k) {
             lo[k] = lds.joint_row_sums[i + 16 * k];
@@ -499,6 +529,11 @@
     }
     const float x = row_tree_16(lane_tree_16(lo, hi));
     const float a1 = __shfl(x, 0, 64), a2 = __shfl(x, 16, 64), a3 = __shfl(x, 32, 64);
+    if (FORM == kFinalMarginals) {
+        if (lane == 0 && p < a.S_local) post_sum(sum_a1(a, p), a1, prev_key);
+        if (lane == 0 && p < a.Wn) post_sum(sum_a2(a, p), a2, prev_key);
+        return;
+    }
     if (a.dbg_h1 && lane < 64) {
         for (int t = lane; t < kBins; t += 64) {
             a.dbg_h1[t] = lds.hist_render[t];
@@ -542,7 +577,7 @@
     }
 }
 
-template <bool SHIFTED, bool BG = true, bool ROWS = false>
+template <bool SHIFTED, bool BG = true, bool ROWS = false, bool LEAN = false>
 __device__ __forceinline__ void exact_candidate(Lds &lds, const GridArgs &a, int tid, int p, unsigned long long &prev_key)
 {
     const int lane = tid & 63, wave = tid >> 6;
@@ -551,17 +586,134 @@
     histogram_phase<true, SHIFTED, 1, kBlock, true, ROWS>(lds, 0, a, a.render_stack + (size_t)s * a.npix, a.warp_stack + (size_t)w * a.npix, tid, 0,
                                                           ROWS ? a.height * a.chunks_per_row : a.npix >> 4);
     __syncthreads();
-    decode_phase<!BG>(lds, 0, a, wave, lane);
+    decode_phase<!BG, LEAN>(lds, 0, a, wave, lane);
     __syncthreads();
     if (wave == 0) {
-        final_phase(lds, a, lane, p, w, s, prev_key);
-        for (int t = lane; t < kBins; t += 64) lds.hist_warped[t] = 0;
+        final_phase<LEAN ? kFinalJoint : kFinalScore>(lds, a, lane, p, w, s, prev_key);
+        if (!LEAN)
+            for (int t = lane; t < kBins; t += 64) lds.hist_warped[t] = 0;
         if (lane == 0) lds.ovf_n[0] = lds.total[0] = 0;
         if (lane < kSide) lds.side_key[0][lane] = lds.side_cnt[0][lane] = 0;
     }
     __syncthreads();
 }
 
-}
-
-}
+constexpr int kMargCopies = 32;
+static_assert(2 * kBins * kMargCopies <= kJointWords && 2 * kBins <= kBlock, "both histograms' copies live in the joint array, one thread per bin sums them");
+
+template <bool SHIFTED>
+__device__ __forceinline__ void marginal_task(Lds &lds, const GridArgs &a, int tid, int i, unsigned long long &prev_key)
+{
+    const int lane = tid & 63, wave = tid >> 6;
+    const uint32_t copy = (uint32_t)lane & (kMargCopies - 1);
+    const int nchunks = a.npix >> 4;
+#pragma unroll 1
+    for (int img = 0; img < 2; ++img) {
+        if (i >= (img ? a.Wn : a.S_local)) continue;
+        const uint8_t *src = (img ? a.warp_stack : a.render_stack) + (size_t)i * a.npix;
+        uint32_t *h = lds.joint + img * kBins * kMargCopies + copy;
+        for (int c = tid; c < nchunks; c += kBlock) {
+            const uint4 v = *reinterpret_cast<const uint4 *>(src + ((uint32_t)c << 4));
+            const uint32_t q[4] = {v.x, v.y, v.z, v.w};
+#pragma unroll
+            for (int j = 0; j < 16; ++j) {
+                uint32_t d = (q[j >> 2] >> (8 * (j & 3))) & 0xFFu;
+                if (SHIFTED) d >>= a.shift;
+                (void)__hip_atomic_fetch_add(&h[d * kMargCopies], 1u, __ATOMIC_RELAXED, __HIP_MEMORY_SCOPE_WORKGROUP);
+            }
+        }
+    }
+    __syncthreads();
+    if (tid < 2 * kBins) {
+        uint32_t *h = lds.joint + tid * kMargCopies;
+        uint32_t sum = 0;
+#pragma unroll
+        for (int j = 0; j < kMargCopies; ++j) {
+            const int c = (j + tid) & (kMargCopies - 1);
+            sum += h[c];
+            h[c] = 0;
+        }
+        (tid < kBins ? lds.hist_render : lds.hist_warped)[tid & (kBins - 1)] = sum;
+    }
+    __syncthreads();
+    if (wave == 0) final_phase<kFinalMarginals>(lds, a, lane, i, 0, 0, prev_key);
+}
+
+__device__ __forceinline__ void finish_search_lean(const GridArgs &a, int lane, unsigned long long prev_key)
+{
+    LevelPlan *plan = const_cast<LevelPlan *>(a.plan);
+    uint32_t arrived = 0;
+    if (lane == 0) {
+        const unsigned int one = prev_key == ~0ull ? 2u : 1u;
+        arrived = __hip_atomic_fetch_add(a.done, one, __ATOMIC_RELAXED, __HIP_MEMORY_SCOPE_AGENT);
+    }
+    if (__builtin_amdgcn_readfirstlane(arrived) != gridDim.x - 1) return;
+    uint32_t bits = 0;
+    unsigned long long *post = nullptr;
+    uint32_t state = 0, max_joint = 0;
+    if (plan && lane < 32) bits = __hip_atomic_exchange(&plan->seen[lane], 0u, __ATOMIC_RELAXED, __HIP_MEMORY_SCOPE_AGENT);
+    if (plan && lane == 0) post = plan->seen_post, state = plan->seen_state, max_joint = plan->seen_max_joint;
+    const int total = a.S_local * a.Wn;
+    constexpr int kBatch = 12;
+    unsigned long long best = 0;
+    for (int p0 = 0; p0 < total; p0 += 64 * kBatch) {
+        uint32_t b1[kBatch], b2[kBatch], b3[kBatch];
+#pragma unroll
+        for (int k = 0; k < kBatch; ++k) {
+            const int p = min(p0 + k * 64 + lane, total - 1);
+            const int w = p / a.S_local, s = p - w * a.S_local;
+            b3[k] = __hip_atomic_load(sum_a3(a, p), __ATOMIC_RELAXED, __HIP_MEMORY_SCOPE_AGENT);
+            b1[k] = __hip_atomic_load(sum_a1(a, s), __ATOMIC_RELAXED, __HIP_MEMORY_SCOPE_AGENT);
+            b2[k] = __hip_atomic_load(sum_a2(a, w), __ATOMIC_RELAXED, __HIP_MEMORY_SCOPE_AGENT);
+        }
+#pragma unroll
+        for (int k = 0; k < kBatch; ++k) {
+            const int p = p0 + k * 64 + lane;
+            if (p >= total) continue;
+            const int w = p / a.S_local, s = p - w * a.S_local;
+            const float a1 = __uint_as_float(b1[k]), a2 = __uint_as_float(b2[k]), a3 = __uint_as_float(b3[k]);
+            float score;
+            if (a1 == 0.0f && a2 == 0.0f && a3 == 0.0f)
+                score = 0.0f;
+            else if (a.mode == NMI_MODE_ENMI_)
+                score = ((-a1) + (-a2)) / (-a3);
+            else if (a.mode == NMI_MODE_SUC_)
+                score = 2.0f * (1.0f - ((-a3) / ((-a1) + (-a2))));
+            else
+                score = -1.0f;
+            if (a.ratings) a.ratings[p] = score;
+            if (score >= 0.0f) {
+                const uint32_t sbits = score == 0.0f ? 0u : __float_as_uint(score);
+                const uint32_t gidx = (uint32_t)(a.w_offset + w) * (uint32_t)a.S_total + (uint32_t)(a.s_offset + s);
+                const unsigned long long key = ((unsigned long long)sbits << 32) | (unsigned long long)(0xFFFFFFFFu - gidx);
+                best = key > best ? key : best;
+            }
+        }
+    }
+#pragma unroll
+    for (int off = 32; off > 0; off >>= 1) {
+        const unsigned long long other = __shfl_xor(best, off, 64);
+        best = other > best ? other : best;
+    }
+    if (lane == 0) {
+        __hip_atomic_store(a.done, 0u, __ATOMIC_RELAXED, __HIP_MEMORY_SCOPE_AGENT);
+        __hip_atomic_store(a.key, best, __ATOMIC_RELAXED, __HIP_MEMORY_SCOPE_AGENT);
+        if (a.out_key) __hip_atomic_store(a.out_key, best, __ATOMIC_RELAXED, __HIP_MEMORY_SCOPE_SYSTEM);
+        if (a.mailbox)
+            __hip_atomic_store(&a.mailbox->word, best | ((unsigned long long)(a.seq & 1u) << 63), __ATOMIC_RELAXED, __HIP_MEMORY_SCOPE_SYSTEM);
+    }
+    if (plan) {
+        const uint32_t n = row_sum_16((uint32_t)__popc(bits));
+        const uint32_t nw = (uint32_t)__shfl((int)n, 16, 64);
+        const uint32_t few = (n > 0u && nw > 0u && n * nw <= max_joint) ? 1u : 0u;
+        if (lane == 0 && post && few != state) {
+            plan->seen_state = few;
+            const uint32_t stamp = 0x80000000u | (uint32_t)wall_clock64();
+            __hip_atomic_store(post, ((unsigned long long)stamp << 32) | ((unsigned long long)n << 16) | nw, __ATOMIC_RELAXED, __HIP_MEMORY_SCOPE_SYSTEM);
+        }
+    }
+}
+
+}
+
+}
diff --git a/orbslam2_nmi_amd/csrc/nmi_kernels.h b/orbslam2_nmi_amd/csrc/nmi_kernels.h
--- a/orbslam2_nmi_amd/csrc/nmi_kernels.h
+++ b/orbslam2_nmi_amd/csrc/nmi_kernels.h
@@ -61,7 +61,10 @@
     unsigned int seq;
     unsigned long long *score_post;
     struct SplitSlab *slabs;
-    unsigned long long *blocks;
+    union {
+        unsigned long long *blocks;
+        uint32_t *marginals;
+    };
     uint32_t epoch;
     uint32_t *split_error;
     unsigned long long *dbg_stamps;
@@ -88,6 +91,15 @@
 hipError_t launch_grid(const GridArgs &a, int workgroups, bool use_bg, hipStream_t stream);
 hipError_t launch_grid_gated(const GridArgs &a, int workgroups, bool use_bg, hipStream_t stream);
 hipError_t launch_grid_rows(const GridArgs &a, int workgroups, bool use_bg, hipStream_t stream);
+hipError_t launch_grid_lean(const GridArgs &a, int workgroups, hipStream_t stream);
+inline size_t marginal_words(int S_local, int Wn) { return (size_t)S_local * Wn + (size_t)S_local + (size_t)Wn; }
+inline int lean_workgroups(int64_t total, int S_local, int Wn, int cap, bool *tasks_ride_along)
+{
+    const int64_t all = total + (S_local > Wn ? S_local : Wn);
+    const int64_t g = all < cap ? all : cap;
+    *tasks_ride_along = (all + g - 1) / g == (total + g - 1) / g;
+    return (int)g;
+}
 hipError_t launch_grid_stamped(const GridArgs &a, int workgroups, hipStream_t stream);
 hipError_t set_stamped_experiment(int k, const uint32_t *cum);
 
diff --git a/orbslam2_nmi_amd/csrc/nmi_kernels.hip b/orbslam2_nmi_amd/csrc/nmi_kernels.hip
--- a/orbslam2_nmi_amd/csrc/nmi_kernels.hip
+++ b/orbslam2_nmi_amd/csrc/nmi_kernels.hip
@@ -7,6 +7,8 @@
 
 #if defined(NMI_GRID_KERNEL_GATED)
 #define NMI_GRID_KERNEL_NAME nmi_grid_kernel_gated
+#elif defined(NMI_GRID_KERNEL_LEAN)
+#define NMI_GRID_KERNEL_NAME nmi_grid_kernel_lean
 #elif defined(NMI_GRID_KERNEL_STAMPED)
 #define NMI_GRID_KERNEL_NAME nmi_grid_kernel_stamped
 #elif defined(NMI_GRID_KERNEL_ROWS)
@@ -55,6 +57,12 @@
 #else
     constexpr bool kRows = false;
 #define NMI_ALL_CHUNKS (a.npix >> 4)
+#endif
+#ifdef NMI_GRID_KERNEL_LEAN
+    constexpr bool kLean = true;
+    static_assert(BG && HIST == 3, "the marginals are per image only when every pixel counts");
+#else
+    constexpr bool kLean = false;
 #endif
     constexpr bool kZero0 = !BG && kOptimistic && !SHIFTED;
     constexpr bool kCountAll = BG || kZero0;
@@ -113,7 +121,7 @@
 #endif
         __syncthreads();
         NMI_GRID_STAMP(3);
-        if (a.phase_mask & 2) decode_phase<kZero0>(lds, par, a, wave, lane);
+        if (a.phase_mask & 2) decode_phase<kZero0, kLean>(lds, par, a, wave, lane);
         __syncthreads();
         NMI_GRID_STAMP(4);
         if (kOptimistic && (a.phase_mask & 3) == 3 && lds.total[par] != (uint32_t)a.npix) {
@@ -121,8 +129,9 @@
             break;
         }
         if (wave == 0) {
-            if (a.phase_mask & 2) final_phase(lds, a, lane, p, w, s, prev_key);
-            for (int t = lane; t < kBins; t += 64) lds.hist_warped[t] = 0;
+            if (a.phase_mask & 2) final_phase<kLean ? kFinalJoint : kFinalScore>(lds, a, lane, p, w, s, prev_key);
+            if (!kLean)
+                for (int t = lane; t < kBins; t += 64) lds.hist_warped[t] = 0;
             if (lane == 0) {
                 lds.ovf_n[par] = 0;
                 lds.total[par ^ 1] = 0;
@@ -142,12 +151,21 @@
         if (tid < 2) lds.total[tid] = lds.ovf_n[tid] = 0;
         if (tid < 2 * kSide) (&lds.side_key[0][0])[tid] = (&lds.side_cnt[0][0])[tid] = 0;
         __syncthreads();
-        for (int o = exact_from; o < total; o += gridDim.x) exact_candidate<SHIFTED, !kZero0, kRows>(lds, a, tid, candidate_at(a, o), prev_key);
-    }
-
+        for (int o = exact_from; o < total; o += gridDim.x) exact_candidate<SHIFTED, !kZero0, kRows, kLean>(lds, a, tid, candidate_at(a, o), prev_key);
+    }
+
+#ifdef NMI_GRID_KERNEL_LEAN
+    {
+        const int tasks = max(a.S_local, a.Wn);
+        const int rounds = slot < total ? (total - slot + (int)gridDim.x - 1) / (int)gridDim.x : 0;
+        for (int o = slot + rounds * (int)gridDim.x; o < total + tasks; o += gridDim.x) marginal_task<SHIFTED>(lds, a, tid, o - total, prev_key);
+    }
+    if (wave == 0) finish_search_lean(a, lane, prev_key);
+#else
     if (wave == 0 && !(a.phase_mask & 16)) {
         finish_search(a, lane, prev_key, gridDim.x);
     }
+#endif
 #ifdef NMI_GRID_KERNEL_STAMPED
     stamp_on = true;
 #endif
@@ -197,6 +215,17 @@
 {
     if (a.hist_variant != 3 || a.shift != 0) return hipErrorInvalidValue;
     hipLaunchKernelGGL((nmi_grid_kernel_stamped<true, false, 3>), dim3(workgroups), dim3(kBlock), 0, stream, a);
+    return hipGetLastError();
+}
+#elif defined(NMI_GRID_KERNEL_LEAN)
+hipError_t launch_grid_lean(const GridArgs &a, int workgroups, hipStream_t stream)
+{
+    if (a.hist_variant != 3 || a.phase_mask != 3 || !a.vec_ok || !a.marginals) return hipErrorInvalidValue;
+    const dim3 grid(workgroups), block(kBlock);
+    if (a.shift != 0)
+        hipLaunchKernelGGL((nmi_grid_kernel_lean<true, true, 3>), grid, block, 0, stream, a);
+    else
+        hipLaunchKernelGGL((nmi_grid_kernel_lean<true, false, 3>), grid, block, 0, stream, a);
     return hipGetLastError();
 }
 #elif defined(NMI_GRID_KERNEL_GATED)
diff --git a/orbslam2_nmi_amd/csrc/nmi_kernels_lean.hip b/orbslam2_nmi_amd/csrc/nmi_kernels_lean.hip
--- /dev/null
+++ b/orbslam2_nmi_amd/csrc/nmi_kernels_lean.hip
@@ -0,0 +1,2 @@
+#define NMI_GRID_KERNEL_LEAN 1
+#include "nmi_kernels.hip"
```

Result: no change. 9.075 million (-0.3%).
